# junofficial/mppi_RobotArm

Hardware: AMD Instinct MI355X
Metric: MPPI rollouts/sec (K×T state-steps/s) + control-step latency, K=65536 T=64 (higher is better)
Workload: dtype f32

## Files before the change

### include/mppi_rocm.h

```cpp
#ifndef MPPI_ROCM_H
#define MPPI_ROCM_H

#ifdef __cplusplus
extern "C" {
#endif

#define MPPI_MAX_T 128
#define MPPI_SEARCH_LEN 30

#define MPPI_OK 0
#define MPPI_E_ARG -1
#define MPPI_E_HIP -2
#define MPPI_E_SINGULAR -3
#define MPPI_E_EXCHANGE -5
#define MPPI_E_RETRY -6
#define MPPI_E_PATH_END -4

#define MPPI_FLAG_FUSED_UPDATE 1u
#define MPPI_FLAG_EXCHANGE 2u
#define MPPI_FLAG_HOST_OUT 4u
#define MPPI_IPC_HANDLE_BYTES 64
#define MPPI_MAX_WORLD 8

typedef struct {
    double m1, m2, l1, l2, lc1, lc2, g;
    double fk_l1, fk_l2;
} mppi_arm_params;

typedef struct {
    int K_local;
    int T;
    int K_total;
    int k_offset;
    double delta_t;
    double param_lambda;
    double param_alpha;
    double param_exploration;
    double sigma[4];
    double stage_cost_weight[4];
    double terminal_cost_weight[4];
    mppi_arm_params arm;
    int lanes_per_sample;
    double param_gamma;
    int clamp_mode;
    double u_min[2];
    double u_max[2];
} mppi_config;

typedef struct mppi_ctx mppi_ctx;

void mppi_config_init(mppi_config *cfg);

int mppi_ctx_create(const mppi_config *cfg, int device, void *stream, mppi_ctx **out);
void mppi_ctx_destroy(mppi_ctx *ctx);
const char *mppi_last_error(void);
int mppi_set_stream(mppi_ctx *ctx, void *stream);
int mppi_ctx_info(const mppi_ctx *ctx, int *lanes_per_sample, int *blocks, int *threads_per_block);

int mppi_ctx_handoff(const mppi_ctx *ctx, int *poll);

int mppi_set_step_inputs(mppi_ctx *ctx, const double *x0, const double *window, int W,
                         const double *u);

int mppi_rollout(mppi_ctx *ctx, const float *noise_dev, double *S_dev, double *partial_dev,
                 unsigned flags);

int mppi_merge_partials(mppi_ctx *ctx, const double *partials_dev, int n, unsigned flags);

int mppi_exchange_handle(mppi_ctx *ctx, int world, void *handle_out);
int mppi_exchange_attach(mppi_ctx *ctx, int rank, int world, const void *handles);

int mppi_get_weighted_noise(mppi_ctx *ctx, double *w_eps_host );
int mppi_get_nominal(mppi_ctx *ctx, double *u_host );

int mppi_rollout_traj(mppi_ctx *ctx, const double *base_u, const float *noise_dev, int K,
                      float *out_dev);

typedef struct mppi_readback mppi_readback;
int mppi_readback_create(int device, int workers, int slots, long long chunk_floats, int copy_streams,
                         mppi_readback **out);
void mppi_readback_destroy(mppi_readback *rb);
int mppi_readback_run(mppi_readback *rb, void *stream, const float *src_dev, double *dst_host, long long n);

int mppi_optimal_traj(mppi_ctx *ctx, float *out_dev);

int mppi_get_step_outputs(mppi_ctx *ctx, double *u_host, const float *traj_dev, float *traj_host);

int mppi_optimal_traj_host(const mppi_ctx *ctx, const double *x0, const double *u_new, double *traj_out);

int mppi_wait_outputs(mppi_ctx *ctx, const double *x0, double *u_out, double *traj_out);

int mppi_step_dropin(mppi_ctx *ctx, const double *x0, const double *window, int W, const double *u,
                     const float *noise_dev, double *S_dev, float *next_noise_dev, unsigned long long seed,
                     unsigned long long next_step, double *u_out, double *traj_out);

typedef struct {
    const double *path;
    int rows, stride;
    double fk_l1, fk_l2;
    const double *x0;
    long long *idx;
    double *u;
    double *traj;
    const float *noise_dev;
    float *next_noise_dev;
    double *S_dev;
    unsigned long long seed;
} mppi_dropin_binding;

int mppi_dropin_bind(mppi_ctx *ctx, const mppi_dropin_binding *b);

int mppi_dropin_tick(mppi_ctx *ctx, unsigned long long next_step);

int mppi_dropin_tick_launch(mppi_ctx *ctx, unsigned long long next_step);
int mppi_dropin_tick_wait(mppi_ctx *ctx);

int mppi_noise_philox(mppi_ctx *ctx, unsigned long long seed, unsigned long long step,
                      float *out_dev);

int mppi_sync(mppi_ctx *ctx);

#define MPPI_MAX_OBSTACLES 8
int mppi_set_obstacles(mppi_ctx *ctx, int n, const double *discs, double cost);

int mppi_debug_obstacle_hits(mppi_ctx *ctx, const float *noise_dev, int K, unsigned *mask_dev,
                             float *dir_dev);

int mppi_debug_set_buffer(mppi_ctx *ctx, void *dbg_dev);

int mppi_debug_dropin_times(const mppi_ctx *ctx, double *us_out);

int mppi_debug_nearest(mppi_ctx *ctx, const float *noise_dev, int K, int *slot_dev, float *pos_dev);

#define MPPI_CHAIN_MAX_DOF 8

typedef struct {
    int n;
    double m[MPPI_CHAIN_MAX_DOF];
    double l[MPPI_CHAIN_MAX_DOF];
    double lc[MPPI_CHAIN_MAX_DOF];
    double I[MPPI_CHAIN_MAX_DOF];
    double fk[MPPI_CHAIN_MAX_DOF];
    double J[MPPI_CHAIN_MAX_DOF];
    double b[MPPI_CHAIN_MAX_DOF];
    double g;
} mppi_chain_params;

typedef struct {
    int K_local, T, K_total, k_offset;
    double delta_t, param_lambda, param_alpha, param_exploration;
    double sigma[MPPI_CHAIN_MAX_DOF * MPPI_CHAIN_MAX_DOF];
    double stage_cost_weight[4];
    double terminal_cost_weight[4];
    mppi_chain_params chain;
    int precision;
    int lanes_per_sample;
    double param_gamma;
    int clamp_mode;
    double u_min[MPPI_CHAIN_MAX_DOF];
    double u_max[MPPI_CHAIN_MAX_DOF];
} mppi_chain_config;

typedef struct mppi_chain_ctx mppi_chain_ctx;

void mppi_chain_config_init(mppi_chain_config *cfg);

int mppi_chain_ctx_create(const mppi_chain_config *cfg, int device, void *stream, mppi_chain_ctx **out);
void mppi_chain_ctx_destroy(mppi_chain_ctx *ctx);
int mppi_chain_set_stream(mppi_chain_ctx *ctx, void *stream);
int mppi_chain_ctx_info(const mppi_chain_ctx *ctx, int *blocks, int *threads_per_block, int *poll,
                        int *lanes_per_sample);
int mppi_chain_set_step_inputs(mppi_chain_ctx *ctx, const double *x0, const double *window, int W,
                               const double *u);
int mppi_chain_rollout(mppi_chain_ctx *ctx, const float *noise_dev, double *S_dev, double *partial_dev,
                       unsigned flags);
int mppi_chain_merge_partials(mppi_chain_ctx *ctx, const double *partials_dev, int n, unsigned flags);
int mppi_chain_exchange_handle(mppi_chain_ctx *ctx, int world, void *handle_out);
int mppi_chain_exchange_attach(mppi_chain_ctx *ctx, int rank, int world, const void *handles);
int mppi_chain_get_weighted_noise(mppi_chain_ctx *ctx, double *w_eps_host);
int mppi_chain_get_nominal(mppi_chain_ctx *ctx, double *u_host);
int mppi_chain_wait_outputs(mppi_chain_ctx *ctx, const double *x0, double *u_out, double *traj_out);
int mppi_chain_last_eta(const mppi_chain_ctx *ctx, double *eta);
int mppi_chain_optimal_traj_host(mppi_chain_ctx *ctx, const double *x0, const double *u_new, double *traj_out);
int mppi_chain_rollout_traj(mppi_chain_ctx *ctx, const double *base_u, const float *noise_dev, int K,
                            float *out_dev);
int mppi_chain_noise_philox(mppi_chain_ctx *ctx, unsigned long long seed, unsigned long long step,
                            float *out_dev);
int mppi_chain_sync(mppi_chain_ctx *ctx);
int mppi_chain_debug_set_buffer(mppi_chain_ctx *ctx, void *dbg_dev);
int mppi_chain_debug_slots(mppi_chain_ctx *ctx, const float *noise_dev, double *S_dev, int *slots_dev);

#define MPPI_NP_POLY_WORDS 312
#define MPPI_NP_LOG_DATA 274
#define MPPI_NP_MAX_DU 8
#define MPPI_NP_MAX_STREAMS 1024
#define MPPI_NP_MAX_NORMALS 2147483647LL

typedef struct {
    unsigned key[624];
    int pos;
    int has_gauss;
    double gauss;
} mppi_np_state;

typedef struct {
    void *out_dev;
    long long K, T;
    int du;
    long long k_offset, K_local;
    long long stride_t, stride_k, stride_d;
    int src[MPPI_NP_MAX_DU];
    double scale[MPPI_NP_MAX_DU];
    double mean[MPPI_NP_MAX_DU];
    int dot2;
    double mat[4];
} mppi_np_target;

typedef struct mppi_np_ctx mppi_np_ctx;

int mppi_np_ctx_create(int device, const double *log_params, mppi_np_ctx **out);
void mppi_np_ctx_destroy(mppi_np_ctx *ctx);
int mppi_np_plan(const mppi_np_ctx *ctx, long long n, int pos, int has_gauss, int *block_stride, int *streams);
int mppi_np_set_jumps(mppi_np_ctx *ctx, int block_stride, int streams, const unsigned long long *polys, int words);
int mppi_np_draw(mppi_np_ctx *ctx, void *stream, const mppi_np_state *st, long long n, const mppi_np_target *tgt);
int mppi_np_draw_result(mppi_np_ctx *ctx, mppi_np_state *st_out);

#ifdef __cplusplus
}
#endif
#endif
```

### mppi_robotarm_amd/_native.py

```python
from __future__ import annotations

import ctypes as C
import os

HERE = os.path.dirname(os.path.abspath(__file__))
LIB_PATH = os.environ.get("MPPI_LIB_PATH") or os.path.join(HERE, "_lib", "libmppi_rocm.so")

MPPI_MAX_T = 128
MPPI_SEARCH_LEN = 30
MPPI_OK = 0
MPPI_E_ARG = -1
MPPI_E_HIP = -2
MPPI_E_SINGULAR = -3
MPPI_E_PATH_END = -4
MPPI_E_EXCHANGE = -5
MPPI_E_RETRY = -6
MPPI_FLAG_FUSED_UPDATE = 1
MPPI_FLAG_EXCHANGE = 2
MPPI_FLAG_HOST_OUT = 4
DP = C.POINTER(C.c_double)
MPPI_IPC_HANDLE_BYTES = 64
MPPI_MAX_WORLD = 8
MPPI_MAX_OBSTACLES = 8

EXPORTS = (
    "mppi_ctx_create", "mppi_ctx_destroy", "mppi_last_error", "mppi_set_stream", "mppi_ctx_info", "mppi_ctx_handoff",
    "mppi_set_step_inputs", "mppi_rollout", "mppi_merge_partials", "mppi_exchange_handle", "mppi_exchange_attach",
    "mppi_get_weighted_noise",
    "mppi_get_nominal", "mppi_rollout_traj", "mppi_optimal_traj", "mppi_get_step_outputs", "mppi_step_dropin",
    "mppi_optimal_traj_host", "mppi_wait_outputs", "mppi_dropin_bind", "mppi_dropin_tick",
    "mppi_dropin_tick_launch", "mppi_dropin_tick_wait",
    "mppi_noise_philox",
    "mppi_sync", "mppi_debug_set_buffer",
    "mppi_debug_nearest", "mppi_debug_dropin_times", "mppi_set_obstacles", "mppi_debug_obstacle_hits",
    "mppi_chain_ctx_create", "mppi_chain_ctx_destroy", "mppi_chain_set_stream", "mppi_chain_ctx_info",
    "mppi_chain_set_step_inputs", "mppi_chain_rollout", "mppi_chain_merge_partials", "mppi_chain_exchange_handle",
    "mppi_chain_exchange_attach",
    "mppi_chain_get_weighted_noise", "mppi_chain_get_nominal", "mppi_chain_rollout_traj",
    "mppi_chain_noise_philox", "mppi_chain_sync", "mppi_chain_debug_set_buffer", "mppi_chain_debug_slots",
    "mppi_chain_wait_outputs", "mppi_chain_optimal_traj_host", "mppi_chain_last_eta",
    "mppi_config_init", "mppi_chain_config_init",
    "mppi_np_ctx_create", "mppi_np_ctx_destroy", "mppi_np_plan", "mppi_np_set_jumps", "mppi_np_draw",
    "mppi_np_draw_result", "mppi_readback_create", "mppi_readback_destroy", "mppi_readback_run",
)


class DropinBindingC(C.Structure):
    _fields_ = [("path", C.c_void_p), ("rows", C.c_int), ("stride", C.c_int), ("fk_l1", C.c_double),
                ("fk_l2", C.c_double), ("x0", C.c_void_p), ("idx", C.c_void_p), ("u", C.c_void_p),
                ("traj", C.c_void_p), ("noise_dev", C.c_void_p), ("next_noise_dev", C.c_void_p),
                ("S_dev", C.c_void_p), ("seed", C.c_ulonglong)]


NP_MAX_DU = 8
NP_LOG_DATA = 274
NP_POLY_WORDS = 312


class NpStateC(C.Structure):
    _fields_ = [("key", C.c_uint * 624), ("pos", C.c_int), ("has_gauss", C.c_int), ("gauss", C.c_double)]


class NpTargetC(C.Structure):
    _fields_ = [("out_dev", C.c_void_p), ("K", C.c_longlong), ("T", C.c_longlong), ("du", C.c_int),
                ("k_offset", C.c_longlong), ("K_local", C.c_longlong), ("stride_t", C.c_longlong),
                ("stride_k", C.c_longlong), ("stride_d", C.c_longlong), ("src", C.c_int * NP_MAX_DU),
                ("scale", C.c_double * NP_MAX_DU), ("mean", C.c_double * NP_MAX_DU), ("dot2", C.c_int),
                ("mat", C.c_double * 4)]


class ArmParamsC(C.Structure):
    _fields_ = [(n, C.c_double) for n in ("m1", "m2", "l1", "l2", "lc1", "lc2", "g", "fk_l1", "fk_l2")]


class ConfigC(C.Structure):
    _fields_ = [
        ("K_local", C.c_int), ("T", C.c_int), ("K_total", C.c_int), ("k_offset", C.c_int),
        ("delta_t", C.c_double), ("param_lambda", C.c_double), ("param_alpha", C.c_double),
        ("param_exploration", C.c_double), ("sigma", C.c_double * 4),
        ("stage_cost_weight", C.c_double * 4), ("terminal_cost_weight", C.c_double * 4),
        ("arm", ArmParamsC), ("lanes_per_sample", C.c_int), ("param_gamma", C.c_double),
        ("clamp_mode", C.c_int), ("u_min", C.c_double * 2), ("u_max", C.c_double * 2),
    ]

    def __init__(self, *args, **kw):
        super().__init__(*args, **kw)
        if "param_gamma" not in kw and len(args) <= [f for f, _ in self._fields_].index("param_gamma"):
            self.param_gamma = float("nan")


CHAIN_MAX_DOF = 8


class ChainParamsC(C.Structure):
    _fields_ = [("n", C.c_int)] + [(f, C.c_double * CHAIN_MAX_DOF) for f in ("m", "l", "lc", "I", "fk", "J", "b")] + \
               [("g", C.c_double)]


class ChainConfigC(C.Structure):
    _fields_ = [
        ("K_local", C.c_int), ("T", C.c_int), ("K_total", C.c_int), ("k_offset", C.c_int),
        ("delta_t", C.c_double), ("param_lambda", C.c_double), ("param_alpha", C.c_double),
        ("param_exploration", C.c_double), ("sigma", C.c_double * (CHAIN_MAX_DOF * CHAIN_MAX_DOF)),
        ("stage_cost_weight", C.c_double * 4), ("terminal_cost_weight", C.c_double * 4),
        ("chain", ChainParamsC), ("precision", C.c_int), ("lanes_per_sample", C.c_int),
        ("param_gamma", C.c_double),
        ("clamp_mode", C.c_int), ("u_min", C.c_double * CHAIN_MAX_DOF), ("u_max", C.c_double * CHAIN_MAX_DOF),
    ]

    def __init__(self, *args, **kw):
        super().__init__(*args, **kw)
        if "param_gamma" not in kw and len(args) <= [f for f, _ in self._fields_].index("param_gamma"):
            self.param_gamma = float("nan")


class MPPIError(RuntimeError):
    """A failed C-ABI call (message from mppi_last_error)."""


class ExchangeError(MPPIError):
    """MPPI_E_EXCHANGE: the in-launch multi-GPU exchange of a step missed its poll bound on some rank.  Every
    rank of that step raises it and none applied the update (the controllers then run the step again over
    the collective fallback)."""


_lib = None


def open_library(path: str):
    if not os.path.exists(path):
        raise OSError(f"{path} is missing: build it with `python -c 'import __graft_entry__ as g; g.build()'`")
    L = C.CDLL(path)
    vp, dp, fp, ip = C.c_void_p, C.POINTER(C.c_double), C.c_void_p, C.POINTER(C.c_int)
    sig = {
        "mppi_ctx_create": ([C.POINTER(ConfigC), C.c_int, vp, C.POINTER(vp)], C.c_int),
        "mppi_ctx_destroy": ([vp], None),
        "mppi_last_error": ([], C.c_char_p),
        "mppi_set_stream": ([vp, vp], C.c_int),
        "mppi_ctx_info": ([vp, ip, ip, ip], C.c_int),
        "mppi_ctx_handoff": ([vp, ip], C.c_int),
        "mppi_set_step_inputs": ([vp, dp, dp, C.c_int, dp], C.c_int),
        "mppi_rollout": ([vp, fp, vp, vp, C.c_uint], C.c_int),
        "mppi_merge_partials": ([vp, vp, C.c_int, C.c_uint], C.c_int),
        "mppi_exchange_handle": ([vp, C.c_int, vp], C.c_int),
        "mppi_exchange_attach": ([vp, C.c_int, C.c_int, vp], C.c_int),
        "mppi_get_weighted_noise": ([vp, dp], C.c_int),
        "mppi_get_nominal": ([vp, dp], C.c_int),
        "mppi_rollout_traj": ([vp, dp, fp, C.c_int, fp], C.c_int),
        "mppi_optimal_traj": ([vp, fp], C.c_int),
        "mppi_get_step_outputs": ([vp, dp, fp, fp], C.c_int),
        "mppi_optimal_traj_host": ([vp, dp, dp, dp], C.c_int),
        "mppi_wait_outputs": ([vp, dp, dp, dp], C.c_int),
        "mppi_step_dropin": ([vp, vp, vp, C.c_int, vp, vp, vp, vp, C.c_ulonglong, C.c_ulonglong, vp, vp], C.c_int),
        "mppi_noise_philox": ([vp, C.c_ulonglong, C.c_ulonglong, fp], C.c_int),
        "mppi_dropin_bind": ([vp, C.POINTER(DropinBindingC)], C.c_int),
        "mppi_dropin_tick": ([vp, C.c_ulonglong], C.c_int),
        "mppi_dropin_tick_launch": ([vp, C.c_ulonglong], C.c_int),
        "mppi_dropin_tick_wait": ([vp], C.c_int),
        "mppi_sync": ([vp], C.c_int),
        "mppi_debug_set_buffer": ([vp, vp], C.c_int),
        "mppi_debug_dropin_times": ([vp, dp], C.c_int),
        "mppi_debug_nearest": ([vp, fp, C.c_int, vp, fp], C.c_int),
        "mppi_set_obstacles": ([vp, C.c_int, dp, C.c_double], C.c_int),
        "mppi_debug_obstacle_hits": ([vp, fp, C.c_int, vp, fp], C.c_int),
        "mppi_chain_ctx_create": ([C.POINTER(ChainConfigC), C.c_int, vp, C.POINTER(vp)], C.c_int),
        "mppi_chain_ctx_destroy": ([vp], None),
        "mppi_chain_set_stream": ([vp, vp], C.c_int),
        "mppi_chain_ctx_info": ([vp, ip, ip, ip, ip], C.c_int),
        "mppi_chain_set_step_inputs": ([vp, dp, dp, C.c_int, dp], C.c_int),
        "mppi_chain_rollout": ([vp, fp, vp, vp, C.c_uint], C.c_int),
        "mppi_chain_merge_partials": ([vp, vp, C.c_int, C.c_uint], C.c_int),
        "mppi_chain_exchange_handle": ([vp, C.c_int, vp], C.c_int),
        "mppi_chain_exchange_attach": ([vp, C.c_int, C.c_int, vp], C.c_int),
        "mppi_chain_get_weighted_noise": ([vp, dp], C.c_int),
        "mppi_chain_get_nominal": ([vp, dp], C.c_int),
        "mppi_chain_rollout_traj": ([vp, dp, fp, C.c_int, fp], C.c_int),
        "mppi_chain_noise_philox": ([vp, C.c_ulonglong, C.c_ulonglong, fp], C.c_int),
        "mppi_chain_sync": ([vp], C.c_int),
        "mppi_chain_debug_set_buffer": ([vp, vp], C.c_int),
        "mppi_chain_debug_slots": ([vp, fp, vp, vp], C.c_int),
        "mppi_chain_wait_outputs": ([vp, dp, dp, dp], C.c_int),
        "mppi_chain_optimal_traj_host": ([vp, dp, dp, dp], C.c_int),
        "mppi_chain_last_eta": ([vp, dp], C.c_int),
        "mppi_config_init": ([C.POINTER(ConfigC)], None),
        "mppi_np_ctx_create": ([C.c_int, vp, C.POINTER(vp)], C.c_int),
        "mppi_np_ctx_destroy": ([vp], None),
        "mppi_np_plan": ([vp, C.c_longlong, C.c_int, C.c_int, ip, ip], C.c_int),
        "mppi_np_set_jumps": ([vp, C.c_int, C.c_int, vp, C.c_int], C.c_int),
        "mppi_np_draw": ([vp, vp, C.POINTER(NpStateC), C.c_longlong, C.POINTER(NpTargetC)], C.c_int),
        "mppi_np_draw_result": ([vp, C.POINTER(NpStateC)], C.c_int),
        "mppi_chain_config_init": ([C.POINTER(ChainConfigC)], None),
        "mppi_readback_create": ([C.c_int, C.c_int, C.c_int, C.c_longlong, C.c_int, C.POINTER(vp)], C.c_int),
        "mppi_readback_destroy": ([vp], None),
        "mppi_readback_run": ([vp, vp, vp, vp, C.c_longlong], C.c_int),
    }
    for name, (args, res) in sig.items():
        if not hasattr(L, name):
            continue
        fn = getattr(L, name)
        fn.argtypes = args
        fn.restype = res
    return L


def load():
    global _lib
    if _lib is None:
        L = open_library(LIB_PATH)
        missing = [n for n in EXPORTS if not hasattr(L, n)]
        if missing:
            raise OSError(f"{LIB_PATH} is stale (missing {', '.join(missing)}): rebuild it")
        _lib = L
    return _lib


def check(rc: int, what: str) -> None:
    if rc != MPPI_OK:
        msg = load().mppi_last_error().decode(errors="replace")
        if rc == MPPI_E_SINGULAR:
            import numpy as np
            raise np.linalg.LinAlgError(msg)
        if rc == MPPI_E_ARG:
            raise ValueError(f"{what}: {msg}")
        if rc == MPPI_E_EXCHANGE:
            raise ExchangeError(f"{what}: {msg}")
        raise MPPIError(f"{what} failed ({rc}): {msg}")
```

### mppi_robotarm_amd/csrc/mppi_device.h

```cpp
#pragma once

#include <hip/hip_runtime.h>

#include <math.h>
#include <stdint.h>

#include <type_traits>
#include <utility>

#include "mppi_rocm.h"

namespace mppi {

#ifdef MPPI_STAMPS
#define STAMP(slot, val) do { if (dbg && threadIdx.x == 0) dbg[(size_t)blockIdx.x * 16 + (slot)] = (val); } while (0)
#define NOW() __builtin_amdgcn_s_memrealtime()
#else
#define STAMP(slot, val) do { (void)dbg; } while (0)
#define NOW() 0ull
#endif

constexpr int kMaxT = MPPI_MAX_T;

constexpr int kSlots = 32;
constexpr float kPadKey = 1.0e30f;
constexpr int kMaxWaves = 16;
constexpr int kGroup = 16;
constexpr double kMergeFloor = 5.421010862427522e-20;
constexpr int kDirectRows = 256;
constexpr int kDirectMax = 16;
constexpr int kSparseMax = 16;


__device__ __forceinline__ void sincos_f32(float x, float* s, float* c) { __sincosf(x, s, c); }

constexpr bool kDppBC = true;
template <int CTRL>
__device__ __forceinline__ float dpp_f32(float v) {
    return __int_as_float(__builtin_amdgcn_mov_dpp(__float_as_int(v), CTRL, 0xF, 0xF, kDppBC));
}

__device__ __forceinline__ int lanes_below(unsigned long long mask) {
    return __builtin_amdgcn_mbcnt_hi((unsigned)(mask >> 32), __builtin_amdgcn_mbcnt_lo((unsigned)mask, 0u));
}

template <int CTRL>
__device__ __forceinline__ double dpp_f64(double v) {
    const long long b = __double_as_longlong(v);
    const int lo = __builtin_amdgcn_mov_dpp((int)b, CTRL, 0xF, 0xF, kDppBC);
    const int hi = __builtin_amdgcn_mov_dpp((int)(b >> 32), CTRL, 0xF, 0xF, kDppBC);
    return __longlong_as_double(((long long)hi << 32) | (unsigned)lo);
}

__device__ __forceinline__ double readlane_f64(double v, int l) {
    const long long b = __double_as_longlong(v);
    const int lo = __builtin_amdgcn_readlane((int)b, l);
    const int hi = __builtin_amdgcn_readlane((int)(b >> 32), l);
    return __longlong_as_double(((long long)hi << 32) | (unsigned)lo);
}
__device__ __forceinline__ float readlane_f32(float v, int l) {
    return __int_as_float(__builtin_amdgcn_readlane(__float_as_int(v), l));
}

__device__ __forceinline__ double min_raw_f64(double a, double b) {
    double r;
    asm("v_min_f64 %0, %1, %2" : "=v"(r) : "v"(a), "v"(b));
    return r;
}
__device__ __forceinline__ double max_raw_f64(double a, double b) {
    double r;
    asm("v_max_f64 %0, %1, %2" : "=v"(r) : "v"(a), "v"(b));
    return r;
}

template <class T, class Op>
__device__ __forceinline__ T wave_reduce(T v, Op op) {
    if constexpr (sizeof(T) == 8) {
        v = op(v, dpp_f64<0xB1>(v));
        v = op(v, dpp_f64<0x4E>(v));
        v = op(v, dpp_f64<0x141>(v));
        v = op(v, dpp_f64<0x140>(v));
        return op(op(readlane_f64(v, 0), readlane_f64(v, 16)), op(readlane_f64(v, 32), readlane_f64(v, 48)));
    } else {
        v = op(v, dpp_f32<0xB1>(v));
        v = op(v, dpp_f32<0x4E>(v));
        v = op(v, dpp_f32<0x141>(v));
        v = op(v, dpp_f32<0x140>(v));
        return op(op(readlane_f32(v, 0), readlane_f32(v, 16)), op(readlane_f32(v, 32), readlane_f32(v, 48)));
    }
}
struct OpMin {
    __device__ double operator()(double a, double b) const { return min_raw_f64(a, b); }
};
struct OpAdd {
    template <class T>
    __device__ T operator()(T a, T b) const { return a + b; }
};
__device__ __forceinline__ double wave_min_f64(double v) { return wave_reduce(v, OpMin{}); }
__device__ __forceinline__ double wave_sum_f64(double v) { return wave_reduce(v, OpAdd{}); }
__device__ __forceinline__ float wave_sum_f32(float v) { return wave_reduce(v, OpAdd{}); }

__device__ __forceinline__ int select_bit(unsigned long long m, int k) {
    int pos = 0;
#pragma unroll
    for (int w = 32; w > 0; w >>= 1) {
        const int cnt = __popcll(m & ((1ull << w) - 1));
        if (k >= cnt) {
            k -= cnt;
            m >>= w;
            pos += w;
        }
    }
    return pos;
}

template <class F, int... I>
__device__ __forceinline__ void unroll_seq(F&& f, std::integer_sequence<int, I...>) {
    (f(std::integral_constant<int, I>{}), ...);
}

#define PIN_LOADS() asm volatile("" ::: "memory")

typedef __attribute__((address_space(4))) const float cfloat;
__device__ __forceinline__ float4 const_ld4(cfloat* p) { return make_float4(p[0], p[1], p[2], p[3]); }

typedef float f32x2 __attribute__((ext_vector_type(2)));
typedef float f32x4 __attribute__((ext_vector_type(4)));

__device__ __forceinline__ float min3_raw(float a, float b, float c) {
    float r;
    asm("v_min3_f32 %0, %1, %2, %3" : "=v"(r) : "v"(a), "v"(b), "v"(c));
    return r;
}
__device__ __forceinline__ float min_raw(float a, float b) {
    float r;
    asm("v_min_f32 %0, %1, %2" : "=v"(r) : "v"(a), "v"(b));
    return r;
}


template <int N>
__device__ __forceinline__ float min_tree(const float (&k)[N]) {
    if constexpr (N == 1) {
        return k[0];
    } else {
        constexpr int M = (N + 2) / 3;
        float r[M];
#pragma unroll
        for (int g = 0; g < M; ++g) {
            const int a = 3 * g;
            if (a + 2 < N) r[g] = min3_raw(k[a], k[a + 1], k[a + 2]);
            else if (a + 1 < N) r[g] = min_raw(k[a], k[a + 1]);
            else r[g] = k[a];
        }
        return min_tree<M>(r);
    }
}

template <int LPS, bool PRECISE = false>
struct Search {
    static constexpr int SL = ((MPPI_SEARCH_LEN + LPS - 1) / LPS + 1) & ~1;
    static constexpr int SP = SL / 2;
    f32x2 krx[SP], kry[SP], kc[SP];
    int sub;
    float cx, cy;

    __device__ __forceinline__ void load(const float4* key, float4 ctr, int lane_sub) {
        static_assert(SL * LPS <= kSlots, "window slots");
        if (LPS == 1) {
            int z;
            asm volatile("v_mov_b32 %0, 0" : "=v"(z));
            sub = z;
        } else {
            sub = lane_sub;
        }
#pragma unroll
        for (int i = 0; i < SP; ++i) {
            const float4 k0 = key[sub * SL + 2 * i];
            const float4 k1 = key[sub * SL + 2 * i + 1];
            krx[i] = f32x2{k0.x, k1.x};
            kry[i] = f32x2{k0.y, k1.y};
            kc[i] = f32x2{k0.z, k1.z};
        }
        cx = ctr.x;
        cy = ctr.y;
    }

    __device__ __forceinline__ unsigned nearest(float px, float py) const { return nearest_d(px - cx, py - cy); }

    __device__ __forceinline__ unsigned nearest_d(float dx, float dy) const {
        const f32x2 ax2 = {dx, dx}, ay2 = {dy, dy};
        const float pp = fmaf(dx, dx, dy * dy);
        const f32x2 pp2 = {pp, pp};
        float kk[2 * SP];
#pragma unroll
        for (int i = 0; i < SP; ++i) {
            f32x2 key = __builtin_elementwise_fma(ax2, krx[i], __builtin_elementwise_fma(ay2, kry[i], kc[i]));
            if constexpr (PRECISE) key = key + pp2;
            const unsigned j = (unsigned)(sub * SL + 2 * i);
            const float k0 = __uint_as_float((__float_as_uint(key.x) & ~31u) | j);
            const float k1 = __uint_as_float((__float_as_uint(key.y) & ~31u) | (j + 1));
            kk[2 * i] = k0;
            kk[2 * i + 1] = k1;
        }
        float best = min_tree<2 * SP>(kk);
        if (LPS >= 2) best = min_raw(best, dpp_f32<0xB1>(best));
        if (LPS >= 4) best = min_raw(best, dpp_f32<0x4E>(best));
        if (LPS >= 8) best = min_raw(best, dpp_f32<0x141>(best));
        if (LPS >= 16) best = min_raw(best, dpp_f32<0x128>(best));
        return __float_as_uint(best) & 31u;
    }
};

struct alignas(16) KeyPair {
    float4 xy;
    float4 c;
};
constexpr int kKeyPairs = kSlots / 2;

template <bool PRECISE = false>
struct SearchLDS {
    const KeyPair* kp;
    float cx, cy;

    __device__ __forceinline__ static void fill(KeyPair* dst, const float4* key, int tid) {
        if (tid < kKeyPairs) {
            const float4 k0 = key[2 * tid], k1 = key[2 * tid + 1];
            dst[tid].xy = make_float4(k0.x, k1.x, k0.y, k1.y);
            dst[tid].c = make_float4(k0.z, k1.z, 0.f, 0.f);
        }
    }

    __device__ __forceinline__ unsigned nearest(float px, float py) const {
        const float dx = px - cx, dy = py - cy;
        const f32x2 ax2 = {dx, dx}, ay2 = {dy, dy};
        const float pp = fmaf(dx, dx, dy * dy);
        const f32x2 pp2 = {pp, pp};
        float best = 3.0e38f;
        constexpr int SP = (MPPI_SEARCH_LEN + 1) / 2;
#pragma unroll
        for (int i = 0; i < SP; ++i) {
            const float4 xy = kp[i].xy, cc = kp[i].c;
            f32x2 key = __builtin_elementwise_fma(ax2, f32x2{xy.x, xy.y},
                                                  __builtin_elementwise_fma(ay2, f32x2{xy.z, xy.w}, f32x2{cc.x, cc.y}));
            if constexpr (PRECISE) key = key + pp2;
            const unsigned j = (unsigned)(2 * i);
            const float k0 = __uint_as_float((__float_as_uint(key.x) & ~31u) | j);
            const float k1 = __uint_as_float((__float_as_uint(key.y) & ~31u) | (j + 1));
            best = min3_raw(best, k0, k1);
        }
        return __float_as_uint(best) & 31u;
    }
};

template <int NL>
__device__ __forceinline__ double gather_col_n(const float* base, int kstride, const int* s_k, const double* s_e,
                                               int nl) {
    float e[NL];
#pragma unroll
    for (int l = 0; l < NL; ++l) e[l] = base[(size_t)(nl > 0 ? s_k[min(l, nl - 1)] : 0) * kstride];
    double acc = 0.0;
#pragma unroll
    for (int l = 0; l < NL; ++l)
        if (l < nl) acc = fma(s_e[l], (double)e[l], acc);
    return acc;
}
__device__ __forceinline__ double gather_col(const float* base, int kstride, const int* s_k, const double* s_e,
                                             int nl) {
    static_assert(kSparseMax == 16, "buckets");
    if (nl <= 1) return gather_col_n<1>(base, kstride, s_k, s_e, nl);
    if (nl <= 2) return gather_col_n<2>(base, kstride, s_k, s_e, nl);
    if (nl <= 4) return gather_col_n<4>(base, kstride, s_k, s_e, nl);
    if (nl <= 8) return gather_col_n<8>(base, kstride, s_k, s_e, nl);
    return gather_col_n<16>(base, kstride, s_k, s_e, nl);
}

__device__ __forceinline__ float weighted_sq(float ex, float ey, float e1, float e2, const float* w) {
    return fmaf(w[0], ex * ex, fmaf(w[1], ey * ey, fmaf(w[2], e1 * e1, w[3] * e2 * e2)));
}


typedef unsigned int u32x2 __attribute__((__vector_size__(2 * sizeof(unsigned int))));
typedef unsigned int u32x4 __attribute__((__vector_size__(4 * sizeof(unsigned int))));
constexpr int kSC1 = 16;

__device__ __forceinline__ __amdgpu_buffer_rsrc_t rows_rsrc(const void* p, int bytes) {
    return __builtin_amdgcn_make_buffer_rsrc(const_cast<void*>(p), 0, bytes, 0x00020000);
}
__device__ __forceinline__ double ld_wt(__amdgpu_buffer_rsrc_t r, int idx) {
    return __builtin_bit_cast(double, __builtin_amdgcn_raw_buffer_load_b64(r, idx * 8, 0, kSC1));
}
__device__ __forceinline__ void st_wt(__amdgpu_buffer_rsrc_t r, int idx, double v) {
    __builtin_amdgcn_raw_buffer_store_b64(__builtin_bit_cast(u32x2, v), r, idx * 8, 0, kSC1);
}
constexpr int kOffRange = 1 << 26;

__device__ __forceinline__ void st_gran(__amdgpu_buffer_rsrc_t r, int idx, double v, unsigned tag) {
    const unsigned long long b = (unsigned long long)__double_as_longlong(v);
    const u32x4 x = {(unsigned)b, tag, (unsigned)(b >> 32), tag};
    __builtin_amdgcn_raw_buffer_store_b128(x, r, idx * 16, 0, kSC1);
}
__device__ __forceinline__ u32x4 ld_gran(__amdgpu_buffer_rsrc_t r, int idx) {
    return __builtin_amdgcn_raw_buffer_load_b128(r, idx * 16, 0, kSC1);
}
__device__ __forceinline__ bool gran_ok(u32x4 x, unsigned tag) { return x[1] == tag && x[3] == tag; }
__device__ __forceinline__ double gran_val(u32x4 x) {
    return __longlong_as_double((long long)(((unsigned long long)x[2] << 32) | x[0]));
}
constexpr unsigned kSpinMax = 1u << 20;
__device__ __forceinline__ void report_timeout(unsigned* tmo) {
    if (tmo) __hip_atomic_store(tmo, 1u, __ATOMIC_RELAXED, __HIP_MEMORY_SCOPE_SYSTEM);
}
#define MPPI_SPIN_OR_GIVE_UP(spins, tmo, lane) MPPI_SPIN_OR_GIVE_UP_L(spins, 0ull, tmo, lane, (void)0)
#define MPPI_SPIN_OR_GIVE_UP_L(spins, deadline, tmo, lane, on_give_up)                                   \
    if (spins >= kSpinMax || ((deadline) && __builtin_amdgcn_s_memrealtime() > (deadline))) {            \
        if ((lane) == 0) report_timeout(tmo);                                                            \
        on_give_up;                                                                                      \
        break;                                                                                           \
    }                                                                                                    \
    __builtin_amdgcn_s_sleep(1)

__device__ __forceinline__ unsigned long long ord_key(double x) {
    const unsigned long long b = (unsigned long long)__double_as_longlong(x);
    return (b >> 63) ? ~b : (b | (1ull << 63));
}
__device__ __forceinline__ double ord_val(unsigned long long k) {
    return __longlong_as_double((long long)((k >> 63) ? (k & ~(1ull << 63)) : ~k));
}


template <int MAXV>
struct MergeScratch {
    double red[kMaxWaves];
    double weps[MAXV];
    double unew[MAXV];
    double rho[kDirectRows];
    double part[2 * kDirectRows];
    double eta;
    double rho_fin;
    int nrel;
};

template <int NT, class SM>
__device__ __forceinline__ double block_min_f64(double v, SM& sm) {
    const int lane = threadIdx.x & 63, wave = threadIdx.x >> 6;
    v = wave_min_f64(v);
    if (lane == 0) sm.red[wave] = v;
    __syncthreads();
    double r = sm.red[0];
#pragma unroll
    for (int w = 1; w < NT / 64; ++w) r = min_raw_f64(r, sm.red[w]);
    return r;
}

struct RowGeo {
    int stride, ncol;
    __device__ explicit RowGeo(int nval) : stride(2 + nval), ncol(1 + nval) {}
};

template <int NT, int MAXCH, class SM>
__device__ __forceinline__ void put_final(double rho, const double (&acc)[MAXCH], double eta, int nrel,
                                          const RowGeo& geo, SM& sm, double* out_row, double* w_eps_out) {
    const int tid = threadIdx.x;
#pragma unroll
    for (int ch = 0; ch < MAXCH; ++ch) {
        const int col = tid + ch * NT;
        if (col >= geo.ncol) continue;
        if (col == 0) {
            sm.nrel = nrel;
            sm.eta = eta;
            sm.rho_fin = rho;
            if (out_row) {
                out_row[0] = rho;
                out_row[1] = acc[ch];
            }
        } else {
            if (out_row) out_row[1 + col] = acc[ch];
            const double w = acc[ch] / eta;
            sm.weps[col - 1] = w;
            if (w_eps_out) w_eps_out[col - 1] = w;
        }
    }
    __syncthreads();
}

template <int NT, int MAXCH, bool final, bool GRAN, class SM>
__device__ __forceinline__ void merge_rows_block(__amdgpu_buffer_rsrc_t rows, int row0, int n, const RowGeo& geo,
                                                 double inv_lambda, SM& sm, const __amdgpu_buffer_rsrc_t* out_wt,
                                                 int out_idx, double* out_row, double* w_eps_out, unsigned tag,
                                                 unsigned* tmo, unsigned long long deadline = 0ull,
                                                 bool* failed = nullptr) {
    constexpr bool EAGER = !GRAN && MAXCH == 1;
    constexpr int LB = EAGER ? 32 : 16;
    constexpr int RB = LB / MAXCH;
    constexpr int R1 = EAGER ? 32 : 16;
    static_assert(RB >= 1 && R1 <= 64, "one row per lane");
    const int tid = threadIdx.x, lane = tid & 63;
    const int stride = geo.stride, ncol = geo.ncol;
    double acc[MAXCH], eta = 0.0, rho = INFINITY;
#pragma unroll
    for (int ch = 0; ch < MAXCH; ++ch) acc[ch] = 0.0;
    int nrel = 0;
    bool gave_up = false;
    for (int r0 = 0; r0 < n; r0 += R1) {
        const int nr = min(R1, n - r0);
        const int rb = row0 + r0;
        const int lrow = lane < nr ? (rb + lane) * stride : kOffRange;
        double rho_r, eta_l = 0.0, v[EAGER ? LB : 1];
        if constexpr (GRAN) {
            u32x4 gr;
            for (unsigned spins = 0;; ++spins) {
                asm volatile("" ::: "memory");
                gr = ld_gran(rows, lrow);
                if (__all(lane >= nr || gran_ok(gr, tag))) break;
                MPPI_SPIN_OR_GIVE_UP_L(spins, deadline, tmo, lane, gave_up = true);
            }
            rho_r = gran_val(gr);
        } else if constexpr (!EAGER) {
            rho_r = ld_wt(rows, lrow);
        } else {
            rho_r = ld_wt(rows, lrow);
            eta_l = ld_wt(rows, lrow + 1);
#pragma unroll
            for (int j = 0; j < LB; ++j) {
                const int i = j / MAXCH, col = tid + (j % MAXCH) * NT;
                v[j] = ld_wt(rows, (i < nr && col < ncol) ? (rb + i) * stride + 1 + col : kOffRange);
            }
        }
        const double rho_l = lane < nr ? rho_r : INFINITY;
        const double rnew = min_raw_f64(rho, wave_min_f64(rho_l));
        double s_l = 0.0;
        if (lane < nr) {
            const double s = exp((rnew - rho_l) * inv_lambda);
            s_l = s >= kMergeFloor ? s : 0.0;
        }
        const unsigned long long rel = __ballot(s_l != 0.0);
        const int nrr = __popcll(rel);
        nrel += nrr;
        if (rnew < rho && rho != INFINITY) {
            const double f = exp((rnew - rho) * inv_lambda);
#pragma unroll
            for (int ch = 0; ch < MAXCH; ++ch) acc[ch] *= f;
            eta *= f;
        }
        rho = rnew;
        if constexpr (EAGER) {
#pragma unroll
            for (int j = 0; j < LB; ++j) {
                const int i = j / MAXCH, ch = j % MAXCH;
                if (i < nr) {
                    const double s = readlane_f64(s_l, i);
                    if (s != 0.0) {
                        acc[ch] = fma(s, v[j], acc[ch]);
                        if (ch == 0) eta = fma(s, readlane_f64(eta_l, i), eta);
                    }
                }
            }
        } else {
            const int krow = lane < nrr ? select_bit(rel, lane) : 0;
            for (int b0 = 0; b0 < nrr; b0 += RB) {
                const bool eta_on = b0 == 0 && lane < nrr;
                const int eidx = eta_on ? (rb + krow) * stride + 1 : kOffRange;
                double x[LB];
                if constexpr (GRAN) {
                    u32x4 ge, gv[LB];
                    for (unsigned spins = 0;; ++spins) {
                        asm volatile("" ::: "memory");
                        ge = ld_gran(rows, eidx);
                        bool ok = !eta_on || gran_ok(ge, tag);
#pragma unroll
                        for (int j = 0; j < LB; ++j) {
                            const int i = b0 + j / MAXCH, col = tid + (j % MAXCH) * NT;
                            const bool on = i < nrr && col < ncol;
                            gv[j] = ld_gran(rows, on ? (rb + __builtin_amdgcn_readlane(krow, i)) * stride + 1 + col
                                                     : kOffRange);
                            ok = ok && (!on || gran_ok(gv[j], tag));
                        }
                        if (__all(ok)) break;
                        MPPI_SPIN_OR_GIVE_UP_L(spins, deadline, tmo, lane, gave_up = true);
                    }
                    if (eta_on) eta_l = gran_val(ge);
#pragma unroll
                    for (int j = 0; j < LB; ++j) x[j] = gran_val(gv[j]);
                } else {
                    if (b0 == 0) eta_l = ld_wt(rows, eidx);
#pragma unroll
                    for (int j = 0; j < LB; ++j) {
                        const int i = b0 + j / MAXCH, col = tid + (j % MAXCH) * NT;
                        x[j] = ld_wt(rows, (i < nrr && col < ncol)
                                               ? (rb + __builtin_amdgcn_readlane(krow, i)) * stride + 1 + col
                                               : kOffRange);
                    }
                }
#pragma unroll
                for (int j = 0; j < LB; ++j) {
                    const int i = b0 + j / MAXCH, ch = j % MAXCH;
                    if (i < nrr) {
                        const double s = readlane_f64(s_l, __builtin_amdgcn_readlane(krow, i));
                        acc[ch] = fma(s, x[j], acc[ch]);
                        if (ch == 0) eta = fma(s, readlane_f64(eta_l, i), eta);
                    }
                }
            }
        }
    }
    if (failed) *failed = __syncthreads_or(gave_up);
    if constexpr (final) {
        put_final<NT, MAXCH>(rho, acc, eta, nrel, geo, sm, out_row, w_eps_out);
    } else {
        auto put = [&](int col, double x) {
            if constexpr (GRAN) st_gran(*out_wt, out_idx * stride + col, x, tag);
            else st_wt(*out_wt, out_idx * stride + col, x);
        };
#pragma unroll
        for (int ch = 0; ch < MAXCH; ++ch) {
            const int col = tid + ch * NT;
            if (col >= ncol) continue;
            if (col == 0) put(0, rho);
            put(1 + col, acc[ch]);
        }
    }
}

template <int NT, int MAXCH, bool GRAN, class SM>
__device__ __forceinline__ bool direct_merge(__amdgpu_buffer_rsrc_t rows, int n, const RowGeo& geo,
                                             double inv_lambda, SM& sm, double* out_row, double* w_eps_out,
                                             unsigned tag, unsigned* tmo, unsigned long long* dbg = nullptr) {
    constexpr int P = kDirectRows / 64;
    constexpr int LB = 16;
    constexpr int RB = LB / MAXCH;
    const int tid = threadIdx.x, lane = tid & 63;
    const int stride = geo.stride, ncol = geo.ncol;
    double rho_l[P];
    if constexpr (GRAN) {
        if (tid < 64) {
            u32x4 gr[P];
            for (unsigned spins = 0;; ++spins) {
                asm volatile("" ::: "memory");
                bool ok = true;
#pragma unroll
                for (int j = 0; j < P; ++j) {
                    const int r = lane + 64 * j;
                    gr[j] = ld_gran(rows, r < n ? r * stride : kOffRange);
                    ok = ok && (r >= n || gran_ok(gr[j], tag));
                }
                if (__all(ok)) break;
                MPPI_SPIN_OR_GIVE_UP(spins, tmo, lane);
            }
#pragma unroll
            for (int j = 0; j < P; ++j) sm.rho[lane + 64 * j] = lane + 64 * j < n ? gran_val(gr[j]) : INFINITY;
        }
        __syncthreads();
#pragma unroll
        for (int j = 0; j < P; ++j) rho_l[j] = sm.rho[lane + 64 * j];
    } else {
#pragma unroll
        for (int j = 0; j < P; ++j) {
            const int r = lane + 64 * j;
            const double x = ld_wt(rows, r < n ? r * stride : kOffRange);
            rho_l[j] = r < n ? x : INFINITY;
        }
    }
    double m = rho_l[0];
#pragma unroll
    for (int j = 1; j < P; ++j) m = min_raw_f64(m, rho_l[j]);
    const double rho = wave_min_f64(m);
    double s_l[P];
    unsigned long long rel[P];
    int nrel = 0;
#pragma unroll
    for (int j = 0; j < P; ++j) {
        const double s = exp((rho - rho_l[j]) * inv_lambda);
        s_l[j] = (lane + 64 * j < n && s >= kMergeFloor) ? s : 0.0;
        rel[j] = __ballot(s_l[j] != 0.0);
        nrel += __popcll(rel[j]);
    }
    const int G = MAXCH == 1 ? max(1, NT / ncol) : 1;
    if (nrel > (G > 1 ? min(64, 2 * kDirectMax * G) : kDirectMax)) return false;
    int k = lane, row = 0;
    bool found = false;
#pragma unroll
    for (int j = 0; j < P; ++j) {
        const int cnt = __popcll(rel[j]);
        if (!found && k < cnt) {
            row = 64 * j + select_bit(rel[j], k);
            found = true;
        } else if (!found) {
            k -= cnt;
        }
    }
    double sk = 0.0;
#pragma unroll
    for (int j = 0; j < P; ++j) {
        const double sj = __shfl(s_l[j], row & 63);
        if ((row >> 6) == j) sk = sj;
    }
    const bool mine = lane < nrel;
    STAMP(13, NOW());
    double acc[MAXCH], eta = 0.0, eta_k = 0.0;
#pragma unroll
    for (int ch = 0; ch < MAXCH; ++ch) acc[ch] = 0.0;
    if (G == 1) {
        for (int b0 = 0; b0 < nrel; b0 += RB) {
            double v[LB];
            if constexpr (GRAN) {
                const bool eta_on = b0 == 0 && mine;
                u32x4 ge, gv[LB];
                for (unsigned spins = 0;; ++spins) {
                    asm volatile("" ::: "memory");
                    ge = ld_gran(rows, eta_on ? row * stride + 1 : kOffRange);
                    bool ok = !eta_on || gran_ok(ge, tag);
#pragma unroll
                    for (int j = 0; j < LB; ++j) {
                        const int i = b0 + j / MAXCH, col = tid + (j % MAXCH) * NT;
                        const bool on = i < nrel && col < ncol;
                        gv[j] = ld_gran(rows, on ? __builtin_amdgcn_readlane(row, i) * stride + 1 + col : kOffRange);
                        ok = ok && (!on || gran_ok(gv[j], tag));
                    }
                    if (__all(ok)) break;
                    MPPI_SPIN_OR_GIVE_UP(spins, tmo, lane);
                }
                if (eta_on) eta_k = gran_val(ge);
#pragma unroll
                for (int j = 0; j < LB; ++j) v[j] = gran_val(gv[j]);
            } else {
                if (b0 == 0) eta_k = ld_wt(rows, mine ? row * stride + 1 : kOffRange);
#pragma unroll
                for (int j = 0; j < LB; ++j) {
                    const int i = b0 + j / MAXCH, col = tid + (j % MAXCH) * NT;
                    v[j] = ld_wt(rows, (i < nrel && col < ncol) ? __builtin_amdgcn_readlane(row, i) * stride + 1 + col
                                                                 : kOffRange);
                }
            }
#pragma unroll
            for (int j = 0; j < LB; ++j) {
                const int i = b0 + j / MAXCH, ch = j % MAXCH;
                if (i < nrel) {
                    const double s = readlane_f64(sk, i);
                    acc[ch] = fma(s, v[j], acc[ch]);
                    if (ch == 0) eta = fma(s, readlane_f64(eta_k, i), eta);
                }
            }
        }
    } else {
        const int grp = tid / ncol, gcol = tid - grp * ncol;
        const bool active = grp < G;
        for (int b0 = 0; b0 < nrel; b0 += RB * G) {
            double v[LB], sf[LB];
            int roff[LB];
            bool on[LB];
#pragma unroll
            for (int j = 0; j < LB; ++j) {
                const int i = b0 + grp + G * j;
                on[j] = active && i < nrel;
                const int r = __builtin_amdgcn_ds_bpermute(min(i, 63) << 2, row);
                sf[j] = __shfl(sk, min(i, 63));
                roff[j] = on[j] ? r * stride + 1 + gcol : kOffRange;
            }
            if constexpr (GRAN) {
                u32x4 gv[LB];
                for (unsigned spins = 0;; ++spins) {
                    asm volatile("" ::: "memory");
                    bool ok = true;
#pragma unroll
                    for (int j = 0; j < LB; ++j) {
                        gv[j] = ld_gran(rows, roff[j]);
                        ok = ok && (!on[j] || gran_ok(gv[j], tag));
                    }
                    if (__all(ok)) break;
                    MPPI_SPIN_OR_GIVE_UP(spins, tmo, lane);
                }
#pragma unroll
                for (int j = 0; j < LB; ++j) v[j] = gran_val(gv[j]);
            } else {
#pragma unroll
                for (int j = 0; j < LB; ++j) v[j] = ld_wt(rows, roff[j]);
            }
#pragma unroll
            for (int j = 0; j < LB; ++j)
                if (on[j]) acc[0] = fma(sf[j], v[j], acc[0]);
        }
        if (active) sm.part[tid] = acc[0];
        __syncthreads();
        if (grp == 0) {
            double a = sm.part[gcol];
            for (int g = 1; g < G; ++g) a += sm.part[g * ncol + gcol];
            acc[0] = a;
            if (tid == 0) sm.red[0] = a;
        }
        __syncthreads();
        eta = sm.red[0];
    }
    STAMP(14, NOW());
    put_final<NT, MAXCH>(rho, acc, eta, nrel, geo, sm, out_row, w_eps_out);
    return true;
}

__device__ __forceinline__ bool arrive_last(unsigned* counter, unsigned expected, unsigned* s_flag, bool acquire) {
    asm volatile("s_waitcnt vmcnt(0)" ::: "memory");
    __syncthreads();
    if (threadIdx.x == 0) {
        const unsigned prev = __hip_atomic_fetch_add(counter, 1u, __ATOMIC_RELAXED, __HIP_MEMORY_SCOPE_AGENT);
        const bool last = prev == expected - 1;
        if (last) __hip_atomic_store(counter, 0u, __ATOMIC_RELAXED, __HIP_MEMORY_SCOPE_AGENT);
        if (last && acquire) {
            __builtin_amdgcn_fence(__ATOMIC_ACQUIRE, "agent");
            asm volatile("s_waitcnt vmcnt(0)" ::: "memory");
        }
        *s_flag = last ? 1u : 0u;
    }
    __syncthreads();
    return *s_flag != 0;
}


struct LaneWeight {
    double wgt;
    bool nz;
    unsigned long long bal;
};

__device__ __forceinline__ LaneWeight block_weigh(bool owner, double S, double rho_b, double inv_lambda, int lane,
                                                  int wave, int* s_cnt, double* s_redd) {
    const double warg = (rho_b - S) * inv_lambda;
    double wgt = 0.0;
    if (__any(owner && warg >= -45.0)) wgt = owner ? exp(warg) : 0.0;
    const bool nz = wgt >= kMergeFloor;
    const unsigned long long bal = __ballot(nz);
    const double esum = wave_sum_f64(nz ? wgt : 0.0);
    if (lane == 0) {
        s_cnt[wave] = __popcll(bal);
        s_redd[wave] = esum;
    }
    return LaneWeight{wgt, nz, bal};
}

template <int NT>
__device__ __forceinline__ int block_compact(const LaneWeight& lw, int k, int wave, const int* s_cnt,
                                             const double* s_redd, int* s_k, double* s_e, double* eta_b) {
    int off = 0, nl = 0;
    double eta = 0.0;
#pragma unroll
    for (int w = 0; w < NT / 64; ++w) {
        off += (w < wave) ? s_cnt[w] : 0;
        nl += s_cnt[w];
        eta += s_redd[w];
    }
    if (lw.nz) {
        const int pos = off + lanes_below(lw.bal);
        s_k[pos] = k;
        s_e[pos] = lw.wgt;
    }
    *eta_b = eta;
    return nl;
}

template <int NT, int NS>
__device__ __forceinline__ void dense_weights(const LaneWeight& lw, int k, int K, double* s_e,
                                              double (&w)[(NS + 63) / 64]) {
    const int tid = threadIdx.x, lane = tid & 63;
    const int k0 = blockIdx.x * NS;
    if (tid < NS) s_e[tid] = 0.0;
    __syncthreads();
    if (lw.nz) s_e[k - k0] = lw.wgt;
    __syncthreads();
#pragma unroll
    for (int i = 0; i < (NS + 63) / 64; ++i) {
        const int ks = lane + 64 * i;
        w[i] = (ks < NS && k0 + ks < K) ? s_e[ks] : 0.0;
    }
}

template <int NT, int MAXCH, bool POLL, class SM>
__device__ __forceinline__ bool handoff_merge(__amdgpu_buffer_rsrc_t slab_r, __amdgpu_buffer_rsrc_t gslab_r, int nrows,
                                              const RowGeo& geo, double inv_lambda, SM& sm, unsigned* counters,
                                              bool acquire, unsigned* s_flag, double* partial_out, double* w_eps_out,
                                              unsigned tag, unsigned* epoch, unsigned* tmo, unsigned long long* dbg,
                                              unsigned long long* direct_dbg) {
    const int ngroups = (nrows + kGroup - 1) / kGroup;
    const int g = blockIdx.x / kGroup;
    const int gsz = min(kGroup, nrows - g * kGroup);
    if constexpr (POLL) {
        if ((int)blockIdx.x != g * kGroup) return false;
        STAMP(3, NOW());
        if (ngroups == 1) {
            merge_rows_block<NT, MAXCH, true, true>(slab_r, 0, gsz, geo, inv_lambda, sm, nullptr, 0, partial_out,
                                                    w_eps_out, tag, tmo);
        } else if (blockIdx.x == 0 && nrows <= kDirectRows &&
                   direct_merge<NT, MAXCH, true>(slab_r, nrows, geo, inv_lambda, sm, partial_out, w_eps_out, tag, tmo,
                                                 direct_dbg)) {
        } else {
            merge_rows_block<NT, MAXCH, false, true>(slab_r, g * kGroup, gsz, geo, inv_lambda, sm, &gslab_r, g, nullptr,
                                                     nullptr, tag, tmo);
            STAMP(10, NOW());
            if (blockIdx.x != 0) return false;
            STAMP(4, NOW());
            merge_rows_block<NT, MAXCH, true, true>(gslab_r, 0, ngroups, geo, inv_lambda, sm, nullptr, 0, partial_out,
                                                    w_eps_out, tag, tmo);
        }
        if (threadIdx.x == 0) __hip_atomic_store(epoch, tag, __ATOMIC_RELAXED, __HIP_MEMORY_SCOPE_AGENT);
    } else {
        if (!arrive_last(counters + g, (unsigned)gsz, s_flag, acquire)) return false;
        STAMP(3, NOW());
        merge_rows_block<NT, MAXCH, false, false>(slab_r, g * kGroup, gsz, geo, inv_lambda, sm, &gslab_r, g, nullptr,
                                                  nullptr, 0u, nullptr);
        STAMP(10, NOW());
        if (!arrive_last(counters + ngroups, (unsigned)ngroups, s_flag, acquire)) return false;
        STAMP(4, NOW());
        if (!(ngroups > 1 && nrows <= kDirectRows &&
              direct_merge<NT, MAXCH, false>(slab_r, nrows, geo, inv_lambda, sm, partial_out, w_eps_out, 0u, nullptr)))
            merge_rows_block<NT, MAXCH, true, false>(gslab_r, 0, ngroups, geo, inv_lambda, sm, nullptr, 0, partial_out,
                                                     w_eps_out, 0u, nullptr);
    }
    return true;
}

__device__ __forceinline__ double median10(double* v) {
#define CX(i, j) { const double lo = min_raw_f64(v[i], v[j]), hi = max_raw_f64(v[i], v[j]); v[i] = lo; v[j] = hi; }
    CX(4, 9) CX(3, 8) CX(2, 7) CX(1, 6) CX(0, 5) CX(1, 4) CX(6, 9) CX(0, 3) CX(5, 8) CX(0, 2)
    CX(3, 6) CX(7, 9) CX(0, 1) CX(2, 4) CX(5, 7) CX(8, 9) CX(1, 2) CX(4, 6) CX(7, 8) CX(3, 5)
    CX(2, 5) CX(6, 8) CX(1, 3) CX(4, 7) CX(2, 3) CX(6, 7) CX(3, 4) CX(5, 6) CX(4, 5)
#undef CX
    return v[5];
}

template <class SM>
__device__ __forceinline__ double median_at(const SM& sm, int t, int d, int T, int du) {
    double v[10];
#pragma unroll
    for (int i = 0; i < 10; ++i) {
        int m = t - 5 + i;
        m = m < 0 ? -m - 1 : m;
        m = m >= T ? 2 * T - 1 - m : m;
        v[i] = sm.weps[m * du + d];
    }
    return median10(v);
}


__device__ __forceinline__ unsigned long long mul_wide(unsigned a, unsigned m) {
    return (unsigned long long)a * m;
}
__device__ __forceinline__ unsigned xor3(unsigned a, unsigned b, unsigned k) {
    unsigned r;
    asm("v_bitop3_b32 %0, %1, %2, %3 bitop3:0x96" : "=v"(r) : "v"(a), "v"(b), "s"(k));
    return r;
}
__device__ __forceinline__ uint4 philox4x32_10(uint4 ctr, uint2 key) {
#pragma unroll
    for (int r = 0; r < 10; ++r) {
        const unsigned long long p0 = mul_wide(ctr.x, 0xD2511F53u);
        const unsigned long long p1 = mul_wide(ctr.z, 0xCD9E8D57u);
        ctr = make_uint4(xor3((unsigned)(p1 >> 32), ctr.y, key.x), (unsigned)p1,
                         xor3((unsigned)(p0 >> 32), ctr.w, key.y), (unsigned)p0);
        key.x += 0x9E3779B9u;
        key.y += 0xBB67AE85u;
    }
    return ctr;
}

constexpr double kBoxMullerScale = 1.1774100225154747;
__device__ __forceinline__ float2 box_muller(unsigned a, unsigned b) {
    const float inv = 2.3283064365386963e-10f;
    const float u0 = fmaf((float)a, inv, inv), u1 = (float)b * inv;
    const float r = __builtin_amdgcn_sqrtf(-__builtin_amdgcn_logf(u0));
    return make_float2(r * __builtin_amdgcn_cosf(u1), r * __builtin_amdgcn_sinf(u1));
}

}

namespace mppi {

constexpr int kMaxWorld = MPPI_MAX_WORLD;
struct XDesc {
    const void* peer[kMaxWorld];
    double* row;
    unsigned* epoch;
    int rank, world, bytes;
    unsigned timeout_ticks;
};
constexpr unsigned kTmoLocal = 1u, kTmoExchange = 2u, kTmoSplit = 4u;
__device__ __forceinline__ void st_gran_sys(__amdgpu_buffer_rsrc_t r, int idx, double v, unsigned tag) {
    const unsigned long long b = (unsigned long long)__double_as_longlong(v);
    const u32x4 x = {(unsigned)b, tag, (unsigned)(b >> 32), tag};
    __builtin_amdgcn_raw_buffer_store_b128(x, r, idx * 16, 0, kSC1 | 1);
}

template <int NT, int MAXCH, class SM>
__device__ __forceinline__ unsigned exchange_send_merge(const XDesc& x, const RowGeo& geo, double inv_lambda, SM& sm,
                                                        double* w_eps_out, unsigned* tmo) {
    const unsigned tag = (unsigned)__builtin_amdgcn_readfirstlane((int)*x.epoch) + 1u;
    const int par = (int)(tag & 1u), stride = geo.stride;
    for (int idx = threadIdx.x; idx < stride; idx += NT) {
        const double v = x.row[idx];
        for (int p = 0; p < x.world; ++p)
            st_gran_sys(rows_rsrc(x.peer[p], x.bytes), (par * x.world + x.rank) * stride + idx, v, tag);
    }
    bool late = false;
    const unsigned long long dl = x.timeout_ticks ? __builtin_amdgcn_s_memrealtime() + x.timeout_ticks : 0ull;
    merge_rows_block<NT, MAXCH, true, true>(rows_rsrc(x.peer[x.rank], x.bytes), par * x.world, x.world, geo,
                                            inv_lambda, sm, nullptr, 0, nullptr, w_eps_out, tag, nullptr, dl, &late);
    late = __syncthreads_or(late || (threadIdx.x == 0 && tmo &&
                                     __hip_atomic_load(tmo, __ATOMIC_RELAXED, __HIP_MEMORY_SCOPE_SYSTEM) != 0u));
    const int sbase = 2 * x.world * stride + par * x.world;
    if ((int)threadIdx.x < x.world)
        st_gran_sys(rows_rsrc(x.peer[threadIdx.x], x.bytes), sbase + x.rank, late ? -1.0 : 1.0, tag);
    return tag;
}

template <int NT>
__device__ __forceinline__ bool exchange_verdict(const XDesc& x, const RowGeo& geo, unsigned tag, unsigned* tmo) {
    const int par = (int)(tag & 1u);
    const int sbase = 2 * x.world * geo.stride + par * x.world;
    const int tid = threadIdx.x, lane = tid & 63;
    bool bad = false, split = false;
    if (tid < 64) {
        const __amdgpu_buffer_rsrc_t own = rows_rsrc(x.peer[x.rank], x.bytes);
        u32x4 g;
        bool missing = false;
        const unsigned long long dl = x.timeout_ticks ? __builtin_amdgcn_s_memrealtime() + x.timeout_ticks : 0ull;
        for (unsigned spins = 0;; ++spins) {
            asm volatile("" ::: "memory");
            g = ld_gran(own, lane < x.world ? sbase + lane : kOffRange);
            if (__all(lane >= x.world || gran_ok(g, tag))) break;
            MPPI_SPIN_OR_GIVE_UP_L(spins, dl, nullptr, lane, missing = true);
        }
        bad = __any(lane < x.world && !(gran_ok(g, tag) && gran_val(g) > 0.0)) || missing;
        split = missing && !__any(lane == x.rank && gran_ok(g, tag) && gran_val(g) < 0.0);
    }
    bad = __syncthreads_or(bad);
    split = __syncthreads_or(split);
    if (tid == 0) {
        if (bad)
            __hip_atomic_store(tmo + 1, split ? kTmoExchange | kTmoSplit : kTmoExchange, __ATOMIC_RELAXED,
                               __HIP_MEMORY_SCOPE_SYSTEM);
        *x.epoch = tag;
    }
    return !bad;
}

}

constexpr int kCuSlots = 2048;
constexpr int kPrioShift = 12;
__device__ __forceinline__ unsigned cu_key() {
    const unsigned hw = __builtin_amdgcn_s_getreg(0xF804);
    const unsigned xcc = __builtin_amdgcn_s_getreg(0xF814);
    return ((xcc & 7u) << 8) | (((hw >> 13) & 7u) << 5) | (((hw >> 12) & 1u) << 4) | ((hw >> 8) & 0xFu);
}
__device__ __forceinline__ void draw_cu_ticket(unsigned* cu_ctr, unsigned* s_parity) {
    if (threadIdx.x == 0)
        *s_parity = __hip_atomic_fetch_add(cu_ctr + cu_key(), 1u, __ATOMIC_RELAXED, __HIP_MEMORY_SCOPE_AGENT) & 1u;
}
__device__ __forceinline__ void fair_priority(unsigned parity) {
    if ((((unsigned)__builtin_amdgcn_s_memrealtime() >> kPrioShift) & 1u) ^ parity)
        __builtin_amdgcn_s_setprio(1);
    else
        __builtin_amdgcn_s_setprio(0);
}
```

### mppi_robotarm_amd/csrc/mppi_rocm.hip

```cpp
#include <hip/hip_runtime.h>

#include <math.h>
#include <stdint.h>
#include <stdio.h>
#include <stdlib.h>
#include <string.h>

#include <algorithm>
#include <chrono>
#include <string>
#include <type_traits>

#include "mppi_device.h"
#include "mppi_host.h"
#include "mppi_rocm.h"

namespace {

using namespace mppi;

constexpr int kThreads = 256;

struct alignas(16) StepStatic {
    float4 win[kSlots];
    float4 key[kSlots];
    float4 x0;
    float4 ctr;
};

struct alignas(16) DevStep {
    float4 ua[kMaxT];
    double u[kMaxT][2];
};

struct KConst {
    int K_local, T, k_offset, k_exploit, nblocks, acquire;
    float dt, fk1, fk2;
    float A, B, D, E, P, Q;
    float sw[4], tw[4];
    double lambda, inv_lambda, gamma;
    double sig_inv[4];
};

struct ClampK {
    double u_lo[2], u_hi[2];
    float v_lo[2], v_hi[2];
    int mode;
};

struct ObstK {
    float cx[MPPI_MAX_OBSTACLES], cy[MPPI_MAX_OBSTACLES];
    float r2[MPPI_MAX_OBSTACLES];
    double w;
    int n;
};

struct Arm {
    f32x2 Q;
    f32x2 dq;
    f32x2 cs1;
    f32x2 cs12;
};

struct DynK {
    f32x2 zB, DA;
    f32x2 ED;
    f32x2 nP0, nQ;
    f32x2 dt2;
    f32x2 fk;
    f32x2 ctr;
    f32x2 w01, w23;
    f32x2 vlo, vhi;
};

template <class V>
__device__ __forceinline__ V vgpr_opaque(V v) {
    asm volatile("" : "+v"(v));
    return v;
}

__device__ __forceinline__ float arg_f(const float& f) {
    float x = f;
    asm volatile("" : "+s"(x));
    return x;
}

__device__ __forceinline__ DynK make_dynk(const KConst& c, float cx, float cy) {
    const float A = arg_f(c.A), B = arg_f(c.B), D = arg_f(c.D), E = arg_f(c.E), P = arg_f(c.P), Q = arg_f(c.Q);
    const float dt = arg_f(c.dt), fk1 = arg_f(c.fk1), fk2 = arg_f(c.fk2);
    DynK k;
    k.zB = vgpr_opaque(f32x2{0.f, B});
    k.DA = vgpr_opaque(f32x2{D, A});
    k.ED = vgpr_opaque(f32x2{E, D});
    k.nP0 = vgpr_opaque(f32x2{-P, 0.f});
    k.nQ = vgpr_opaque(f32x2{-Q, -Q});
    k.dt2 = vgpr_opaque(f32x2{dt, dt * 0.15915494309189535f});
    k.fk = vgpr_opaque(f32x2{fk1, fk2});
    k.ctr = vgpr_opaque(f32x2{cx, cy});
    k.w01 = vgpr_opaque(f32x2{arg_f(c.sw[0]), arg_f(c.sw[1])});
    k.w23 = vgpr_opaque(f32x2{arg_f(c.sw[2]), arg_f(c.sw[3])});
    return k;
}

__device__ __forceinline__ void dynk_limits(DynK& k, const ClampK& cl) {
    k.vlo = vgpr_opaque(f32x2{arg_f(cl.v_lo[0]), arg_f(cl.v_lo[1])});
    k.vhi = vgpr_opaque(f32x2{arg_f(cl.v_hi[0]), arg_f(cl.v_hi[1])});
}

__device__ __forceinline__ f32x2 clamp_v(f32x2 v, const DynK& k) {
    return f32x2{__builtin_amdgcn_fmed3f(v.x, k.vlo.x, k.vhi.x), __builtin_amdgcn_fmed3f(v.y, k.vlo.y, k.vhi.y)};
}

__device__ __forceinline__ f32x2 splat(float x) { return f32x2{x, x}; }

constexpr int kObstPairs = MPPI_MAX_OBSTACLES / 2;
struct ObstR {
    const float4* rec;
    int n;
};
struct DiscPair {
    f32x2 cX, cY, r2;
};
__device__ __forceinline__ void stage_obst(float4* rec, const ObstK& ob) {
#pragma unroll
    for (int p = 0; p < kObstPairs; ++p) {
        rec[2 * p] = make_float4(ob.cx[2 * p], ob.cx[2 * p + 1], ob.cy[2 * p], ob.cy[2 * p + 1]);
        rec[2 * p + 1] = make_float4(ob.r2[2 * p], ob.r2[2 * p + 1], 0.f, 0.f);
    }
}
__device__ __forceinline__ DiscPair load_pair(const ObstR& o, int p) {
    const float4 a = o.rec[2 * p], b = o.rec[2 * p + 1];
    return DiscPair{f32x2{a.x, a.y}, f32x2{a.z, a.w}, f32x2{b.x, b.y}};
}

__device__ __forceinline__ void seg_hits(f32x2 pX, f32x2 pY, f32x2 cs, float L, f32x2 r2, bool& ha, bool& hb) {
    const f32x2 s = __builtin_elementwise_fma(pY, splat(cs.y), pX * splat(cs.x));
    const f32x2 t = {__builtin_amdgcn_fmed3f(s.x, 0.f, L), __builtin_amdgcn_fmed3f(s.y, 0.f, L)};
    const f32x2 oX = __builtin_elementwise_fma(-t, splat(cs.x), pX);
    const f32x2 oY = __builtin_elementwise_fma(-t, splat(cs.y), pY);
    const f32x2 d = __builtin_elementwise_fma(oY, oY, oX * oX);
    ha = d.x < r2.x;
    hb = d.y < r2.y;
}

__device__ __forceinline__ void disc_pair_hits(const ObstR& o, int p, f32x2 cs1, f32x2 cs12, f32x2 fk, bool (&h)[4]) {
    const DiscPair d = load_pair(o, p);
    seg_hits(d.cX, d.cY, cs1, fk.x, d.r2, h[0], h[2]);
    const f32x2 qX = __builtin_elementwise_fma(splat(-fk.x), splat(cs1.x), d.cX);
    const f32x2 qY = __builtin_elementwise_fma(splat(-fk.x), splat(cs1.y), d.cY);
    seg_hits(qX, qY, cs12, fk.y, d.r2, h[1], h[3]);
}

template <int NP>
__device__ __forceinline__ bool obst_any(const ObstR& o, f32x2 cs1, f32x2 cs12, f32x2 fk) {
    bool any = false;
#pragma unroll
    for (int p = 0; p < (NP ? NP : kObstPairs); ++p) {
        if (NP == 0 && 2 * p >= o.n) break;
        bool h[4];
        disc_pair_hits(o, p, cs1, cs12, fk, h);
        any |= (h[0] | h[1]) | (h[2] | h[3]);
    }
    return any;
}

__device__ __forceinline__ unsigned obst_mask(const ObstR& o, f32x2 cs1, f32x2 cs12, f32x2 fk) {
    unsigned m = 0;
#pragma unroll
    for (int p = 0; p < kObstPairs; ++p) {
        if (2 * p >= o.n) break;
        bool h[4];
        disc_pair_hits(o, p, cs1, cs12, fk, h);
#pragma unroll
        for (int b = 0; b < 4; ++b) m |= (h[b] ? 1u : 0u) << (4 * p + b);
    }
    return m;
}

__device__ __forceinline__ f32x2 cossin_rev(float a) { return f32x2{__builtin_amdgcn_cosf(a), __builtin_amdgcn_sinf(a)}; }

__device__ __forceinline__ void arm_init(Arm& x, float4 x0) {
    x.Q = f32x2{x0.x, x0.y} * 0.15915494309189535f;
    x.dq = f32x2{x0.z, x0.w};
    x.cs1 = cossin_rev(x.Q.x);
    x.cs12 = cossin_rev(x.Q.x + x.Q.y);
}

__device__ __forceinline__ f32x2 cos_sin_diff(f32x2 cs1, f32x2 cs12) {
    const f32x2 m = cs12 * splat(cs1.x);
    f32x2 r;
    asm("v_pk_fma_f32 %0, %1, %2, %3 op_sel:[1,1,0] op_sel_hi:[0,1,1] neg_hi:[1,0,0]"
        : "=v"(r) : "v"(cs12), "v"(cs1), "v"(m));
    return r;
}

__device__ __forceinline__ void arm_step(Arm& x, f32x2 v, const DynK& k) {
    const float c1 = x.cs1.x, c12 = x.cs12.x;
    const f32x2 cs2 = cos_sin_diff(x.cs1, x.cs12);
    const float c2 = cs2.x, s2 = cs2.y;
    const f32x2 DM11 = __builtin_elementwise_fma(k.zB, splat(c2), k.DA);
    const float M12 = fmaf(k.ED.x, c2, k.ED.y);
    const float h = k.ED.x * s2;
    const f32x2 w = __builtin_elementwise_fma(k.nQ, splat(c12), __builtin_elementwise_fma(k.nP0, splat(c1), v));
    const float dq1 = x.dq.x, dq2 = x.dq.y;
    const float hd1 = h * dq1;
    const f32x2 r = {fmaf(h * dq2, fmaf(2.f, dq1, dq2), w.x), fmaf(-hd1, dq1, w.y)};
    const float det = fmaf(DM11.y, k.ED.y, -(M12 * M12));
    const float rdet = __builtin_amdgcn_rcpf(det);
    const f32x2 ddq = __builtin_elementwise_fma(splat(-M12), f32x2{r.y, r.x}, DM11 * r) * splat(rdet);
    x.dq = __builtin_elementwise_fma(ddq, splat(k.dt2.x), x.dq);
    x.Q = __builtin_elementwise_fma(x.dq, splat(k.dt2.y), x.Q);
    x.cs1 = cossin_rev(x.Q.x);
    x.cs12 = cossin_rev(x.Q.x + x.Q.y);
}

__device__ __forceinline__ f32x2 arm_fk(const Arm& x, const DynK& k) {
    return __builtin_elementwise_fma(splat(k.fk.x), x.cs1, splat(k.fk.y) * x.cs12);
}

__device__ __forceinline__ float cost_pk(f32x2 e, f32x2 f, f32x2 w01, f32x2 w23) {
    const f32x2 s = __builtin_elementwise_fma(f * w23, f, (e * w01) * e);
    return s.x + s.y;
}

using Scratch = MergeScratch<2 * kMaxT>;

__device__ __forceinline__ double nominal_src(const DevStep* st, int tid, int T) {
    const int t = tid >> 1, src = t + 1 < T ? t + 1 : T - 1;
    return tid < 2 * T ? st->u[src][tid & 1] : 0.0;
}
__device__ __forceinline__ double nominal_first(const DevStep* st, int tid) {
    return tid < 2 ? st->u[0][tid] : 0.0;
}

struct HostOut {
    double* p;
    unsigned seq;
};

__host__ __device__ __forceinline__ double clamp_u(double u, double lo, double hi) { return u < lo ? lo : (u > hi ? hi : u); }

template <int NT, bool CLAMP>
__device__ void nominal_update_block(DevStep* nxt, const KConst& c, Scratch& sm, double u_src, double u_first,
                                     float* upd, HostOut ho, const ClampK& cl, bool publish = true) {
    const int tid = threadIdx.x;
    const int T = c.T;
    if (tid < ((2 * T + 63) & ~63)) {
        const int t = tid >> 1, d = tid & 1;
        const int src = t + 1 < T ? t + 1 : T - 1;
        double un = tid < 2 * T ? u_src + median_at(sm, src, d, T, 2) : 0.0;
        bool clampu = false;
        if constexpr (CLAMP) clampu = cl.mode == 2;
        if (clampu) un = clamp_u(un, cl.u_lo[d], cl.u_hi[d]);
        const double other = dpp_f64<0xB1>(un);
        if ((upd || ho.p) && tid < 2) {
            double u0 = u_first + median_at(sm, 0, d, T, 2);
            if (clampu) u0 = clamp_u(u0, cl.u_lo[d], cl.u_hi[d]);
            if (upd) upd[d] = (float)u0;
            if (ho.p) ho.p[2 + d] = u0;
        }
        if (tid < 2 * T) {
            if (upd && t + 1 < T) upd[2 * (t + 1) + d] = (float)un;
            if (ho.p) ho.p[4 + tid] = un;
            nxt->u[t][d] = un;
            if (d == 0) {
                const double u0 = un, u1 = other;
                const double g0 = c.gamma * u0, g1 = c.gamma * u1;
                const double a0 = g0 * c.sig_inv[0] + g1 * c.sig_inv[2];
                const double a1 = g0 * c.sig_inv[1] + g1 * c.sig_inv[3];
                nxt->ua[t] = make_float4((float)u0, (float)u1, (float)a0, (float)a1);
            }
        }
    }
    if (ho.p) {
        __threadfence_system();
        if (!publish) return;
        __syncthreads();
        if (tid == 0) __hip_atomic_store(reinterpret_cast<unsigned*>(ho.p), ho.seq, __ATOMIC_RELEASE, __HIP_MEMORY_SCOPE_SYSTEM);
    }
}


constexpr int kPF = 4;

template <int LPS, int NT, bool POLL, bool CLAMP, bool OBST>
__global__ __launch_bounds__(NT) void rollout_kernel(
    const KConst c, const StepStatic ss, const DevStep* __restrict__ st, const float2* __restrict__ noise,
    double* __restrict__ S_out, double* __restrict__ slab, double* __restrict__ gslab,
    unsigned* __restrict__ counters, double* __restrict__ partial_out, double* __restrict__ w_eps_out,
    DevStep* __restrict__ nxt, unsigned flags, const XDesc xd, unsigned* __restrict__ epoch, unsigned* __restrict__ tmo,
    float* __restrict__ upd, const HostOut ho, unsigned long long* __restrict__ dbg, const ClampK cl,
    const ObstK ob) {
    static_assert(CLAMP || !OBST, "the OBST kernels are built with CLAMP only");
    __shared__ float4 s_win[kSlots];
    __shared__ float4 s_ua[kMaxT + kPF];
    __shared__ double s_redd[NT / 64];
    __shared__ int s_cnt[NT / 64];
    __shared__ int s_k[NT];
    __shared__ double s_e[NT];
    __shared__ unsigned s_flag;
    __shared__ Scratch sm;

    const int tid = threadIdx.x, lane = tid & 63, wave = tid >> 6;
    const int k_raw = (blockIdx.x * NT + tid) / LPS;
    const bool valid = k_raw < c.K_local;
    const int k = valid ? k_raw : c.K_local - 1;
    const float exf = (c.k_offset + k) < c.k_exploit ? 1.f : 0.f;
    const int K = c.K_local, T = c.T;

    STAMP(0, NOW());
#ifdef MPPI_STAMPS
    STAMP(8, (unsigned long long)__builtin_amdgcn_s_getreg(0xF804));
    STAMP(9, (unsigned long long)__builtin_amdgcn_s_getreg(0xF814));
#endif
    const float2* np = noise + k;
    float2 ring[kPF];
#pragma unroll
    for (int j = 0; j < kPF; ++j) ring[j] = np[(size_t)(j < T ? j : T - 1) * K];
    const unsigned tag_v = POLL ? __hip_atomic_load(epoch, __ATOMIC_RELAXED, __HIP_MEMORY_SCOPE_AGENT) + 1u : 0u;
    const double u_cur = (flags & MPPI_FLAG_FUSED_UPDATE) ? nominal_src(st, tid, T) : 0.0;
    const double u_first = (flags & MPPI_FLAG_FUSED_UPDATE) ? nominal_first(st, tid) : 0.0;
    const float4 wrow = ss.win[tid & (kSlots - 1)];
    Search<LPS> sr;
    sr.load(ss.key, ss.ctr, tid & (LPS - 1));
    Arm x;
    arm_init(x, ss.x0);
    DynK dk = make_dynk(c, sr.cx, sr.cy);
    if constexpr (CLAMP) dynk_limits(dk, cl);
    ObstR od{};
    if constexpr (OBST) {
        __shared__ float4 s_obst[2 * kObstPairs];
        if (tid == 0) stage_obst(s_obst, ob);
        od = ObstR{s_obst, __builtin_amdgcn_readfirstlane(ob.n)};
    }
    int hits = 0;
    bool hit_last = false;
    for (int i = tid; i < T + kPF; i += NT) s_ua[i] = st->ua[i < T ? i : T - 1];
    if (tid < kSlots) s_win[tid] = wrow;
    __syncthreads();
    float4 uring[kPF];
#pragma unroll
    for (int j = 0; j < kPF; ++j) uring[j] = s_ua[j < T ? j : T - 1];

    double S = 0.0;
    f32x2 S4 = {0.f, 0.f};
    f32x2 ee = {0.f, 0.f}, ef = {0.f, 0.f};
    float4 pr = make_float4(0.f, 0.f, 0.f, 0.f);
    f32x2 pp = {0.f, 0.f}, pd = {0.f, 0.f};
    auto add_pending = [&]() {
        f32x4 r = {pr.x, pr.y, pr.z, pr.w};
        asm volatile("" : "+v"(r) : "v"(x.cs12));
        ee = pp - f32x2{r.x, r.y};
        ef = pd - f32x2{r.z, r.w};
        S4 = __builtin_elementwise_fma(ef * dk.w23, ef, __builtin_elementwise_fma(ee * dk.w01, ee, S4));
    };
    int ua_off = vgpr_opaque(0);
    auto dstep = [&](int t, auto slot_c, auto h_c, auto np_c) {
        constexpr int slot = decltype(slot_c)::value;
        constexpr int H = decltype(h_c)::value;
        constexpr int NP = decltype(np_c)::value;
        const bool h = H == 2 ? t > 0 : H == 1;
        f32x2 e = {ring[slot].x, ring[slot].y};
        f32x4 ua = {uring[slot].x, uring[slot].y, uring[slot].z, uring[slot].w};
        asm volatile("" : "+v"(e), "+v"(ua));
        f32x2 v = __builtin_elementwise_fma(splat(exf), f32x2{ua.x, ua.y}, e);
        if constexpr (CLAMP) v = clamp_v(v, dk);
        S4 = __builtin_elementwise_fma(f32x2{ua.z, ua.w}, v, S4);
        const int tl = t + kPF < T ? t + kPF : T - 1;
        ring[slot] = np[(size_t)tl * K];
        uring[slot] = *reinterpret_cast<const float4*>(reinterpret_cast<const char*>(s_ua) + ua_off +
                                                       (kPF + slot) * (int)sizeof(float4));
        if (slot == kPF - 1) ua_off += kPF * (int)sizeof(float4);
        PIN_LOADS();
        arm_step(x, v, dk);
        if (h) {
            add_pending();
            if (slot == 0) {
                S += (double)(S4.x + S4.y);
                S4 = f32x2{0.f, 0.f};
            }
        }
        if constexpr (OBST) {
            hit_last = obst_any<NP>(od, x.cs1, x.cs12, dk.fk);
            hits += hit_last ? 1 : 0;
        }
        pp = arm_fk(x, dk);
        pd = x.dq;
        const f32x2 d = pp - dk.ctr;
        pr = s_win[sr.nearest_d(d.x, d.y)];
    };
    using I0 = std::integral_constant<int, 0>;
    using I1 = std::integral_constant<int, 1>;
    using I2 = std::integral_constant<int, 2>;
    using I3 = std::integral_constant<int, 3>;
    using H0 = std::integral_constant<int, 0>;
    using H1 = std::integral_constant<int, 1>;
    using H2 = std::integral_constant<int, 2>;
    static_assert(kPF == 4, "unrolled for a 4-deep ring");
    using NP = std::integral_constant<int, (OBST && LPS == 1) ? kObstPairs : 0>;
    int t = 0;
    STAMP(12, NOW());
    if constexpr (LPS == 1) {
        dstep(0, I0{}, H0{}, NP{});
        for (t = 1; t + kPF <= T; t += kPF) {
            dstep(t, I1{}, H1{}, NP{});
            dstep(t + 1, I2{}, H1{}, NP{});
            dstep(t + 2, I3{}, H1{}, NP{});
            dstep(t + 3, I0{}, H1{}, NP{});
#ifdef MPPI_STAMPS
            if (t == 1) STAMP(13, NOW());
            if (t + kPF == T / 2 + 1) STAMP(14, NOW());
#endif
        }
        if (t < T) dstep(t, I1{}, H1{}, NP{});
        if (t + 1 < T) dstep(t + 1, I2{}, H1{}, NP{});
        if (t + 2 < T) dstep(t + 2, I3{}, H1{}, NP{});
    } else {
        for (; t + kPF <= T; t += kPF) {
            dstep(t, I0{}, H2{}, NP{});
            dstep(t + 1, I1{}, H2{}, NP{});
            dstep(t + 2, I2{}, H2{}, NP{});
            dstep(t + 3, I3{}, H2{}, NP{});
#ifdef MPPI_STAMPS
            if (t == 0) STAMP(13, NOW());
            if (t + kPF == T / 2) STAMP(14, NOW());
#endif
        }
        if (t < T) dstep(t, I0{}, H2{}, NP{});
        if (t + 1 < T) dstep(t + 1, I1{}, H2{}, NP{});
        if (t + 2 < T) dstep(t + 2, I2{}, H2{}, NP{});
    }
    add_pending();
    S += (double)(S4.x + S4.y);
    S += (double)cost_pk(ee, ef, f32x2{arg_f(c.tw[0]), arg_f(c.tw[1])}, f32x2{arg_f(c.tw[2]), arg_f(c.tw[3])});
    if constexpr (OBST) {
        hits += hit_last ? 1 : 0;
        S += ob.w * (double)hits;
    }

    STAMP(1, NOW());
    const bool owner = valid && sr.sub == 0;
    if (S_out && owner) S_out[k] = S;

    const int stride = 2 + 2 * T;
    const RowGeo geo(2 * T);
    const int nrows = c.nblocks;
    const int ngroups = (nrows + kGroup - 1) / kGroup;
    constexpr int kValBytes = POLL ? 16 : 8;
    const __amdgpu_buffer_rsrc_t slab_r = rows_rsrc(slab, nrows * stride * kValBytes);
    const __amdgpu_buffer_rsrc_t gslab_r = rows_rsrc(gslab, ngroups * stride * kValBytes);
    const unsigned tag = __builtin_amdgcn_readfirstlane(tag_v);
    auto publish = [&](int idx, double v) {
        if constexpr (POLL) st_gran(slab_r, idx, v, tag);
        else st_wt(slab_r, idx, v);
    };
    const double rho_b = block_min_f64<NT>(owner ? S : INFINITY, sm);
    if (tid == 0) publish(blockIdx.x * stride, rho_b);
    const LaneWeight lw = block_weigh(owner, S, rho_b, c.inv_lambda, lane, wave, s_cnt, s_redd);
    __syncthreads();
    double eta_b;
    int nl = block_compact<NT>(lw, k, wave, s_cnt, s_redd, s_k, s_e, &eta_b);
    __syncthreads();
    if (tid == 0) publish(blockIdx.x * stride + 1, eta_b);
    STAMP(15, NOW());
    nl = __builtin_amdgcn_readfirstlane(nl);
    if (nl <= kSparseMax) {
        const float* nf = reinterpret_cast<const float*>(noise);
        for (int col = tid; col < 2 * T; col += NT) {
            const float* base = nf + (size_t)(col >> 1) * K * 2 + (col & 1);
            publish(blockIdx.x * stride + 2 + col, gather_col(base, 2, s_k, s_e, nl));
        }
    } else {
        constexpr int NS = NT / LPS;
        constexpr int PER = (NS + 63) / 64;
        constexpr int kRowBatch = 4;
        const int k0 = blockIdx.x * NS;
        double w[PER];
        dense_weights<NT, NS>(lw, k, K, s_e, w);
        for (int tb = wave * kRowBatch; tb < T; tb += (NT / 64) * kRowBatch) {
            float2 e[kRowBatch][PER];
#pragma unroll
            for (int r = 0; r < kRowBatch; ++r) {
                const int tr = min(tb + r, T - 1);
#pragma unroll
                for (int i = 0; i < PER; ++i)
                    e[r][i] = noise[(size_t)tr * K + min(k0 + lane + 64 * i, K - 1)];
            }
#pragma unroll
            for (int r = 0; r < kRowBatch; ++r) {
                double ax = 0.0, ay = 0.0;
#pragma unroll
                for (int i = 0; i < PER; ++i) {
                    ax = fma(w[i], (double)e[r][i].x, ax);
                    ay = fma(w[i], (double)e[r][i].y, ay);
                }
                ax = wave_sum_f64(ax);
                ay = wave_sum_f64(ay);
                if (lane == 0 && tb + r < T) {
                    publish(blockIdx.x * stride + 2 + 2 * (tb + r), ax);
                    publish(blockIdx.x * stride + 3 + 2 * (tb + r), ay);
                }
            }
        }
    }
    STAMP(2, NOW());
    STAMP(5, (unsigned long long)nl);
    if (!handoff_merge<NT, 1, POLL>(slab_r, gslab_r, nrows, geo, c.inv_lambda, sm, counters, c.acquire != 0, &s_flag,
                                    partial_out, w_eps_out, tag, epoch, tmo, dbg, dbg))
        return;
    STAMP(11, NOW());
    STAMP(6, (unsigned long long)sm.nrel);
    if (flags & MPPI_FLAG_EXCHANGE) {
        const unsigned xtag = exchange_send_merge<NT, 1>(xd, geo, c.inv_lambda, sm, w_eps_out, tmo);
        if (flags & MPPI_FLAG_FUSED_UPDATE) nominal_update_block<NT, CLAMP>(nxt, c, sm, u_cur, u_first, upd, ho, cl, false);
        exchange_verdict<NT>(xd, geo, xtag, tmo);
        if ((flags & MPPI_FLAG_FUSED_UPDATE) && ho.p && threadIdx.x == 0)
            __hip_atomic_store(reinterpret_cast<unsigned*>(ho.p), ho.seq, __ATOMIC_RELEASE, __HIP_MEMORY_SCOPE_SYSTEM);
    } else if (flags & MPPI_FLAG_FUSED_UPDATE) {
        nominal_update_block<NT, CLAMP>(nxt, c, sm, u_cur, u_first, upd, ho, cl);
    }
    STAMP(7, NOW());
}

template <int NT, bool CLAMP>
__global__ __launch_bounds__(NT) void merge_kernel(const KConst c, const double* parts, int n, double* w_eps_out,
                                                   const DevStep* cur, DevStep* nxt, unsigned flags, float* upd,
                                                   const HostOut ho, const ClampK cl) {
    __shared__ Scratch sm;
    const int tid = threadIdx.x;
    const double u_cur = (flags & MPPI_FLAG_FUSED_UPDATE) ? nominal_src(cur, tid, c.T) : 0.0;
    const double u_first = (flags & MPPI_FLAG_FUSED_UPDATE) ? nominal_first(cur, tid) : 0.0;
    const __amdgpu_buffer_rsrc_t r = rows_rsrc(parts, n * (2 + 2 * c.T) * 8);
    merge_rows_block<NT, 1, true, false>(r, 0, n, RowGeo(2 * c.T), c.inv_lambda, sm, nullptr, 0, nullptr, w_eps_out,
                                         0u, nullptr);
    if (flags & MPPI_FLAG_FUSED_UPDATE) nominal_update_block<NT, CLAMP>(nxt, c, sm, u_cur, u_first, upd, ho, cl);
}

constexpr int kTrajTB = 8;
template <bool NOISE, bool CLAMP>
__global__ __launch_bounds__(kThreads) void traj_kernel(const KConst c, const StepStatic ss,
                                                        const float2* __restrict__ base, int bstride,
                                                        const float2* __restrict__ noise, int Kn,
                                                        float4* __restrict__ out, const ClampK cl) {
    __shared__ float4 tile[kTrajTB][kThreads];
    const int tid = threadIdx.x;
    const int k0 = blockIdx.x * kThreads;
    const int k = min(k0 + tid, Kn - 1);
    const int nk = min(kThreads, Kn - k0);
    const int T = c.T;
    const float exf = NOISE ? ((c.k_offset + k) < c.k_exploit ? 1.f : 0.f) : 1.f;
    Arm x;
    arm_init(x, ss.x0);
    DynK dk = make_dynk(c, 0.f, 0.f);
    if constexpr (CLAMP) dynk_limits(dk, cl);
    auto load_tile = [&](int t0, float2 (&d)[kTrajTB]) {
#pragma unroll
        for (int j = 0; j < kTrajTB; ++j) {
            const int t = min(t0 + j, T - 1);
            const int ti = t == 0 ? T - 1 : t - 1;
            d[j] = NOISE ? noise[(size_t)ti * c.K_local + k] : make_float2(0.f, 0.f);
        }
    };
    auto tile_steps = [&](const float2 (&cur)[kTrajTB], int t0) {
        const int nt = min(kTrajTB, T - t0);
#pragma unroll
        for (int j = 0; j < kTrajTB; ++j) {
            if (j >= nt) break;
            const int t = t0 + j;
            const int ti = t == 0 ? T - 1 : t - 1;
            const float2 b = base[ti * bstride];
            f32x2 v = {b.x, b.y};
            if (NOISE) v = __builtin_elementwise_fma(splat(exf), v, f32x2{cur[j].x, cur[j].y});
            if constexpr (CLAMP) v = clamp_v(v, dk);
            arm_step(x, v, dk);
            const f32x2 q = x.Q * 6.283185307179586f;
            tile[j][tid] = make_float4(q.x, q.y, x.dq.x, x.dq.y);
        }
        __syncthreads();
        for (int i = tid; i < nk * nt; i += kThreads) {
            const int s = i / nt, j = i - s * nt;
            out[(size_t)(k0 + s) * T + t0 + j] = tile[j][s];
        }
        __syncthreads();
    };
    float2 ta[kTrajTB], tb[kTrajTB], tc[kTrajTB];
    load_tile(0, ta);
    load_tile(kTrajTB, tb);
    for (int t0 = 0; t0 < T; t0 += 3 * kTrajTB) {
        load_tile(t0 + 2 * kTrajTB, tc);
        tile_steps(ta, t0);
        if (t0 + kTrajTB >= T) break;
        load_tile(t0 + 3 * kTrajTB, ta);
        tile_steps(tb, t0 + kTrajTB);
        if (t0 + 2 * kTrajTB >= T) break;
        load_tile(t0 + 4 * kTrajTB, tb);
        tile_steps(tc, t0 + 2 * kTrajTB);
    }
}

__global__ __launch_bounds__(kThreads) void nearest_debug_kernel(const KConst c, const StepStatic ss,
                                                                 const DevStep* __restrict__ st,
                                                                 const float2* __restrict__ noise, int Kn,
                                                                 int* __restrict__ slot, float2* __restrict__ pos,
                                                                 const ClampK cl) {
    const int k = blockIdx.x * kThreads + threadIdx.x;
    if (k >= Kn) return;
    const int T = c.T;
    const float exf = (c.k_offset + k) < c.k_exploit ? 1.f : 0.f;
    Search<1> sr;
    sr.load(ss.key, ss.ctr, 0);
    Arm x;
    arm_init(x, ss.x0);
    DynK dk = make_dynk(c, sr.cx, sr.cy);
    dynk_limits(dk, cl);
    const bool clampv = cl.mode != 0;
    for (int t = 0; t < T; ++t) {
        const float4 ua = st->ua[t];
        const float2 e = noise[(size_t)t * c.K_local + k];
        f32x2 v = __builtin_elementwise_fma(splat(exf), f32x2{ua.x, ua.y}, f32x2{e.x, e.y});
        if (clampv) v = clamp_v(v, dk);
        arm_step(x, v, dk);
        const f32x2 p = arm_fk(x, dk);
        const f32x2 d = p - dk.ctr;
        slot[(size_t)k * T + t] = (int)sr.nearest_d(d.x, d.y);
        pos[(size_t)k * T + t] = make_float2(p.x, p.y);
    }
}

__global__ __launch_bounds__(kThreads) void obstacle_debug_kernel(const KConst c, const StepStatic ss,
                                                                  const DevStep* __restrict__ st,
                                                                  const float2* __restrict__ noise, int Kn,
                                                                  unsigned* __restrict__ mask, float4* __restrict__ dir,
                                                                  const ClampK cl, const ObstK ob) {
    const int k = blockIdx.x * kThreads + threadIdx.x;
    const int T = c.T;
    const float exf = (c.k_offset + k) < c.k_exploit ? 1.f : 0.f;
    Arm x;
    arm_init(x, ss.x0);
    DynK dk = make_dynk(c, 0.f, 0.f);
    dynk_limits(dk, cl);
    __shared__ float4 s_obst[2 * kObstPairs];
    if (threadIdx.x == 0) stage_obst(s_obst, ob);
    __syncthreads();
    const ObstR od{s_obst, __builtin_amdgcn_readfirstlane(ob.n)};
    if (k >= Kn) return;
    for (int t = 0; t < T; ++t) {
        const float4 ua = st->ua[t];
        const float2 e = noise[(size_t)t * c.K_local + k];
        f32x2 v = __builtin_elementwise_fma(splat(exf), f32x2{ua.x, ua.y}, f32x2{e.x, e.y});
        v = clamp_v(v, dk);
        arm_step(x, v, dk);
        mask[(size_t)k * T + t] = obst_mask(od, x.cs1, x.cs12, dk.fk);
        dir[(size_t)k * T + t] = make_float4(x.cs1.x, x.cs1.y, x.cs12.x, x.cs12.y);
    }
}

__global__ __launch_bounds__(kThreads) void philox_noise_kernel(int K_local, int T, long long k_offset,
                                                                unsigned long long seed,
                                                                unsigned long long step, float L00,
                                                                float L10, float L11, float2* out) {
    const int k = (int)blockIdx.x * kThreads + (int)threadIdx.x;
    if (k >= K_local) return;
    const int t0 = 2 * (int)blockIdx.y;
    const unsigned long long kg = (unsigned long long)(k_offset + k);
    const uint4 ctr = make_uint4((unsigned)kg, (unsigned)(kg >> 32), (unsigned)t0, (unsigned)step);
    const uint2 key = make_uint2((unsigned)seed, (unsigned)(seed >> 32) ^ (unsigned)(step >> 32));
    const uint4 r = philox4x32_10(ctr, key);
    const float2 za = box_muller(r.x, r.y), zb = box_muller(r.z, r.w);
    const float z0 = za.x, z1 = za.y, z2 = zb.x, z3 = zb.y;
    out[(size_t)t0 * K_local + k] = make_float2(L00 * z0, fmaf(L10, z0, L11 * z1));
    if (t0 + 1 < T) out[(size_t)(t0 + 1) * K_local + k] = make_float2(L00 * z2, fmaf(L10, z2, L11 * z3));
}

}


struct mppi_ctx {
    mppi_config cfg;
    int device = 0;
    hipStream_t stream = nullptr;
    int lps = 1, nt = 256, nblocks = 0;
    KConst kc;
    ClampK ck{};
    ObstK ok{};
    StepStatic stat{};
    mppi_host::DevBuf<DevStep> d_step;
    int cur = 0;
    mppi_host::PinnedBuf<DevStep> h_step;
    mppi_host::Event staged;
    bool stage_pending = false;
    bool nominal_published = false;
    bool x_flipped = false;
    mppi_host::MappedBuf<double> h_dout;
    unsigned dseq = 0;
    double dropin_us[6] = {};
    mppi_host::Handoff hand;
    mppi_host::DevBuf<double> d_weps;
    mppi_host::PinnedBuf<double> h_buf;
    mppi_host::DevBuf<float2> d_base;
    mppi_host::PinnedBuf<float2> h_base;
    mppi_host::DevBuf<float2> d_upd;
    bool upd_valid = false;
    mppi_host::PinnedBuf<double> h_out;
    mppi_dropin_binding bind{};
    bool bound = false;
    std::chrono::steady_clock::time_point tick_t0{};
    bool in_tick = false;
    bool tick_launched = false;
    std::chrono::steady_clock::time_point step_t0{};
    double sig_inv[4];
    unsigned long long* d_dbg = nullptr;
    mppi_host::Exchange ex;
};

namespace {
using mppi_host::fail;
using mppi_host::launch_check;

using mppi_host::with_bool;
using mppi_host::with_value;

template <class F>
void with_rollout(const mppi_ctx* c, bool poll, F&& f) {
    with_value<1, 2, 4, 8, 16>(c->lps, [&](auto lps) {
        with_value<256, 512>(c->nt, [&](auto nt) {
            with_bool(poll, [&](auto p) {
                if (c->ok.n > 0)
                    f(lps, nt, p, std::true_type{}, std::true_type{});
                else
                    with_bool(c->ck.mode != 0, [&](auto cl) { f(lps, nt, p, cl, std::false_type{}); });
            });
        });
    });
}

bool took_update(mppi_ctx* c, int rc, unsigned flags) {
    if (rc != MPPI_OK || !(flags & MPPI_FLAG_FUSED_UPDATE)) return false;
    c->cur ^= 1;
    c->upd_valid = true;
    c->nominal_published = false;
    return true;
}

int check_timeout(mppi_ctx* c) {
    unsigned v;
    const int rc = c->hand.take_timeout(&v);
    if (v == kTmoExchange) {
        if (c->x_flipped) c->cur ^= 1;
        c->x_flipped = false;
        c->upd_valid = false;
        c->nominal_published = false;
    }
    return rc;
}

int auto_lps(int K_local) {
    const long long waves1 = ((long long)K_local + 63) / 64;
    if (waves1 >= 1024) return 1;
    if (waves1 >= 512) return 2;
    if (waves1 >= 128) return 4;
    if (waves1 >= 64) return 8;
    return 16;
}

int alloc(mppi_ctx* c) {
    HIP_TRY(hipSetDevice(c->device));
    int ncu = 0, per_cu = 0;
    HIP_TRY(hipDeviceGetAttribute(&ncu, hipDeviceAttributeMultiprocessorCount, c->device));
    with_rollout(c, true, [&](auto lps, auto nt, auto p, auto cl, auto ob) {
        const void* f = (const void*)rollout_kernel<lps, nt, p, cl, ob>;
        if (hipOccupancyMaxActiveBlocksPerMultiprocessor(&per_cu, f, nt, 0) != hipSuccess) per_cu = 0;
    });
    if (int rc = c->hand.setup(c->nblocks, ncu, per_cu, 2 + 2 * c->cfg.T, 0)) return rc;
    c->kc.acquire = c->hand.acquire;
    if (int rc = c->d_step.alloc_zeroed(2)) return rc;
    if (int rc = c->d_weps.alloc_zeroed(2 * kMaxT)) return rc;
    if (int rc = c->d_base.alloc(kMaxT)) return rc;
    if (int rc = c->d_upd.alloc(kMaxT)) return rc;
    if (int rc = c->h_out.alloc(4 * kMaxT)) return rc;
    if (int rc = c->h_step.alloc(1)) return rc;
    if (int rc = c->h_buf.alloc(2 * kMaxT)) return rc;
    if (int rc = c->h_base.alloc(kMaxT)) return rc;
    if (int rc = c->h_dout.alloc(4 + 2 * kMaxT, mppi_host::kCoherent)) return rc;
    if (int rc = c->staged.create()) return rc;
    HIP_TRY(hipDeviceSynchronize());
    memset(c->h_step, 0, sizeof(DevStep));
    memset(c->h_dout, 0, (4 + 2 * kMaxT) * sizeof(double));
    return MPPI_OK;
}
}

extern "C" {

void mppi_config_init(mppi_config* cfg) {
    if (!cfg) return;
    memset(cfg, 0, sizeof(*cfg));
    cfg->param_gamma = NAN;
    cfg->arm = mppi_arm_params{1.0, 1.0, 1.0, 1.0, 0.5, 0.5, 9.81, 1.0, 1.0};
}

const char* mppi_last_error(void) { return mppi_host::last_error(); }

int mppi_ctx_create(const mppi_config* cfg, int device, void* stream, mppi_ctx** out) {
    if (!cfg || !out) return fail(MPPI_E_ARG, "null argument");
    *out = nullptr;
    if (cfg->T < 1 || cfg->T > MPPI_MAX_T) return fail(MPPI_E_ARG, "T must be in [1, 128]");
    if (int rc = mppi_host::check_sample_geometry(cfg->K_local, cfg->K_total, cfg->k_offset)) return rc;
    if (cfg->clamp_mode < 0 || cfg->clamp_mode > 2) return fail(MPPI_E_ARG, "clamp_mode must be 0, 1 or 2");
    if (cfg->clamp_mode > 0)
        for (int d = 0; d < 2; ++d) {
            if (isnan(cfg->u_min[d])) return fail(MPPI_E_ARG, "u_min: a limit is NaN (use -inf for no limit)");
            if (isnan(cfg->u_max[d])) return fail(MPPI_E_ARG, "u_max: a limit is NaN (use +inf for no limit)");
            if (cfg->u_min[d] > cfg->u_max[d]) return fail(MPPI_E_ARG, "u_min[d] > u_max[d]: the limits are crossed");
        }
    const double* S = cfg->sigma;
    const double det = S[0] * S[3] - S[1] * S[2];
    if (det == 0.0 || !isfinite(det)) return fail(MPPI_E_SINGULAR, "Singular matrix");
    auto c = std::make_unique<mppi_ctx>();
    c->cfg = *cfg;
    c->device = device;
    c->stream = (hipStream_t)stream;
    c->sig_inv[0] = S[3] / det;
    c->sig_inv[1] = -S[1] / det;
    c->sig_inv[2] = -S[2] / det;
    c->sig_inv[3] = S[0] / det;
    int lps = cfg->lanes_per_sample > 0 ? cfg->lanes_per_sample : auto_lps(cfg->K_local);
    if (lps != 1 && lps != 2 && lps != 4 && lps != 8 && lps != 16)
        return fail(MPPI_E_ARG, "lanes_per_sample must be 0, 1, 2, 4, 8 or 16");
    c->lps = lps;
    const long long lanes = (long long)cfg->K_local * lps;
    c->nt = lanes >= 512LL * 256 ? 512 : 256;
    if (const char* ev = getenv("MPPI_BLOCK")) c->nt = atoi(ev) == 512 ? 512 : 256;
    if (2 * cfg->T + 1 > c->nt) c->nt = 512;
    c->nblocks = (int)((lanes + c->nt - 1) / c->nt);
    if (c->nblocks > 1024 * 1024) return fail(MPPI_E_ARG, "too many samples");
    const mppi_arm_params& a = cfg->arm;
    KConst& k = c->kc;
    memset(&k, 0, sizeof(k));
    mppi_host::set_common_consts(k, *cfg, c->nblocks);
    k.dt = (float)cfg->delta_t;
    k.fk1 = (float)a.fk_l1;
    k.fk2 = (float)a.fk_l2;
    k.A = (float)(a.m1 * a.lc1 * a.lc1 + a.l1 + a.m2 * (a.l1 * a.l1 + a.lc2 * a.lc2) + a.l2);
    k.B = (float)(2.0 * a.m2 * a.l1 * a.lc2);
    k.D = (float)(a.m2 * a.lc2 * a.lc2 + a.l2);
    k.E = (float)(a.m2 * a.l1 * a.lc2);
    k.P = (float)((a.m1 * a.lc1 + a.m2 * a.l1) * a.g);
    k.Q = (float)(a.m2 * a.lc2 * a.g);
    for (int i = 0; i < 4; ++i) {
        k.sw[i] = (float)(cfg->stage_cost_weight[i] * 10000.0);
        k.tw[i] = (float)(cfg->terminal_cost_weight[i] * 10000.0);
    }
    for (int i = 0; i < 4; ++i) k.sig_inv[i] = c->sig_inv[i];
    ClampK& ck = c->ck;
    ck.mode = cfg->clamp_mode;
    for (int d = 0; d < 2; ++d) {
        ck.u_lo[d] = cfg->clamp_mode ? cfg->u_min[d] : -INFINITY;
        ck.u_hi[d] = cfg->clamp_mode ? cfg->u_max[d] : INFINITY;
        ck.v_lo[d] = (float)ck.u_lo[d];
        ck.v_hi[d] = (float)ck.u_hi[d];
    }

    for (int j = 0; j < MPPI_MAX_OBSTACLES; ++j) c->ok.r2[j] = -1.f;

    if (int rc = alloc(c.get())) return rc;
    *out = c.release();
    return MPPI_OK;
}

void mppi_ctx_destroy(mppi_ctx* c) {
    if (!c) return;
    if (c->stream) (void)hipStreamSynchronize(c->stream);
    (void)hipDeviceSynchronize();
    delete c;
}

int mppi_set_stream(mppi_ctx* c, void* stream) {
    if (!c) return fail(MPPI_E_ARG, "null context");
    c->stream = (hipStream_t)stream;
    return MPPI_OK;
}

int mppi_ctx_info(const mppi_ctx* c, int* lps, int* blocks, int* threads) {
    if (!c) return fail(MPPI_E_ARG, "null context");
    if (lps) *lps = c->lps;
    if (blocks) *blocks = c->nblocks;
    if (threads) *threads = c->nt;
    return MPPI_OK;
}

}

namespace {

int stage_inputs(mppi_ctx* c, const double* x0, const double* window, int W, const double* u, bool skip_same) {
    if (!x0 || !window) return fail(MPPI_E_ARG, "null argument");
    if (W < 1 || W > MPPI_SEARCH_LEN) return fail(MPPI_E_ARG, "window rows must be in [1, 30]");
    StepStatic& h = c->stat;
    mppi_host::stage_window(window, W, h.win, h.key, &h.ctr);
    h.x0 = make_float4((float)x0[0], (float)x0[1], (float)x0[2], (float)x0[3]);
    if (!u) return MPPI_OK;
    const int T = c->cfg.T;
    if (skip_same && c->nominal_published && !memcmp(u, c->h_dout + 4, 2 * (size_t)T * sizeof(double)))
        return MPPI_OK;
    if (c->stage_pending) HIP_TRY(hipEventSynchronize(c->staged));
    DevStep* d = c->h_step;
    const KConst& k = c->kc;
    for (int t = 0; t < T; ++t) {
        const double u0 = u[2 * t], u1 = u[2 * t + 1];
        const double g0 = k.gamma * u0, g1 = k.gamma * u1;
        const double a0 = g0 * k.sig_inv[0] + g1 * k.sig_inv[2];
        const double a1 = g0 * k.sig_inv[1] + g1 * k.sig_inv[3];
        d->ua[t] = make_float4((float)u0, (float)u1, (float)a0, (float)a1);
        d->u[t][0] = u0;
        d->u[t][1] = u1;
    }
    HIP_TRY(hipMemcpyAsync(c->d_step + c->cur, d, sizeof(DevStep), hipMemcpyHostToDevice, c->stream));
    HIP_TRY(hipEventRecord(c->staged, c->stream));
    c->stage_pending = true;
    c->nominal_published = false;
    c->upd_valid = false;
    return MPPI_OK;
}

int launch_rollout(mppi_ctx* c, const float* noise_dev, double* S_dev, double* partial_dev, unsigned flags,
                   HostOut ho);

HostOut next_host_out(mppi_ctx* c, unsigned flags) {
    if (!(flags & MPPI_FLAG_HOST_OUT)) return HostOut{nullptr, 0u};
    if (++c->dseq == 0) ++c->dseq;
    return HostOut{c->h_dout.dev, c->dseq};
}

int wait_host_out(mppi_ctx* c) {
    if (c->dseq == 0) return fail(MPPI_E_ARG, "no MPPI_FLAG_HOST_OUT launch to wait for");
    const unsigned seq = c->dseq;
    volatile unsigned* flag = reinterpret_cast<volatile unsigned*>(c->h_dout.h);
    const auto t0 = std::chrono::steady_clock::now();
    for (unsigned long long n = 0; __atomic_load_n(flag, __ATOMIC_ACQUIRE) != seq; ++n) {
        if ((n & 1023) == 1023) {
            const hipError_t e = hipStreamQuery(c->stream);
            if (e != hipSuccess && e != hipErrorNotReady)
                return fail(MPPI_E_HIP, std::string("fused step: ") + hipGetErrorString(e));
            if (e == hipSuccess && __atomic_load_n(flag, __ATOMIC_ACQUIRE) != seq)
                return fail(MPPI_E_HIP, "fused step finished without publishing its outputs");
            if (std::chrono::steady_clock::now() - t0 > std::chrono::seconds(30))
                return fail(MPPI_E_HIP, "fused step: no result after 30 s");
        }
        __builtin_ia32_pause();
    }
    c->stage_pending = false;
    if (int rc = check_timeout(c)) return rc;
    c->nominal_published = true;
    c->x_flipped = false;
    return MPPI_OK;
}

void host_F(const mppi_arm_params& a, double dt, double* x, double u1, double u2) {
    const double q1 = x[0], q2 = x[1], dq1 = x[2], dq2 = x[3];
    double s2, c2;
    sincos(q2, &s2, &c2);
    const double M11 = a.m1 * a.lc1 * a.lc1 + a.l1 + a.m2 * (a.l1 * a.l1 + a.lc2 * a.lc2 + 2 * a.l1 * a.lc2 * c2) + a.l2;
    const double M22 = a.m2 * a.lc2 * a.lc2 + a.l2;
    const double M12 = a.m2 * a.l1 * a.lc2 * c2 + a.m2 * a.lc2 * a.lc2 + a.l2;
    const double h = a.m2 * a.l1 * a.lc2 * s2;
    const double c1 = cos(q1), c12 = cos(q1 + q2);
    const double g1 = a.m1 * a.lc1 * a.g * c1 + a.m2 * a.g * (a.lc2 * c12 + a.l1 * c1);
    const double g2 = a.m2 * a.lc2 * a.g * c12;
    const double r1 = u1 - ((-h * dq2) * dq1 + (-h * dq1 - h * dq2) * dq2) - g1;
    const double r2 = u2 - ((h * dq1) * dq1 + 0.0 * dq2) - g2;
    const double det = M11 * M22 - M12 * M12;
    const double ddq1 = (M22 * r1 - M12 * r2) / det;
    const double ddq2 = (-M12 * r1 + M11 * r2) / det;
    x[2] = dq1 + ddq1 * dt;
    x[3] = dq2 + ddq2 * dt;
    x[0] = q1 + x[2] * dt;
    x[1] = q2 + x[3] * dt;
}

void launch_traj(mppi_ctx* c, int blocks, const float2* base, int bstride, const float2* noise, int K, float4* out) {
    const bool cl = c->ck.mode != 0;
    auto* f = noise ? (cl ? traj_kernel<true, true> : traj_kernel<true, false>)
                    : (cl ? traj_kernel<false, true> : traj_kernel<false, false>);
    hipLaunchKernelGGL(f, dim3(blocks), dim3(kThreads), 0, c->stream, c->kc, c->stat, base, bstride, noise, K, out,
                       c->ck);
}

}

extern "C" {

int mppi_set_step_inputs(mppi_ctx* c, const double* x0, const double* window, int W, const double* u) {
    if (!c) return fail(MPPI_E_ARG, "null argument");
    return stage_inputs(c, x0, window, W, u, false);
}

int mppi_rollout(mppi_ctx* c, const float* noise_dev, double* S_dev, double* partial_dev, unsigned flags) {
    if (!c || !noise_dev) return fail(MPPI_E_ARG, "null argument");
    if ((flags & MPPI_FLAG_HOST_OUT) && !(flags & MPPI_FLAG_FUSED_UPDATE))
        return fail(MPPI_E_ARG, "MPPI_FLAG_HOST_OUT needs MPPI_FLAG_FUSED_UPDATE");
    return launch_rollout(c, noise_dev, S_dev, partial_dev, flags, next_host_out(c, flags));
}

}

namespace {
int launch_rollout(mppi_ctx* c, const float* noise_dev, double* S_dev, double* partial_dev, unsigned flags,
                   HostOut ho) {
    if ((flags & MPPI_FLAG_FUSED_UPDATE) && c->cfg.T < 5)
        return fail(MPPI_E_ARG, "device median filter needs T >= 5 (use the host update)");
    if (flags & MPPI_FLAG_EXCHANGE) {
        if (c->ex.xd.world < 1) return fail(MPPI_E_ARG, "MPPI_FLAG_EXCHANGE before mppi_exchange_attach");
        if (partial_dev) return fail(MPPI_E_ARG, "MPPI_FLAG_EXCHANGE merges on device: no partial_out");
        partial_dev = c->ex.d_xrow;
    }
    const DevStep* cur = c->d_step + c->cur;
    DevStep* nxt = c->d_step + (c->cur ^ 1);
    const float2* nz = reinterpret_cast<const float2*>(noise_dev);
    with_rollout(c, c->hand.poll, [&](auto lps, auto nt, auto p, auto cl, auto ob) {
        hipLaunchKernelGGL((rollout_kernel<lps, nt, p, cl, ob>), dim3(c->nblocks), dim3(nt), 0, c->stream, c->kc, c->stat, cur,
                           nz, S_dev, c->hand.d_slab, c->hand.d_gslab, c->hand.d_counter, partial_dev, c->d_weps, nxt,
                           flags, c->ex.xd, c->hand.d_epoch, c->hand.h_tmo.dev, reinterpret_cast<float*>(c->d_upd.h),
                           ho, c->d_dbg, c->ck, c->ok);
    });
    const int rc = launch_check("rollout_kernel");
    if (took_update(c, rc, flags)) c->x_flipped = (flags & MPPI_FLAG_EXCHANGE) != 0;
    return rc;
}
}

extern "C" {

int mppi_exchange_handle(mppi_ctx* c, int world, void* handle_out) {
    if (!c || !handle_out || world < 1 || world > kMaxWorld) return fail(MPPI_E_ARG, "bad argument");
    return c->ex.handle(c->device, 2 + 2 * c->cfg.T, world, handle_out);
}

int mppi_exchange_attach(mppi_ctx* c, int rank, int world, const void* handles) {
    if (!c || !handles || world < 1 || rank < 0 || rank >= world) return fail(MPPI_E_ARG, "bad argument");
    if (!c->ex.d_inbox || c->ex.world_alloc != world) return fail(MPPI_E_ARG, "call mppi_exchange_handle(world) first");
    return c->ex.attach(c->device, rank, world, handles);
}

int mppi_merge_partials(mppi_ctx* c, const double* partials_dev, int n, unsigned flags) {
    if (!c || !partials_dev || n < 1) return fail(MPPI_E_ARG, "bad argument");
    if ((flags & MPPI_FLAG_FUSED_UPDATE) && c->cfg.T < 5)
        return fail(MPPI_E_ARG, "device median filter needs T >= 5 (use the host update)");
    if ((flags & MPPI_FLAG_HOST_OUT) && !(flags & MPPI_FLAG_FUSED_UPDATE))
        return fail(MPPI_E_ARG, "MPPI_FLAG_HOST_OUT needs MPPI_FLAG_FUSED_UPDATE");
    const DevStep* cur = c->d_step + c->cur;
    DevStep* nxt = c->d_step + (c->cur ^ 1);
    const HostOut ho = next_host_out(c, flags);
    const bool big = 2 * c->cfg.T + 1 > 256, cl = c->ck.mode != 0;
    auto* f = big ? (cl ? merge_kernel<512, true> : merge_kernel<512, false>)
                  : (cl ? merge_kernel<256, true> : merge_kernel<256, false>);
    hipLaunchKernelGGL(f, dim3(1), dim3(big ? 512 : 256), 0, c->stream, c->kc, partials_dev, n, c->d_weps, cur, nxt,
                       flags, reinterpret_cast<float*>(c->d_upd.h), ho, c->ck);
    const int rc = launch_check("merge_kernel");
    took_update(c, rc, flags);
    return rc;
}

int mppi_get_weighted_noise(mppi_ctx* c, double* w_eps_host) {
    if (!c || !w_eps_host) return fail(MPPI_E_ARG, "null argument");
    const size_t bytes = 2 * (size_t)c->cfg.T * sizeof(double);
    HIP_TRY(hipMemcpyAsync(c->h_buf, c->d_weps, bytes, hipMemcpyDeviceToHost, c->stream));
    HIP_TRY(hipStreamSynchronize(c->stream));
    memcpy(w_eps_host, c->h_buf, bytes);
    return check_timeout(c);
}

int mppi_get_nominal(mppi_ctx* c, double* u_host) {
    if (!c || !u_host) return fail(MPPI_E_ARG, "null argument");
    const size_t bytes = 2 * (size_t)c->cfg.T * sizeof(double);
    HIP_TRY(hipMemcpyAsync(c->h_buf, (const char*)(c->d_step + c->cur) + offsetof(DevStep, u), bytes,
                           hipMemcpyDeviceToHost, c->stream));
    HIP_TRY(hipStreamSynchronize(c->stream));
    memcpy(u_host, c->h_buf, bytes);
    return MPPI_OK;
}

int mppi_rollout_traj(mppi_ctx* c, const double* base_u, const float* noise_dev, int K, float* out_dev) {
    if (!c || !out_dev || K < 1 || K > c->cfg.K_local) return fail(MPPI_E_ARG, "bad argument");
    const DevStep* cur = c->d_step + c->cur;
    const float2* base;
    int bstride = 1;
    if (base_u) {
        HIP_TRY(hipEventSynchronize(c->staged));
        for (int t = 0; t < c->cfg.T; ++t) c->h_base[t] = make_float2((float)base_u[2 * t], (float)base_u[2 * t + 1]);
        HIP_TRY(hipMemcpyAsync(c->d_base, c->h_base, c->cfg.T * sizeof(float2), hipMemcpyHostToDevice, c->stream));
        HIP_TRY(hipEventRecord(c->staged, c->stream));
        base = c->d_base;
    } else {
        base = reinterpret_cast<const float2*>(reinterpret_cast<const char*>(cur) + offsetof(DevStep, ua));
        bstride = 2;
    }
    const int blocks = (K + kThreads - 1) / kThreads;
    launch_traj(c, blocks, base, bstride, reinterpret_cast<const float2*>(noise_dev), K, reinterpret_cast<float4*>(out_dev));
    return launch_check("traj_kernel");
}

int mppi_optimal_traj(mppi_ctx* c, float* out_dev) {
    if (!c || !out_dev) return fail(MPPI_E_ARG, "null argument");
    if (!c->upd_valid) return fail(MPPI_E_ARG, "mppi_optimal_traj needs a preceding MPPI_FLAG_FUSED_UPDATE launch");
    launch_traj(c, 1, c->d_upd, 1, nullptr, 1, reinterpret_cast<float4*>(out_dev));
    return launch_check("traj_kernel");
}

int mppi_get_step_outputs(mppi_ctx* c, double* u_host, const float* traj_dev, float* traj_host) {
    if (!c || !u_host || (traj_dev && !traj_host)) return fail(MPPI_E_ARG, "bad argument");
    const int T = c->cfg.T;
    const size_t ub = 2 * (size_t)T * sizeof(double), tb = 4 * (size_t)T * sizeof(float);
    float* h_traj = reinterpret_cast<float*>(c->h_out + 2 * kMaxT);
    HIP_TRY(hipMemcpyAsync(c->h_out, (const char*)(c->d_step + c->cur) + offsetof(DevStep, u), ub,
                           hipMemcpyDeviceToHost, c->stream));
    if (traj_dev) HIP_TRY(hipMemcpyAsync(h_traj, traj_dev, tb, hipMemcpyDeviceToHost, c->stream));
    HIP_TRY(hipStreamSynchronize(c->stream));
    memcpy(u_host, c->h_out, ub);
    if (traj_dev) memcpy(traj_host, h_traj, tb);
    return check_timeout(c);
}

int mppi_optimal_traj_host(const mppi_ctx* c, const double* x0, const double* u_new, double* traj_out) {
    if (!c || !x0 || !u_new || !traj_out) return fail(MPPI_E_ARG, "null argument");
    const int T = c->cfg.T;
    double x[4] = {x0[0], x0[1], x0[2], x0[3]};
    const ClampK& k = c->ck;
    for (int t = 0; t < T; ++t) {
        const double* ut = u_new + 2 * (t == 0 ? T - 1 : t - 1);
        double u0 = ut[0], u1 = ut[1];
        if (k.mode >= 1) {
            u0 = clamp_u(u0, k.u_lo[0], k.u_hi[0]);
            u1 = clamp_u(u1, k.u_lo[1], k.u_hi[1]);
        }
        host_F(c->cfg.arm, c->cfg.delta_t, x, u0, u1);
        memcpy(traj_out + 4 * t, x, sizeof(x));
    }
    return MPPI_OK;
}

int mppi_wait_outputs(mppi_ctx* c, const double* x0, double* u_out, double* traj_out) {
    if (!c || !u_out || (traj_out && !x0)) return fail(MPPI_E_ARG, "bad argument");
    if (int rc = wait_host_out(c)) return rc;
    const int T = c->cfg.T;
    memcpy(u_out, c->h_dout + 4, 2 * (size_t)T * sizeof(double));
    if (traj_out) {
        double un[2 * kMaxT];
        un[0] = c->h_dout[2];
        un[1] = c->h_dout[3];
        memcpy(un + 2, c->h_dout + 4, 2 * (size_t)(T - 1) * sizeof(double));
        return mppi_optimal_traj_host(c, x0, un, traj_out);
    }
    return MPPI_OK;
}

}

namespace {
int dropin_launch(mppi_ctx* c, const double* x0, const double* window, int W, const double* u, const float* noise_dev,
                  double* S_dev, float* next_noise_dev, unsigned long long seed, unsigned long long next_step) {
    if (!c || !x0 || !window || !noise_dev) return fail(MPPI_E_ARG, "null argument");
    if (c->cfg.T < 5) return fail(MPPI_E_ARG, "device median filter needs T >= 5 (use the host update)");
    using clk = std::chrono::steady_clock;
    const auto t0 = c->in_tick ? c->tick_t0 : clk::now();
    c->in_tick = false;
    c->step_t0 = t0;
    auto mark = [&](int i) { c->dropin_us[i] = std::chrono::duration<double, std::micro>(clk::now() - t0).count(); };
    if (int rc = stage_inputs(c, x0, window, W, u, true)) return rc;
    mark(0);
    const unsigned fl = MPPI_FLAG_FUSED_UPDATE | MPPI_FLAG_HOST_OUT | (c->ex.xd.world >= 1 ? MPPI_FLAG_EXCHANGE : 0u);
    if (int rc = launch_rollout(c, noise_dev, S_dev, nullptr, fl, next_host_out(c, fl))) return rc;
    mark(1);
    if (next_noise_dev)
        if (int rc = mppi_noise_philox(c, seed, next_step, next_noise_dev)) return rc;
    mark(2);
    return MPPI_OK;
}

int dropin_finish(mppi_ctx* c, const double* x0, double* u_out, double* traj_out) {
    if (!u_out) return fail(MPPI_E_ARG, "null argument");
    using clk = std::chrono::steady_clock;
    auto mark = [&](int i) {
        c->dropin_us[i] = std::chrono::duration<double, std::micro>(clk::now() - c->step_t0).count();
    };
    if (int rc = wait_host_out(c)) return rc;
    mark(3);
    if (int rc = mppi_wait_outputs(c, x0, u_out, traj_out)) return rc;
    mark(4);
    return MPPI_OK;
}
}

extern "C" {

int mppi_step_dropin(mppi_ctx* c, const double* x0, const double* window, int W, const double* u,
                     const float* noise_dev, double* S_dev, float* next_noise_dev, unsigned long long seed,
                     unsigned long long next_step, double* u_out, double* traj_out) {
    if (!u_out) return fail(MPPI_E_ARG, "null argument");
    if (int rc = dropin_launch(c, x0, window, W, u, noise_dev, S_dev, next_noise_dev, seed, next_step)) return rc;
    return dropin_finish(c, x0, u_out, traj_out);
}

int mppi_dropin_bind(mppi_ctx* c, const mppi_dropin_binding* b) {
    if (!c || !b) return fail(MPPI_E_ARG, "null argument");
    if (!b->path || b->rows < 1 || b->stride < 4 || !b->x0 || !b->idx || !b->u || !b->noise_dev)
        return fail(MPPI_E_ARG, "binding: path (rows >= 1, stride >= 4), x0, idx, u and noise_dev are required");
    c->bind = *b;
    c->bound = true;
    return MPPI_OK;
}

int mppi_dropin_tick(mppi_ctx* c, unsigned long long next_step) {
    if (int rc = mppi_dropin_tick_launch(c, next_step)) return rc;
    return mppi_dropin_tick_wait(c);
}

int mppi_dropin_tick_wait(mppi_ctx* c) {
    if (!c) return fail(MPPI_E_ARG, "null context");
    if (!c->tick_launched) return fail(MPPI_E_ARG, "mppi_dropin_tick_wait without a launched tick");
    c->tick_launched = false;
    return dropin_finish(c, c->bind.x0, c->bind.u, c->bind.traj);
}

int mppi_dropin_tick_launch(mppi_ctx* c, unsigned long long next_step) {
    if (!c) return fail(MPPI_E_ARG, "null context");
    if (!c->bound) return fail(MPPI_E_ARG, "mppi_dropin_tick before mppi_dropin_bind");
    if (c->tick_launched) return fail(MPPI_E_ARG, "a launched tick was not waited for (mppi_dropin_tick_wait)");
    const mppi_dropin_binding& b = c->bind;
    c->tick_t0 = std::chrono::steady_clock::now();
    c->in_tick = true;
    const double q1 = b.x0[0], q2 = b.x0[1];
    const double x = b.fk_l1 * cos(q1) + b.fk_l2 * cos(q1 + q2);
    const double y = b.fk_l1 * sin(q1) + b.fk_l2 * sin(q1 + q2);
    const long long prev = b.idx[0];
    if (prev < 0 || prev >= b.rows) {
        c->in_tick = false;
        return fail(MPPI_E_ARG, "prev_waypoints_idx outside ref_path");
    }
    const int n = (int)std::min<long long>(MPPI_SEARCH_LEN, b.rows - prev);
    int best = 0;
    double dmin = 0.0;
    for (int j = 0; j < n; ++j) {
        const double* r = b.path + (prev + j) * (long long)b.stride;
        const double dx = x - r[0], dy = y - r[1];
        const double d = (dx * dx + dy * dy) * 100;
        if (j == 0 || d < dmin) {
            dmin = d;
            best = j;
        }
    }
    const long long idx = prev + best;
    b.idx[1] = prev;
    b.idx[0] = idx;
    if (idx >= b.rows - 1) {
        c->in_tick = false;
        return fail(MPPI_E_PATH_END, "Reached the end of the reference path.");
    }
    const int W = (int)std::min<long long>(MPPI_SEARCH_LEN, b.rows - idx);
    double win[4 * MPPI_SEARCH_LEN];
    for (int j = 0; j < W; ++j) memcpy(win + 4 * j, b.path + (idx + j) * (long long)b.stride, 4 * sizeof(double));
    const int rc = dropin_launch(c, b.x0, win, W, b.u, b.noise_dev, b.S_dev, b.next_noise_dev, b.seed, next_step);
    c->tick_launched = rc == MPPI_OK;
    return rc;
}

int mppi_noise_philox(mppi_ctx* c, unsigned long long seed, unsigned long long step, float* out_dev) {
    if (!c || !out_dev) return fail(MPPI_E_ARG, "null argument");
    const double* S = c->cfg.sigma;
    const double s01 = 0.5 * (S[1] + S[2]);
    if (!(S[0] > 0.0)) return fail(MPPI_E_ARG, "Sigma not positive definite");
    const double L00 = sqrt(S[0]), L10 = s01 / L00, d = S[3] - L10 * L10;
    if (!(d >= 0.0)) return fail(MPPI_E_ARG, "Sigma not positive semi-definite");
    const double L11 = sqrt(d);
    constexpr double bm = kBoxMullerScale;
    const dim3 grid((unsigned)((c->cfg.K_local + kThreads - 1) / kThreads), (unsigned)((c->cfg.T + 1) / 2));
    hipLaunchKernelGGL(philox_noise_kernel, grid, dim3(kThreads), 0, c->stream, c->cfg.K_local,
                       c->cfg.T, (long long)c->cfg.k_offset, seed, step, (float)(L00 * bm), (float)(L10 * bm), (float)(L11 * bm),
                       reinterpret_cast<float2*>(out_dev));
    return launch_check("philox_noise_kernel");
}

int mppi_debug_set_buffer(mppi_ctx* c, void* dbg_dev) {
    if (!c) return fail(MPPI_E_ARG, "null context");
    c->d_dbg = (unsigned long long*)dbg_dev;
    return MPPI_OK;
}

int mppi_debug_nearest(mppi_ctx* c, const float* noise_dev, int K, int* slot_dev, float* pos_dev) {
    if (!c || !noise_dev || !slot_dev || !pos_dev || K < 1 || K > c->cfg.K_local) return fail(MPPI_E_ARG, "bad argument");
    hipLaunchKernelGGL(nearest_debug_kernel, dim3((K + kThreads - 1) / kThreads), dim3(kThreads), 0, c->stream, c->kc,
                       c->stat, c->d_step + c->cur, reinterpret_cast<const float2*>(noise_dev), K, slot_dev,
                       reinterpret_cast<float2*>(pos_dev), c->ck);
    return launch_check("nearest_debug_kernel");
}

int mppi_set_obstacles(mppi_ctx* c, int n, const double* discs, double cost) {
    if (!c) return fail(MPPI_E_ARG, "null context");
    if (n < 0 || n > MPPI_MAX_OBSTACLES) return fail(MPPI_E_ARG, "obstacles: n must be in [0, 8]");
    if (n > 0 && !discs) return fail(MPPI_E_ARG, "obstacles: null discs");
    if (!(cost >= 0.0) || isinf(cost)) return fail(MPPI_E_ARG, "obstacles: the cost must be finite and >= 0");
    ObstK k{};
    for (int j = 0; j < MPPI_MAX_OBSTACLES; ++j) k.r2[j] = -1.f;
    for (int j = 0; j < n; ++j) {
        const double cx = discs[3 * j], cy = discs[3 * j + 1], r = discs[3 * j + 2];
        if (!isfinite((float)cx) || !isfinite((float)cy)) return fail(MPPI_E_ARG, "obstacles: a centre is not finite");
        if (!(r >= 0.0)) return fail(MPPI_E_ARG, "obstacles: a radius is NaN or negative");
        k.cx[j] = (float)cx;
        k.cy[j] = (float)cy;
        k.r2[j] = (float)(r * r);
    }
    k.w = cost;
    k.n = n;
    c->ok = k;
    return MPPI_OK;
}

int mppi_debug_obstacle_hits(mppi_ctx* c, const float* noise_dev, int K, unsigned* mask_dev, float* dir_dev) {
    if (!c || !noise_dev || !mask_dev || !dir_dev || K < 1 || K > c->cfg.K_local) return fail(MPPI_E_ARG, "bad argument");
    hipLaunchKernelGGL(obstacle_debug_kernel, dim3((K + kThreads - 1) / kThreads), dim3(kThreads), 0, c->stream, c->kc,
                       c->stat, c->d_step + c->cur, reinterpret_cast<const float2*>(noise_dev), K, mask_dev,
                       reinterpret_cast<float4*>(dir_dev), c->ck, c->ok);
    return launch_check("obstacle_debug_kernel");
}

int mppi_debug_dropin_times(const mppi_ctx* c, double* us_out) {
    if (!c || !us_out) return fail(MPPI_E_ARG, "null argument");
    memcpy(us_out, c->dropin_us, 5 * sizeof(double));
    return MPPI_OK;
}

int mppi_sync(mppi_ctx* c) {
    if (!c) return fail(MPPI_E_ARG, "null context");
    HIP_TRY(hipStreamSynchronize(c->stream));
    return check_timeout(c);
}

int mppi_ctx_handoff(const mppi_ctx* c, int* poll) {
    if (!c || !poll) return fail(MPPI_E_ARG, "null argument");
    *poll = c->hand.poll ? 1 : 0;
    return MPPI_OK;
}

}
```

### mppi_robotarm_amd/engine.py

```python
from __future__ import annotations

import ctypes as C
import math

import numpy as np
import torch

from . import _native as N
from .params import ArmParams


def _raw_stream(index: int) -> int:
    get = getattr(torch._C, "_cuda_getCurrentRawStream", None)
    return get(index) if get is not None else torch.cuda.current_stream(index).cuda_stream


def _dptr(a: np.ndarray):
    return a.ctypes.data_as(C.POINTER(C.c_double))


class _Engine:

    CALLS = ("ctx_create", "ctx_destroy", "set_stream", "set_step_inputs", "rollout", "merge_partials",
             "exchange_handle", "exchange_attach", "get_weighted_noise", "get_nominal", "rollout_traj",
             "wait_outputs", "optimal_traj_host", "noise_philox", "sync")
    WAIT_FOLLOWS_STREAM = False

    def __init__(self, prefix: str, dim_u: int, dim_x: int, cfg, K_local: int, T: int, K_total: int | None,
                 k_offset: int, device: int | torch.device | None):
        self._lib = N.load()
        self._prefix, self.dim_u, self.dim_x = prefix, int(dim_u), int(dim_x)
        for name in self.CALLS:
            setattr(self, "_c_" + name, getattr(self._lib, prefix + name))
        if device is None:
            device = torch.cuda.current_device()
        self.device = torch.device("cuda", device if isinstance(device, int) else device.index)
        self.K_local, self.T = int(K_local), int(T)
        self.K_total = int(K_total if K_total is not None else K_local)
        self.k_offset = int(k_offset)
        cfg.K_local, cfg.T, cfg.K_total, cfg.k_offset = self.K_local, self.T, self.K_total, self.k_offset
        with torch.cuda.device(self.device):
            self.stream = torch.cuda.current_stream(self.device)
            ctx = C.c_void_p()
            N.check(self._c_ctx_create(C.byref(cfg), self.device.index, C.c_void_p(self.stream.cuda_stream),
                                       C.byref(ctx)), prefix + "ctx_create")
        self._ctx = ctx
        self.partial_len = 2 + self.dim_u * self.T

    @staticmethod
    def clamp_mode(u_min, u_max, clamp_nominal: bool) -> int:
        if u_min is None and u_max is None:
            return 0
        return 2 if clamp_nominal else 1

    def _set_limits(self, cfg, dim_u: int, u_min, u_max, clamp_nominal: bool) -> None:
        cfg.clamp_mode = self.clamp_mode(u_min, u_max, clamp_nominal)
        if cfg.clamp_mode:
            lo = np.broadcast_to(np.asarray(-np.inf if u_min is None else u_min, dtype=np.float64), (dim_u,))
            hi = np.broadcast_to(np.asarray(np.inf if u_max is None else u_max, dtype=np.float64), (dim_u,))
            for d in range(dim_u):
                cfg.u_min[d], cfg.u_max[d] = float(lo[d]), float(hi[d])
        self.u_min = None if not cfg.clamp_mode else np.array(cfg.u_min[:dim_u])
        self.u_max = None if not cfg.clamp_mode else np.array(cfg.u_max[:dim_u])

    def close(self) -> None:
        if getattr(self, "_ctx", None):
            self._c_ctx_destroy(self._ctx)
            self._ctx = None
        self._noise_stage = None

    def __del__(self):
        try:
            self.close()
        except Exception:
            pass

    def _sync_stream(self):
        if _raw_stream(self.device.index) == self.stream.cuda_stream:
            return
        s = torch.cuda.current_stream(self.device)
        if s.cuda_stream != self.stream.cuda_stream:
            s.wait_stream(self.stream)
            self.stream = s
            N.check(self._c_set_stream(self._ctx, C.c_void_p(s.cuda_stream)), self._prefix + "set_stream")

    def new_noise(self) -> torch.Tensor:
        return torch.empty((self.T, self.K_local, self.dim_u), dtype=torch.float32, device=self.device)

    def new_partial(self) -> torch.Tensor:
        return torch.empty(self.partial_len, dtype=torch.float64, device=self.device)

    def upload_noise(self, eps_kt: np.ndarray, out: torch.Tensor | None = None) -> torch.Tensor:
        out = self.new_noise() if out is None else out
        eps = np.ascontiguousarray(eps_kt, dtype=np.float64)
        stage = getattr(self, "_noise_stage", None)
        if stage is None or tuple(stage.shape) != eps.shape:
            stage = self._noise_stage = torch.empty(eps.shape, dtype=torch.float64, device=self.device)
        stage.copy_(torch.from_numpy(eps))
        out.copy_(stage.permute(1, 0, 2))
        return out

    def upload_std_noise(self, noise, z: torch.Tensor, out: torch.Tensor) -> torch.Event:
        self._sync_stream()
        K, T, du = noise.z.shape
        lo, kl = self.k_offset, self.K_local
        zz = z[:K * T * du].view(K, T, du)[lo:lo + kl]
        stage = getattr(self, "_noise_stage", None)
        if stage is None or tuple(stage.shape) != (kl, T, du):
            stage = self._noise_stage = torch.empty((kl, T, du), dtype=torch.float64, device=self.device)
        stage.copy_(zz, non_blocking=True)
        ev = torch.cuda.Event()
        ev.record(self.stream)
        key = (noise.src.tobytes(), noise.scale.tobytes(), noise.mean.tobytes())
        if getattr(self, "_std_key", None) != key:
            self._std_key = key
            self._std_t = (torch.from_numpy(noise.src).to(self.device), torch.from_numpy(noise.scale).to(self.device),
                           torch.from_numpy(noise.mean).to(self.device),
                           bool(np.array_equal(noise.src, np.arange(du))))
        src, scale, mean, ident = self._std_t
        x = stage if ident else stage.index_select(2, src)
        x = torch.mul(x, scale)
        x.add_(mean)
        out.copy_(x.permute(1, 0, 2))
        return ev

    def set_step_inputs(self, x0, window, u=None) -> None:
        self._sync_stream()
        x0 = np.ascontiguousarray(np.asarray(x0, dtype=np.float64).ravel()[:self.dim_x])
        win = np.ascontiguousarray(np.asarray(window, dtype=np.float64)[:, :4])
        if win.ndim != 2 or win.shape[0] < 1 or win.shape[0] > N.MPPI_SEARCH_LEN:
            raise ValueError("window must have 1..30 rows of [x, y, dq1, dq2]")
        uu = None
        if u is not None:
            uu = np.ascontiguousarray(np.asarray(u, dtype=np.float64).reshape(self.T, self.dim_u))
        N.check(self._c_set_step_inputs(self._ctx, _dptr(x0), _dptr(win), win.shape[0],
                                        _dptr(uu) if uu is not None else None),
                self._prefix + "set_step_inputs")
        self._keep = (x0, win, uu)

    def exchange_handle(self, world: int) -> bytes:
        buf = C.create_string_buffer(N.MPPI_IPC_HANDLE_BYTES)
        N.check(self._c_exchange_handle(self._ctx, int(world), buf), self._prefix + "exchange_handle")
        return buf.raw

    def exchange_attach(self, rank: int, world: int, handles) -> None:
        blob = b"".join(bytes(h) for h in handles)
        if len(blob) != world * N.MPPI_IPC_HANDLE_BYTES:
            raise ValueError("one 64-byte handle per rank")
        N.check(self._c_exchange_attach(self._ctx, int(rank), int(world), C.create_string_buffer(blob, len(blob))),
                self._prefix + "exchange_attach")
        self.exchange_world = int(world)

    def rollout(self, noise: torch.Tensor, S_out: torch.Tensor | None = None,
                partial_out: torch.Tensor | None = None, fused_update: bool = False, exchange: bool = False,
                host_out: bool = False) -> None:
        self._sync_stream()
        self._check_noise(noise)
        if S_out is not None:
            assert S_out.dtype == torch.float64 and S_out.numel() >= self.K_local and S_out.device == self.device
        if partial_out is not None:
            assert partial_out.dtype == torch.float64 and partial_out.numel() >= self.partial_len
        N.check(self._c_rollout(self._ctx, C.c_void_p(noise.data_ptr()),
                                C.c_void_p(S_out.data_ptr()) if S_out is not None else None,
                                C.c_void_p(partial_out.data_ptr()) if partial_out is not None else None,
                                (N.MPPI_FLAG_FUSED_UPDATE if fused_update else 0)
                                | (N.MPPI_FLAG_EXCHANGE if exchange else 0)
                                | (N.MPPI_FLAG_HOST_OUT if host_out else 0)),
                self._prefix + "rollout")

    def merge(self, partials: torch.Tensor, n: int, fused_update: bool = False, flags: int = 0) -> None:
        self._sync_stream()
        assert partials.dtype == torch.float64 and partials.is_contiguous()
        assert partials.numel() >= n * self.partial_len
        N.check(self._c_merge_partials(self._ctx, C.c_void_p(partials.data_ptr()), int(n),
                                       (N.MPPI_FLAG_FUSED_UPDATE if fused_update else 0) | flags),
                self._prefix + "merge_partials")

    def wait_outputs(self, x0=None):
        if self.WAIT_FOLLOWS_STREAM:
            self._sync_stream()
        u_out = np.empty((self.T, self.dim_u))
        traj = None
        xp = None
        if x0 is not None:
            x = np.ascontiguousarray(np.asarray(x0, dtype=np.float64).ravel()[:self.dim_x])
            traj = np.empty((self.T, self.dim_x))
            xp = _dptr(x)
        N.check(self._c_wait_outputs(self._ctx, xp, _dptr(u_out), _dptr(traj) if traj is not None else None),
                self._prefix + "wait_outputs")
        return u_out, traj

    def weighted_noise(self) -> np.ndarray:
        self._sync_stream()
        out = np.zeros((self.T, self.dim_u))
        N.check(self._c_get_weighted_noise(self._ctx, _dptr(out)), self._prefix + "get_weighted_noise")
        return out

    def nominal(self) -> np.ndarray:
        self._sync_stream()
        out = np.zeros((self.T, self.dim_u))
        N.check(self._c_get_nominal(self._ctx, _dptr(out)), self._prefix + "get_nominal")
        return out

    def trajectories(self, base_u=None, noise: torch.Tensor | None = None, K: int | None = None) -> torch.Tensor:
        self._sync_stream()
        K = self.K_local if K is None else int(K)
        out = torch.empty((K, self.T, self.dim_x), dtype=torch.float32, device=self.device)
        bu = None
        if base_u is not None:
            bu = np.ascontiguousarray(np.asarray(base_u, dtype=np.float64).reshape(self.T, self.dim_u))
        if noise is not None:
            self._check_noise(noise)
        N.check(self._c_rollout_traj(self._ctx, _dptr(bu) if bu is not None else None,
                                     C.c_void_p(noise.data_ptr()) if noise is not None else None,
                                     K, C.c_void_p(out.data_ptr())),
                self._prefix + "rollout_traj")
        self._keep_traj = bu
        return out

    def optimal_traj_host(self, x0, u_new) -> np.ndarray:
        x = np.ascontiguousarray(np.asarray(x0, dtype=np.float64).ravel()[:self.dim_x])
        un = np.ascontiguousarray(np.asarray(u_new, dtype=np.float64).reshape(self.T, self.dim_u))
        out = np.empty((self.T, self.dim_x))
        N.check(self._c_optimal_traj_host(self._ctx, _dptr(x), _dptr(un), _dptr(out)),
                self._prefix + "optimal_traj_host")
        return out

    def philox_noise(self, seed: int, step: int = 0, out: torch.Tensor | None = None) -> torch.Tensor:
        self._sync_stream()
        out = self.new_noise() if out is None else out
        self._check_noise(out)
        N.check(self._c_noise_philox(self._ctx, int(seed) & (2 ** 64 - 1), int(step) & (2 ** 64 - 1),
                                     C.c_void_p(out.data_ptr())), self._prefix + "noise_philox")
        return out

    def synchronize(self) -> None:
        N.check(self._c_sync(self._ctx), self._prefix + "sync")

    def _check_noise(self, noise: torch.Tensor) -> None:
        shape = (self.T, self.K_local, self.dim_u)
        if (noise.dtype != torch.float32 or not noise.is_contiguous() or noise.device != self.device
                or tuple(noise.shape) != shape):
            raise ValueError(f"noise must be a contiguous fp32 {shape} tensor on {self.device}")


class RolloutEngine(_Engine):

    def __init__(self, K_local: int, T: int, delta_t: float, param_lambda: float, param_alpha: float,
                 sigma, stage_cost_weight, terminal_cost_weight, param_exploration: float = 0.0,
                 arm: ArmParams = ArmParams(), K_total: int | None = None, k_offset: int = 0,
                 device: int | torch.device | None = None, lanes_per_sample: int = 0,
                 param_gamma: float | None = None, u_min=None, u_max=None, clamp_nominal: bool = True):
        cfg = N.ConfigC()
        self._set_limits(cfg, 2, u_min, u_max, clamp_nominal)
        cfg.delta_t = float(delta_t)
        cfg.param_lambda = float(param_lambda)
        cfg.param_alpha = float(param_alpha)
        cfg.param_exploration = float(param_exploration)
        sig = np.asarray(sigma, dtype=np.float64).reshape(2, 2)
        for i, v in enumerate(sig.ravel()):
            cfg.sigma[i] = float(v)
        for i in range(4):
            cfg.stage_cost_weight[i] = float(stage_cost_weight[i])
            cfg.terminal_cost_weight[i] = float(terminal_cost_weight[i])
        for f in ("m1", "m2", "l1", "l2", "lc1", "lc2", "g", "fk_l1", "fk_l2"):
            setattr(cfg.arm, f, float(getattr(arm, f)))
        cfg.lanes_per_sample = int(lanes_per_sample)
        cfg.param_gamma = float("nan") if param_gamma is None else float(param_gamma)
        self.sigma = sig
        self.param_lambda = float(param_lambda)
        super().__init__("mppi_", 2, 4, cfg, K_local, T, K_total, k_offset, device)
        lps, blocks, threads = C.c_int(), C.c_int(), C.c_int()
        N.check(self._lib.mppi_ctx_info(self._ctx, C.byref(lps), C.byref(blocks), C.byref(threads)), "mppi_ctx_info")
        self.lanes_per_sample, self.blocks, self.threads = lps.value, blocks.value, threads.value
        poll = C.c_int()
        N.check(self._lib.mppi_ctx_handoff(self._ctx, C.byref(poll)), "mppi_ctx_handoff")
        self.handoff = "poll" if poll.value else "counter"
        self.obstacles, self.obstacle_cost = np.zeros((0, 3)), 0.0

    def merge(self, partials: torch.Tensor, n: int, fused_update: bool = False, host_out: bool = False) -> None:
        super().merge(partials, n, fused_update, N.MPPI_FLAG_HOST_OUT if host_out else 0)

    @staticmethod
    def check_obstacles(discs, cost) -> tuple[np.ndarray, float]:
        try:
            a = np.zeros((0, 3)) if discs is None else np.array(discs, dtype=np.float64, ndmin=1)
            w = float(cost)
        except (TypeError, ValueError) as e:
            raise ValueError(f"obstacles: {e}") from None
        if a.size == 0:
            a = np.zeros((0, 3))
        if a.ndim != 2 or a.shape[1] != 3:
            raise ValueError(f"obstacles must be (n, 3) rows of (cx, cy, r), got shape {a.shape}")
        if a.shape[0] > N.MPPI_MAX_OBSTACLES:
            raise ValueError(f"at most {N.MPPI_MAX_OBSTACLES} obstacles, got {a.shape[0]}")
        if not np.all(np.isfinite(a[:, :2].astype(np.float32))):
            raise ValueError("obstacles: a centre is not finite")
        if not np.all(a[:, 2] >= 0.0):
            raise ValueError("obstacles: a radius is NaN or negative")
        if not (w >= 0.0 and math.isfinite(w)):
            raise ValueError("obstacle_cost must be finite and >= 0")
        return np.ascontiguousarray(a), w

    def set_obstacles(self, discs, cost: float = 1.0e10) -> None:
        a, w = self.check_obstacles(discs, cost)
        N.check(self._lib.mppi_set_obstacles(self._ctx, a.shape[0], _dptr(a) if a.shape[0] else None, w),
                "mppi_set_obstacles")
        self.obstacles, self.obstacle_cost = a, w

    def obstacle_hits(self, noise: torch.Tensor, K: int | None = None) -> tuple[np.ndarray, np.ndarray]:
        self._sync_stream()
        self._check_noise(noise)
        K = self.K_local if K is None else int(K)
        mask = torch.zeros((K, self.T), dtype=torch.int32, device=self.device)
        d = torch.empty((K, self.T, 4), dtype=torch.float32, device=self.device)
        N.check(self._lib.mppi_debug_obstacle_hits(self._ctx, C.c_void_p(noise.data_ptr()), K,
                                                   C.c_void_p(mask.data_ptr()), C.c_void_p(d.data_ptr())),
                "mppi_debug_obstacle_hits")
        self.synchronize()
        return mask.cpu().numpy().view(np.uint32), d.cpu().numpy()

    def optimal_traj(self, out: torch.Tensor | None = None) -> torch.Tensor:
        self._sync_stream()
        out = torch.empty((self.T, 4), dtype=torch.float32, device=self.device) if out is None else out
        N.check(self._lib.mppi_optimal_traj(self._ctx, C.c_void_p(out.data_ptr())), "mppi_optimal_traj")
        return out

    def step_outputs(self, traj: torch.Tensor | None = None):
        self._sync_stream()
        u = np.zeros((self.T, 2))
        tr = np.zeros((self.T, 4), dtype=np.float32) if traj is not None else None
        N.check(self._lib.mppi_get_step_outputs(self._ctx, _dptr(u),
                                                C.c_void_p(traj.data_ptr()) if traj is not None else None,
                                                tr.ctypes.data_as(C.c_void_p) if tr is not None else None),
                "mppi_get_step_outputs")
        return u, tr

    def step_dropin(self, x0, window, u, noise: torch.Tensor, S_out: torch.Tensor | None = None,
                    next_noise: torch.Tensor | None = None, seed: int = 0, next_step: int = 0,
                    want_traj: bool = True):
        self._sync_stream()
        x = np.ascontiguousarray(x0, dtype=np.float64)
        if x.shape != (4,):
            x = np.ascontiguousarray(x.ravel()[:4])
        win = window
        if not (isinstance(win, np.ndarray) and win.dtype == np.float64 and win.ndim == 2 and win.shape[1] == 4
                and win.flags.c_contiguous):
            win = np.ascontiguousarray(np.asarray(window, dtype=np.float64)[:, :4])
        if not 1 <= win.shape[0] <= N.MPPI_SEARCH_LEN:
            raise ValueError("window must have 1..30 rows of [x, y, dq1, dq2]")
        uu = None if u is None else np.ascontiguousarray(u, dtype=np.float64)
        if uu is not None and uu.shape != (self.T, 2):
            raise ValueError(f"u must be ({self.T}, 2)")
        if noise.data_ptr() != getattr(self, "_checked_noise", 0):
            self._check_noise(noise)
            self._checked_noise = noise.data_ptr()
        if getattr(self, "_u_out", None) is None:
            self._u_out = np.empty((self.T, 2))
        traj = np.empty((self.T, 4)) if want_traj else None
        N.check(self._lib.mppi_step_dropin(
            self._ctx, x.ctypes.data, win.ctypes.data, win.shape[0], uu.ctypes.data if uu is not None else None,
            noise.data_ptr(), S_out.data_ptr() if S_out is not None else None,
            next_noise.data_ptr() if next_noise is not None else None, seed & 0xFFFFFFFFFFFFFFFF,
            next_step & 0xFFFFFFFFFFFFFFFF,
            self._u_out.ctypes.data, traj.ctypes.data if traj is not None else None), "mppi_step_dropin")
        return self._u_out, traj

    def dropin_bind(self, path: np.ndarray, fk_l1: float, fk_l2: float, x_buf: np.ndarray, idx_buf: np.ndarray,
                    u: np.ndarray, traj_buf: np.ndarray | None, noise: torch.Tensor,
                    next_noise: torch.Tensor | None, S_out: torch.Tensor | None, seed: int) -> None:
        self._check_noise(noise)
        if next_noise is not None:
            self._check_noise(next_noise)
        b = N.DropinBindingC()
        b.path, b.rows, b.stride = path.ctypes.data, path.shape[0], path.strides[0] // 8
        b.fk_l1, b.fk_l2 = float(fk_l1), float(fk_l2)
        b.x0, b.idx, b.u = x_buf.ctypes.data, idx_buf.ctypes.data, u.ctypes.data
        b.traj = traj_buf.ctypes.data if traj_buf is not None else None
        b.noise_dev = noise.data_ptr()
        b.next_noise_dev = next_noise.data_ptr() if next_noise is not None else None
        b.S_dev = S_out.data_ptr() if S_out is not None else None
        b.seed = int(seed) & 0xFFFFFFFFFFFFFFFF
        N.check(self._lib.mppi_dropin_bind(self._ctx, C.byref(b)), "mppi_dropin_bind")

    def dropin_tick(self, next_step: int) -> int:
        self._sync_stream()
        rc = self._lib.mppi_dropin_tick(self._ctx, next_step)
        if rc != N.MPPI_OK and rc != N.MPPI_E_PATH_END:
            N.check(rc, "mppi_dropin_tick")
        return rc

    def dropin_tick_launch(self, next_step: int) -> int:
        self._sync_stream()
        rc = self._lib.mppi_dropin_tick_launch(self._ctx, next_step)
        if rc != N.MPPI_OK and rc != N.MPPI_E_PATH_END:
            N.check(rc, "mppi_dropin_tick_launch")
        return rc

    def dropin_tick_wait(self) -> None:
        N.check(self._lib.mppi_dropin_tick_wait(self._ctx), "mppi_dropin_tick_wait")

    def dropin_times(self) -> np.ndarray:
        out = np.zeros(5)
        N.check(self._lib.mppi_debug_dropin_times(self._ctx, _dptr(out)), "mppi_debug_dropin_times")
        return out

    def nearest_slots(self, noise: torch.Tensor, K: int | None = None) -> tuple[np.ndarray, np.ndarray]:
        self._sync_stream()
        self._check_noise(noise)
        K = self.K_local if K is None else int(K)
        slot = torch.empty((K, self.T), dtype=torch.int32, device=self.device)
        pos = torch.empty((K, self.T, 2), dtype=torch.float32, device=self.device)
        N.check(self._lib.mppi_debug_nearest(self._ctx, C.c_void_p(noise.data_ptr()), K,
                                             C.c_void_p(slot.data_ptr()), C.c_void_p(pos.data_ptr())),
                "mppi_debug_nearest")
        self.synchronize()
        return slot.cpu().numpy(), pos.cpu().numpy()


def readback_workers() -> int:
    import os
    env = os.environ.get("MPPI_READBACK_WORKERS")
    if env:
        return max(1, min(64, int(env)))
    n = len(os.sched_getaffinity(0)) if hasattr(os, "sched_getaffinity") else (os.cpu_count() or 1)
    omp = os.environ.get("OMP_NUM_THREADS", "")
    if omp.isdigit() and int(omp) > 0:
        n = min(n, int(omp))
    return max(1, min(16, n))


class HostReadback:

    CHUNK = 1 << 20
    SLOTS = 8
    STREAMS = 2

    def __init__(self, device: torch.device, workers: int | None = None, chunk: int | None = None,
                 slots: int | None = None, streams: int | None = None):
        self._lib = N.load()
        self.device = device
        self.workers = readback_workers() if workers is None else int(workers)
        self.chunk = self.CHUNK if chunk is None else int(chunk)
        self.slots = self.SLOTS if slots is None else int(slots)
        self.streams = self.STREAMS if streams is None else int(streams)
        rb = C.c_void_p()
        with torch.cuda.device(device):
            N.check(self._lib.mppi_readback_create(device.index, self.workers, self.slots, self.chunk, self.streams,
                                                   C.byref(rb)), "mppi_readback_create")
        self._rb = rb

    def run(self, src: torch.Tensor, dst: np.ndarray) -> np.ndarray:
        if not (src.dtype == torch.float32 and src.is_contiguous() and src.device == self.device
                and dst.dtype == np.float64 and dst.flags.c_contiguous and dst.flags.writeable
                and dst.size == src.numel()):
            raise ValueError("HostReadback.run: a contiguous fp32 device tensor into a writable C-contiguous "
                             "fp64 array of the same size")
        N.check(self._lib.mppi_readback_run(self._rb, C.c_void_p(_raw_stream(self.device.index)),
                                            C.c_void_p(src.data_ptr()), C.c_void_p(dst.ctypes.data), src.numel()),
                "mppi_readback_run")
        return dst

    def close(self) -> None:
        if getattr(self, "_rb", None):
            self._lib.mppi_readback_destroy(self._rb)
            self._rb = None

    def __del__(self):
        try:
            self.close()
        except Exception:
            pass


class NpDeviceStream:

    def __init__(self, device: torch.device):
        from . import hostrng
        self._lib = N.load()
        self.device = device
        params = hostrng.log_params()
        if params is None:
            raise RuntimeError("the device NumPy draw needs libm's log constants (hostrng.log_params)")
        self._params = params
        ctx = C.c_void_p()
        with torch.cuda.device(device):
            N.check(self._lib.mppi_np_ctx_create(device.index, params.ctypes.data, C.byref(ctx)), "mppi_np_ctx_create")
        self._ctx = ctx
        self._jumps = (0, 0)
        self._st = N.NpStateC()
        self._st_ref = C.byref(self._st)
        self._key_addr = C.addressof(self._st.key)
        self._P, self._ns = C.c_int(), C.c_int()
        self._P_ref, self._ns_ref = C.byref(self._P), C.byref(self._ns)
        self._targets = {}
        self.draws = 0
        self.retries = 0

    def close(self) -> None:
        if getattr(self, "_ctx", None):
            self._lib.mppi_np_ctx_destroy(self._ctx)
            self._ctx = None

    def __del__(self):
        try:
            self.close()
        except Exception:
            pass

    def draw(self, state, shape, plan, out: torch.Tensor, stream, k_offset: int, K_local: int, strides) -> None:
        K, T, du = shape
        n = K * T * du
        pos, has_gauss = int(state[2]), int(state[3])
        N.check(self._lib.mppi_np_plan(self._ctx, n, pos, has_gauss, self._P_ref, self._ns_ref), "mppi_np_plan")
        P, ns = self._P.value, self._ns.value
        if self._jumps[0] != P or self._jumps[1] < ns:
            from . import hostrng
            polys = hostrng.jump_polys(P, ns)
            if polys is None:
                raise RuntimeError("MT19937 jump polynomials unavailable")
            polys = np.ascontiguousarray(polys)
            N.check(self._lib.mppi_np_set_jumps(self._ctx, P, ns, polys.ctypes.data if polys.size else None,
                                                N.NP_POLY_WORDS), "mppi_np_set_jumps")
            self._jumps = (P, ns)
        st = self._st
        key = state[1]
        if not (isinstance(key, np.ndarray) and key.dtype == np.uint32 and key.flags.c_contiguous and key.size == 624):
            key = np.ascontiguousarray(key, dtype=np.uint32)
        C.memmove(self._key_addr, key.ctypes.data, 624 * 4)
        st.pos, st.has_gauss, st.gauss = pos, has_gauss, float(state[4])
        ck = (K, T, du, out.data_ptr(), int(k_offset), int(K_local), tuple(int(x) for x in strides))
        hit = self._targets.get(ck)
        if hit is None or hit[0] is not plan:
            t = N.NpTargetC()
            t.out_dev = out.data_ptr()
            t.K, t.T, t.du, t.k_offset, t.K_local = K, T, du, int(k_offset), int(K_local)
            t.stride_t, t.stride_k, t.stride_d = ck[6]
            src, scale, mean = plan[:3]
            for d in range(du):
                t.src[d], t.scale[d], t.mean[d] = int(src[d]), float(scale[d]), float(mean[d])
            mat = plan[4] if len(plan) > 4 else None
            t.dot2 = 0 if mat is None else 1
            if mat is not None:
                for i, v in enumerate(np.asarray(mat, dtype=np.float64).ravel()):
                    t.mat[i] = float(v)
            if len(self._targets) >= 8:
                self._targets.clear()
            hit = (plan, t, C.byref(t))
            self._targets[ck] = hit
        N.check(self._lib.mppi_np_draw(self._ctx, C.c_void_p(stream), self._st_ref, n, hit[2]), "mppi_np_draw")
        self.draws += 1

    def result(self):
        st = self._st
        rc = self._lib.mppi_np_draw_result(self._ctx, C.byref(st))
        if rc == N.MPPI_E_RETRY:
            self.retries += 1
            return None
        N.check(rc, "mppi_np_draw_result")
        key = np.frombuffer(st.key, dtype=np.uint32).copy()
        return ("MT19937", key, st.pos, st.has_gauss, st.gauss)


def exploit_count(param_exploration: float, K: int) -> int:
    thr = (1.0 - param_exploration) * K
    return 0 if thr <= 0 else min(K, int(math.ceil(thr)))
```

Before: 157.1 billion.

## Defer cross-block merge and nominal update into the next rollout launch

When a rollout runs with only the fused-update flag, each block writes its row and per-block minimum into a double-buffered slab and returns without the last-block hand-off merge. The merge and nominal update for that step run at the start of the next rollout launch, which reads the previous slab and rebuilds the control table in shared memory, so the serial tail of each step is removed. A finalize kernel and finalize_pending calls on every accessor keep outputs correct when results are read. In exchange, every block redundantly repeats the merge work at launch start, only block 0 stores the result, and the extra per-block minima plus the ping-pong slab add state and complexity.

```diff
diff --git a/include/mppi_rocm.h b/include/mppi_rocm.h
--- a/include/mppi_rocm.h
+++ b/include/mppi_rocm.h
@@ -19,6 +19,7 @@
 #define MPPI_FLAG_FUSED_UPDATE 1u
 #define MPPI_FLAG_EXCHANGE 2u
 #define MPPI_FLAG_HOST_OUT 4u
+#define MPPI_FLAG_INLINE_MERGE 8u
 #define MPPI_IPC_HANDLE_BYTES 64
 #define MPPI_MAX_WORLD 8
 
@@ -58,6 +59,8 @@
 int mppi_ctx_info(const mppi_ctx *ctx, int *lanes_per_sample, int *blocks, int *threads_per_block);
 
 int mppi_ctx_handoff(const mppi_ctx *ctx, int *poll);
+
+int mppi_debug_pending(const mppi_ctx *ctx, int *pending);
 
 int mppi_set_step_inputs(mppi_ctx *ctx, const double *x0, const double *window, int W,
                          const double *u);
diff --git a/mppi_robotarm_amd/_native.py b/mppi_robotarm_amd/_native.py
--- a/mppi_robotarm_amd/_native.py
+++ b/mppi_robotarm_amd/_native.py
@@ -18,6 +18,7 @@
 MPPI_FLAG_FUSED_UPDATE = 1
 MPPI_FLAG_EXCHANGE = 2
 MPPI_FLAG_HOST_OUT = 4
+MPPI_FLAG_INLINE_MERGE = 8
 DP = C.POINTER(C.c_double)
 MPPI_IPC_HANDLE_BYTES = 64
 MPPI_MAX_WORLD = 8
@@ -31,7 +32,7 @@
     "mppi_optimal_traj_host", "mppi_wait_outputs", "mppi_dropin_bind", "mppi_dropin_tick",
     "mppi_dropin_tick_launch", "mppi_dropin_tick_wait",
     "mppi_noise_philox",
-    "mppi_sync", "mppi_debug_set_buffer",
+    "mppi_sync", "mppi_debug_set_buffer", "mppi_debug_pending",
     "mppi_debug_nearest", "mppi_debug_dropin_times", "mppi_set_obstacles", "mppi_debug_obstacle_hits",
     "mppi_chain_ctx_create", "mppi_chain_ctx_destroy", "mppi_chain_set_stream", "mppi_chain_ctx_info",
     "mppi_chain_set_step_inputs", "mppi_chain_rollout", "mppi_chain_merge_partials", "mppi_chain_exchange_handle",
@@ -139,6 +140,7 @@
         "mppi_set_stream": ([vp, vp], C.c_int),
         "mppi_ctx_info": ([vp, ip, ip, ip], C.c_int),
         "mppi_ctx_handoff": ([vp, ip], C.c_int),
+        "mppi_debug_pending": ([vp, ip], C.c_int),
         "mppi_set_step_inputs": ([vp, dp, dp, C.c_int, dp], C.c_int),
         "mppi_rollout": ([vp, fp, vp, vp, C.c_uint], C.c_int),
         "mppi_merge_partials": ([vp, vp, C.c_int, C.c_uint], C.c_int),
diff --git a/mppi_robotarm_amd/csrc/mppi_device.h b/mppi_robotarm_amd/csrc/mppi_device.h
--- a/mppi_robotarm_amd/csrc/mppi_device.h
+++ b/mppi_robotarm_amd/csrc/mppi_device.h
@@ -289,6 +289,9 @@
 }
 __device__ __forceinline__ double ld_wt(__amdgpu_buffer_rsrc_t r, int idx) {
     return __builtin_bit_cast(double, __builtin_amdgcn_raw_buffer_load_b64(r, idx * 8, 0, kSC1));
+}
+__device__ __forceinline__ double ld_prev(__amdgpu_buffer_rsrc_t r, int idx) {
+    return __builtin_bit_cast(double, __builtin_amdgcn_raw_buffer_load_b64(r, idx * 8, 0, 0));
 }
 __device__ __forceinline__ void st_wt(__amdgpu_buffer_rsrc_t r, int idx, double v) {
     __builtin_amdgcn_raw_buffer_store_b64(__builtin_bit_cast(u32x2, v), r, idx * 8, 0, kSC1);
@@ -522,11 +525,14 @@
     }
 }
 
-template <int NT, int MAXCH, bool GRAN, class SM>
+template <int NT, int MAXCH, bool GRAN, bool PRE = false, class SM>
 __device__ __forceinline__ bool direct_merge(__amdgpu_buffer_rsrc_t rows, int n, const RowGeo& geo,
                                              double inv_lambda, SM& sm, double* out_row, double* w_eps_out,
-                                             unsigned tag, unsigned* tmo, unsigned long long* dbg = nullptr) {
+                                             unsigned tag, unsigned* tmo, unsigned long long* dbg = nullptr,
+                                             const double* rho_pre = nullptr) {
     constexpr int P = kDirectRows / 64;
+    static_assert(!(PRE && GRAN), "granules are polled here");
+    auto ld = [](__amdgpu_buffer_rsrc_t r, int idx) { return PRE ? ld_prev(r, idx) : ld_wt(r, idx); };
     constexpr int LB = 16;
     constexpr int RB = LB / MAXCH;
     const int tid = threadIdx.x, lane = tid & 63;
@@ -553,6 +559,9 @@
         __syncthreads();
 #pragma unroll
         for (int j = 0; j < P; ++j) rho_l[j] = sm.rho[lane + 64 * j];
+    } else if constexpr (PRE) {
+#pragma unroll
+        for (int j = 0; j < P; ++j) rho_l[j] = rho_pre[j];
     } else {
 #pragma unroll
         for (int j = 0; j < P; ++j) {
@@ -624,12 +633,12 @@
 #pragma unroll
                 for (int j = 0; j < LB; ++j) v[j] = gran_val(gv[j]);
             } else {
-                if (b0 == 0) eta_k = ld_wt(rows, mine ? row * stride + 1 : kOffRange);
+                if (b0 == 0) eta_k = ld(rows, mine ? row * stride + 1 : kOffRange);
 #pragma unroll
                 for (int j = 0; j < LB; ++j) {
                     const int i = b0 + j / MAXCH, col = tid + (j % MAXCH) * NT;
-                    v[j] = ld_wt(rows, (i < nrel && col < ncol) ? __builtin_amdgcn_readlane(row, i) * stride + 1 + col
-                                                                 : kOffRange);
+                    v[j] = ld(rows, (i < nrel && col < ncol) ? __builtin_amdgcn_readlane(row, i) * stride + 1 + col
+                                                              : kOffRange);
                 }
             }
 #pragma unroll
@@ -674,7 +683,7 @@
                 for (int j = 0; j < LB; ++j) v[j] = gran_val(gv[j]);
             } else {
 #pragma unroll
-                for (int j = 0; j < LB; ++j) v[j] = ld_wt(rows, roff[j]);
+                for (int j = 0; j < LB; ++j) v[j] = ld(rows, roff[j]);
             }
 #pragma unroll
             for (int j = 0; j < LB; ++j)
@@ -815,6 +824,91 @@
     return true;
 }
 
+template <int NT, class SM>
+__device__ __forceinline__ void deferred_merge(__amdgpu_buffer_rsrc_t rows, int n, const RowGeo& geo, double inv_lambda,
+                                               SM& sm, int* l_row, double* w_eps_out) {
+    constexpr int P = kDirectRows / 64;
+    constexpr int LB = 32;
+    static_assert(kGroup == 16, "a group is one DPP row of lanes");
+    static_assert(kDirectRows / kGroup <= 16, "the group rows merge in one round in either hand-off form");
+    const int tid = threadIdx.x, lane = tid & 63;
+    const int stride = geo.stride, ncol = geo.ncol;
+    double rho_l[P];
+#pragma unroll
+    for (int j = 0; j < P; ++j) {
+        const int r = lane + 64 * j;
+        const double x = ld_prev(rows, r < n ? n * stride + r : kOffRange);
+        rho_l[j] = r < n ? x : INFINITY;
+    }
+    if (n > kGroup && direct_merge<NT, 1, false, true>(rows, n, geo, inv_lambda, sm, nullptr, w_eps_out, 0u, nullptr,
+                                                       nullptr, rho_l))
+        return;
+    double rho_g[P], m = INFINITY;
+#pragma unroll
+    for (int j = 0; j < P; ++j) {
+        double v = rho_l[j];
+        v = min_raw_f64(v, dpp_f64<0xB1>(v));
+        v = min_raw_f64(v, dpp_f64<0x4E>(v));
+        v = min_raw_f64(v, dpp_f64<0x141>(v));
+        v = min_raw_f64(v, dpp_f64<0x140>(v));
+        rho_g[j] = v;
+        m = min_raw_f64(m, v);
+    }
+    const double rho = wave_min_f64(m);
+    if (tid < 64) {
+        int base = 0;
+#pragma unroll
+        for (int j = 0; j < P; ++j) {
+            const bool in = lane + 64 * j < n;
+            const double s1 = exp((rho_g[j] - rho_l[j]) * inv_lambda);
+            const double s2 = exp((rho - rho_g[j]) * inv_lambda);
+            const bool need = in && s1 >= kMergeFloor && s2 >= kMergeFloor;
+            const unsigned long long bal = __ballot(need);
+            if (need) {
+                const int pos = base + lanes_below(bal);
+                l_row[pos] = lane + 64 * j;
+                sm.rho[pos] = s1;
+                sm.part[pos] = s2;
+            }
+            base += __popcll(bal);
+        }
+        if (lane == 0) sm.nrel = base;
+    }
+    __syncthreads();
+    const int nn = sm.nrel;
+    double acc = 0.0, accg = 0.0;
+    for (int b0 = 0; b0 < nn; b0 += LB) {
+        double v[LB];
+#pragma unroll
+        for (int j = 0; j < LB; ++j) {
+            const int i = b0 + j;
+            v[j] = ld_prev(rows, (i < nn && tid < ncol) ? l_row[i] * stride + 1 + tid : kOffRange);
+        }
+#pragma unroll
+        for (int j = 0; j < LB; ++j) {
+            const int i = b0 + j;
+            if (i < nn) {
+                accg = fma(sm.rho[i], v[j], accg);
+                if (i + 1 == nn || (l_row[i + 1] / kGroup) != (l_row[i] / kGroup)) {
+                    acc = fma(sm.part[i], accg, acc);
+                    accg = 0.0;
+                }
+            }
+        }
+    }
+    if (tid == 0) {
+        sm.eta = acc;
+        sm.rho_fin = rho;
+    }
+    __syncthreads();
+    if (tid >= 1 && tid < ncol) {
+        const double w = acc / sm.eta;
+        sm.weps[tid - 1] = w;
+        if (w_eps_out) w_eps_out[tid - 1] = w;
+    }
+    __syncthreads();
+}
+
 __device__ __forceinline__ double median10(double* v) {
 #define CX(i, j) { const double lo = min_raw_f64(v[i], v[j]), hi = max_raw_f64(v[i], v[j]); v[i] = lo; v[j] = hi; }
     CX(4, 9) CX(3, 8) CX(2, 7) CX(1, 6) CX(0, 5) CX(1, 4) CX(6, 9) CX(0, 3) CX(5, 8) CX(0, 2)
diff --git a/mppi_robotarm_amd/csrc/mppi_rocm.hip b/mppi_robotarm_amd/csrc/mppi_rocm.hip
--- a/mppi_robotarm_amd/csrc/mppi_rocm.hip
+++ b/mppi_robotarm_amd/csrc/mppi_rocm.hip
@@ -225,6 +225,10 @@
 
 using Scratch = MergeScratch<2 * kMaxT>;
 
+constexpr int kPF = 4;
+
+constexpr unsigned kFlagPending = 1u << 31;
+
 __device__ __forceinline__ double nominal_src(const DevStep* st, int tid, int T) {
     const int t = tid >> 1, src = t + 1 < T ? t + 1 : T - 1;
     return tid < 2 * T ? st->u[src][tid & 1] : 0.0;
@@ -240,11 +244,14 @@
 
 __host__ __device__ __forceinline__ double clamp_u(double u, double lo, double hi) { return u < lo ? lo : (u > hi ? hi : u); }
 
-template <int NT, bool CLAMP>
+template <int NT, bool CLAMP, bool DEFER = false>
 __device__ void nominal_update_block(DevStep* nxt, const KConst& c, Scratch& sm, double u_src, double u_first,
-                                     float* upd, HostOut ho, const ClampK& cl, bool publish = true) {
+                                     float* upd, HostOut ho, const ClampK& cl, bool publish = true,
+                                     float4* s_ua = nullptr, bool store = true) {
     const int tid = threadIdx.x;
     const int T = c.T;
+    if constexpr (!DEFER) store = true;
+    if (!store) upd = nullptr;
     if (tid < ((2 * T + 63) & ~63)) {
         const int t = tid >> 1, d = tid & 1;
         const int src = t + 1 < T ? t + 1 : T - 1;
@@ -262,13 +269,19 @@
         if (tid < 2 * T) {
             if (upd && t + 1 < T) upd[2 * (t + 1) + d] = (float)un;
             if (ho.p) ho.p[4 + tid] = un;
-            nxt->u[t][d] = un;
+            if (store) nxt->u[t][d] = un;
             if (d == 0) {
                 const double u0 = un, u1 = other;
                 const double g0 = c.gamma * u0, g1 = c.gamma * u1;
                 const double a0 = g0 * c.sig_inv[0] + g1 * c.sig_inv[2];
                 const double a1 = g0 * c.sig_inv[1] + g1 * c.sig_inv[3];
-                nxt->ua[t] = make_float4((float)u0, (float)u1, (float)a0, (float)a1);
+                const float4 row = make_float4((float)u0, (float)u1, (float)a0, (float)a1);
+                if (store) nxt->ua[t] = row;
+                if constexpr (DEFER) {
+                    s_ua[t] = row;
+                    if (t == T - 1)
+                        for (int p = 0; p < kPF; ++p) s_ua[T + p] = row;
+                }
             }
         }
     }
@@ -280,10 +293,20 @@
     }
 }
 
-
-constexpr int kPF = 4;
-
-template <int LPS, int NT, bool POLL, bool CLAMP, bool OBST>
+template <int NT, bool CLAMP>
+__device__ __forceinline__ void deferred_finish(const KConst& c, const double* rows, const DevStep* st, DevStep* nxt,
+                                                double* w_eps_out, float* upd, const ClampK& cl, Scratch& sm,
+                                                int* l_row, float4* s_ua, bool store) {
+    const int tid = threadIdx.x;
+    const double u_cur = nominal_src(st, tid, c.T), u_first = nominal_first(st, tid);
+    const RowGeo geo(2 * c.T);
+    deferred_merge<NT>(rows_rsrc(rows, c.nblocks * (geo.stride + 1) * 8), c.nblocks, geo, c.inv_lambda, sm, l_row,
+                       store ? w_eps_out : nullptr);
+    nominal_update_block<NT, CLAMP, true>(nxt, c, sm, u_cur, u_first, upd, HostOut{nullptr, 0u}, cl, false, s_ua, store);
+}
+
+
+template <int LPS, int NT, bool POLL, bool CLAMP, bool OBST, bool DEFER = false>
 __global__ __launch_bounds__(NT) void rollout_kernel(
     const KConst c, const StepStatic ss, const DevStep* __restrict__ st, const float2* __restrict__ noise,
     double* __restrict__ S_out, double* __restrict__ slab, double* __restrict__ gslab,
@@ -292,6 +315,8 @@
     float* __restrict__ upd, const HostOut ho, unsigned long long* __restrict__ dbg, const ClampK cl,
     const ObstK ob) {
     static_assert(CLAMP || !OBST, "the OBST kernels are built with CLAMP only");
+    static_assert(!DEFER || !POLL, "the deferred form leaves plain rows");
+    static_assert(!DEFER || NT >= kDirectRows, "s_k holds the deferred merge's row list");
     __shared__ float4 s_win[kSlots];
     __shared__ float4 s_ua[kMaxT + kPF];
     __shared__ double s_redd[NT / 64];
@@ -318,8 +343,14 @@
 #pragma unroll
     for (int j = 0; j < kPF; ++j) ring[j] = np[(size_t)(j < T ? j : T - 1) * K];
     const unsigned tag_v = POLL ? __hip_atomic_load(epoch, __ATOMIC_RELAXED, __HIP_MEMORY_SCOPE_AGENT) + 1u : 0u;
-    const double u_cur = (flags & MPPI_FLAG_FUSED_UPDATE) ? nominal_src(st, tid, T) : 0.0;
-    const double u_first = (flags & MPPI_FLAG_FUSED_UPDATE) ? nominal_first(st, tid) : 0.0;
+    const double u_cur = (!DEFER && (flags & MPPI_FLAG_FUSED_UPDATE)) ? nominal_src(st, tid, T) : 0.0;
+    const double u_first = (!DEFER && (flags & MPPI_FLAG_FUSED_UPDATE)) ? nominal_first(st, tid) : 0.0;
+    bool pending = false;
+    if constexpr (DEFER) {
+        pending = (flags & kFlagPending) != 0;
+        if (pending) deferred_finish<NT, CLAMP>(c, gslab, st, nxt, w_eps_out, upd, cl, sm, s_k, s_ua, blockIdx.x == 0);
+        STAMP(10, NOW());
+    }
     const float4 wrow = ss.win[tid & (kSlots - 1)];
     Search<LPS> sr;
     sr.load(ss.key, ss.ctr, tid & (LPS - 1));
@@ -335,7 +366,8 @@
     }
     int hits = 0;
     bool hit_last = false;
-    for (int i = tid; i < T + kPF; i += NT) s_ua[i] = st->ua[i < T ? i : T - 1];
+    if (!pending)
+        for (int i = tid; i < T + kPF; i += NT) s_ua[i] = st->ua[i < T ? i : T - 1];
     if (tid < kSlots) s_win[tid] = wrow;
     __syncthreads();
     float4 uring[kPF];
@@ -447,7 +479,7 @@
     const int nrows = c.nblocks;
     const int ngroups = (nrows + kGroup - 1) / kGroup;
     constexpr int kValBytes = POLL ? 16 : 8;
-    const __amdgpu_buffer_rsrc_t slab_r = rows_rsrc(slab, nrows * stride * kValBytes);
+    const __amdgpu_buffer_rsrc_t slab_r = rows_rsrc(slab, nrows * (stride + (DEFER ? 1 : 0)) * kValBytes);
     const __amdgpu_buffer_rsrc_t gslab_r = rows_rsrc(gslab, ngroups * stride * kValBytes);
     const unsigned tag = __builtin_amdgcn_readfirstlane(tag_v);
     auto publish = [&](int idx, double v) {
@@ -456,6 +488,8 @@
     };
     const double rho_b = block_min_f64<NT>(owner ? S : INFINITY, sm);
     if (tid == 0) publish(blockIdx.x * stride, rho_b);
+    if constexpr (DEFER)
+        if (tid == 0) publish(nrows * stride + blockIdx.x, rho_b);
     const LaneWeight lw = block_weigh(owner, S, rho_b, c.inv_lambda, lane, wave, s_cnt, s_redd);
     __syncthreads();
     double eta_b;
@@ -505,6 +539,7 @@
     }
     STAMP(2, NOW());
     STAMP(5, (unsigned long long)nl);
+    if constexpr (DEFER) return;
     if (!handoff_merge<NT, 1, POLL>(slab_r, gslab_r, nrows, geo, c.inv_lambda, sm, counters, c.acquire != 0, &s_flag,
                                     partial_out, w_eps_out, tag, epoch, tmo, dbg, dbg))
         return;
@@ -534,6 +569,15 @@
     merge_rows_block<NT, 1, true, false>(r, 0, n, RowGeo(2 * c.T), c.inv_lambda, sm, nullptr, 0, nullptr, w_eps_out,
                                          0u, nullptr);
     if (flags & MPPI_FLAG_FUSED_UPDATE) nominal_update_block<NT, CLAMP>(nxt, c, sm, u_cur, u_first, upd, ho, cl);
+}
+
+template <int NT, bool CLAMP>
+__global__ __launch_bounds__(NT) void finalize_kernel(const KConst c, const double* rows, const DevStep* cur,
+                                                      DevStep* nxt, double* w_eps_out, float* upd, const ClampK cl) {
+    __shared__ Scratch sm;
+    __shared__ int s_row[kDirectRows];
+    __shared__ float4 s_ua[kMaxT + kPF];
+    deferred_finish<NT, CLAMP>(c, rows, cur, nxt, w_eps_out, upd, cl, sm, s_row, s_ua, true);
 }
 
 constexpr int kTrajTB = 8;
@@ -686,6 +730,9 @@
     StepStatic stat{};
     mppi_host::DevBuf<DevStep> d_step;
     int cur = 0;
+    mppi_host::DevBuf<double> d_drows;
+    int drow = 0;
+    bool pending = false;
     mppi_host::PinnedBuf<DevStep> h_step;
     mppi_host::Event staged;
     bool stage_pending = false;
@@ -734,6 +781,33 @@
     });
 }
 
+bool capturing(const mppi_ctx* c) {
+    if (!c->stream) return false;
+    hipStreamCaptureStatus cs = hipStreamCaptureStatusNone;
+    if (hipStreamIsCapturing(c->stream, &cs) != hipSuccess) {
+        (void)hipGetLastError();
+        return false;
+    }
+    return cs != hipStreamCaptureStatusNone;
+}
+
+int finalize_pending(mppi_ctx* c) {
+    if (!c->pending) return MPPI_OK;
+    if (capturing(c))
+        return fail(MPPI_E_ARG, "a deferred fused step is pending on a capturing stream: call mppi_sync before the capture");
+    const size_t slab = (size_t)c->nblocks * (3 + 2 * c->cfg.T);
+    const bool big = c->nt == 512, cl = c->ck.mode != 0;
+    auto* f = big ? (cl ? finalize_kernel<512, true> : finalize_kernel<512, false>)
+                  : (cl ? finalize_kernel<256, true> : finalize_kernel<256, false>);
+    hipLaunchKernelGGL(f, dim3(1), dim3(c->nt), 0, c->stream, c->kc, c->d_drows + c->drow * slab,
+                       c->d_step + c->cur, c->d_step + (c->cur ^ 1), c->d_weps, reinterpret_cast<float*>(c->d_upd.h),
+                       c->ck);
+    if (int rc = launch_check("finalize_kernel")) return rc;
+    c->pending = false;
+    c->cur ^= 1;
+    return MPPI_OK;
+}
+
 bool took_update(mppi_ctx* c, int rc, unsigned flags) {
     if (rc != MPPI_OK || !(flags & MPPI_FLAG_FUSED_UPDATE)) return false;
     c->cur ^= 1;
@@ -774,6 +848,8 @@
     if (int rc = c->hand.setup(c->nblocks, ncu, per_cu, 2 + 2 * c->cfg.T, 0)) return rc;
     c->kc.acquire = c->hand.acquire;
     if (int rc = c->d_step.alloc_zeroed(2)) return rc;
+    if (c->nblocks <= kDirectRows)
+        if (int rc = c->d_drows.alloc_zeroed(2 * (size_t)c->nblocks * (3 + 2 * c->cfg.T))) return rc;
     if (int rc = c->d_weps.alloc_zeroed(2 * kMaxT)) return rc;
     if (int rc = c->d_base.alloc(kMaxT)) return rc;
     if (int rc = c->d_upd.alloc(kMaxT)) return rc;
@@ -870,6 +946,7 @@
 
 void mppi_ctx_destroy(mppi_ctx* c) {
     if (!c) return;
+    (void)finalize_pending(c);
     if (c->stream) (void)hipStreamSynchronize(c->stream);
     (void)hipDeviceSynchronize();
     delete c;
@@ -877,6 +954,8 @@
 
 int mppi_set_stream(mppi_ctx* c, void* stream) {
     if (!c) return fail(MPPI_E_ARG, "null context");
+    if (c->stream != (hipStream_t)stream)
+        if (int rc = finalize_pending(c)) return rc;
     c->stream = (hipStream_t)stream;
     return MPPI_OK;
 }
@@ -900,6 +979,7 @@
     mppi_host::stage_window(window, W, h.win, h.key, &h.ctr);
     h.x0 = make_float4((float)x0[0], (float)x0[1], (float)x0[2], (float)x0[3]);
     if (!u) return MPPI_OK;
+    if (int rc = finalize_pending(c)) return rc;
     const int T = c->cfg.T;
     if (skip_same && c->nominal_published && !memcmp(u, c->h_dout + 4, 2 * (size_t)T * sizeof(double)))
         return MPPI_OK;
@@ -1014,9 +1094,32 @@
         if (partial_dev) return fail(MPPI_E_ARG, "MPPI_FLAG_EXCHANGE merges on device: no partial_out");
         partial_dev = c->ex.d_xrow;
     }
+    const float2* nz = reinterpret_cast<const float2*>(noise_dev);
+    if (flags == MPPI_FLAG_FUSED_UPDATE && !partial_dev && c->d_drows && !capturing(c)) {
+        const size_t slab = (size_t)c->nblocks * (3 + 2 * c->cfg.T);
+        double* prev = c->d_drows + c->drow * slab;
+        double* mine = c->d_drows + (c->drow ^ 1) * slab;
+        const unsigned fl = flags | (c->pending ? kFlagPending : 0u);
+        with_rollout(c, false, [&](auto lps, auto nt, auto p, auto cl, auto ob) {
+            hipLaunchKernelGGL((rollout_kernel<lps, nt, false, cl, ob, true>), dim3(c->nblocks), dim3(nt), 0, c->stream,
+                               c->kc, c->stat, c->d_step + c->cur, nz, S_dev, mine, prev, nullptr, nullptr, c->d_weps,
+                               c->d_step + (c->cur ^ 1), fl, c->ex.xd, nullptr, nullptr,
+                               reinterpret_cast<float*>(c->d_upd.h), HostOut{nullptr, 0u}, c->d_dbg, c->ck, c->ok);
+        });
+        const int rc = launch_check("rollout_kernel");
+        if (rc != MPPI_OK) return rc;
+        if (c->pending) c->cur ^= 1;
+        c->drow ^= 1;
+        c->pending = true;
+        c->upd_valid = true;
+        c->nominal_published = false;
+        c->x_flipped = false;
+        return rc;
+    }
+    if (int rc = finalize_pending(c)) return rc;
+    flags &= ~MPPI_FLAG_INLINE_MERGE;
     const DevStep* cur = c->d_step + c->cur;
     DevStep* nxt = c->d_step + (c->cur ^ 1);
-    const float2* nz = reinterpret_cast<const float2*>(noise_dev);
     with_rollout(c, c->hand.poll, [&](auto lps, auto nt, auto p, auto cl, auto ob) {
         hipLaunchKernelGGL((rollout_kernel<lps, nt, p, cl, ob>), dim3(c->nblocks), dim3(nt), 0, c->stream, c->kc, c->stat, cur,
                            nz, S_dev, c->hand.d_slab, c->hand.d_gslab, c->hand.d_counter, partial_dev, c->d_weps, nxt,
@@ -1044,6 +1147,7 @@
 
 int mppi_merge_partials(mppi_ctx* c, const double* partials_dev, int n, unsigned flags) {
     if (!c || !partials_dev || n < 1) return fail(MPPI_E_ARG, "bad argument");
+    if (int rc = finalize_pending(c)) return rc;
     if ((flags & MPPI_FLAG_FUSED_UPDATE) && c->cfg.T < 5)
         return fail(MPPI_E_ARG, "device median filter needs T >= 5 (use the host update)");
     if ((flags & MPPI_FLAG_HOST_OUT) && !(flags & MPPI_FLAG_FUSED_UPDATE))
@@ -1063,6 +1167,7 @@
 
 int mppi_get_weighted_noise(mppi_ctx* c, double* w_eps_host) {
     if (!c || !w_eps_host) return fail(MPPI_E_ARG, "null argument");
+    if (int rc = finalize_pending(c)) return rc;
     const size_t bytes = 2 * (size_t)c->cfg.T * sizeof(double);
     HIP_TRY(hipMemcpyAsync(c->h_buf, c->d_weps, bytes, hipMemcpyDeviceToHost, c->stream));
     HIP_TRY(hipStreamSynchronize(c->stream));
@@ -1072,6 +1177,7 @@
 
 int mppi_get_nominal(mppi_ctx* c, double* u_host) {
     if (!c || !u_host) return fail(MPPI_E_ARG, "null argument");
+    if (int rc = finalize_pending(c)) return rc;
     const size_t bytes = 2 * (size_t)c->cfg.T * sizeof(double);
     HIP_TRY(hipMemcpyAsync(c->h_buf, (const char*)(c->d_step + c->cur) + offsetof(DevStep, u), bytes,
                            hipMemcpyDeviceToHost, c->stream));
@@ -1082,6 +1188,7 @@
 
 int mppi_rollout_traj(mppi_ctx* c, const double* base_u, const float* noise_dev, int K, float* out_dev) {
     if (!c || !out_dev || K < 1 || K > c->cfg.K_local) return fail(MPPI_E_ARG, "bad argument");
+    if (int rc = finalize_pending(c)) return rc;
     const DevStep* cur = c->d_step + c->cur;
     const float2* base;
     int bstride = 1;
@@ -1102,6 +1209,7 @@
 
 int mppi_optimal_traj(mppi_ctx* c, float* out_dev) {
     if (!c || !out_dev) return fail(MPPI_E_ARG, "null argument");
+    if (int rc = finalize_pending(c)) return rc;
     if (!c->upd_valid) return fail(MPPI_E_ARG, "mppi_optimal_traj needs a preceding MPPI_FLAG_FUSED_UPDATE launch");
     launch_traj(c, 1, c->d_upd, 1, nullptr, 1, reinterpret_cast<float4*>(out_dev));
     return launch_check("traj_kernel");
@@ -1109,6 +1217,7 @@
 
 int mppi_get_step_outputs(mppi_ctx* c, double* u_host, const float* traj_dev, float* traj_host) {
     if (!c || !u_host || (traj_dev && !traj_host)) return fail(MPPI_E_ARG, "bad argument");
+    if (int rc = finalize_pending(c)) return rc;
     const int T = c->cfg.T;
     const size_t ub = 2 * (size_t)T * sizeof(double), tb = 4 * (size_t)T * sizeof(float);
     float* h_traj = reinterpret_cast<float*>(c->h_out + 2 * kMaxT);
@@ -1288,6 +1397,7 @@
 
 int mppi_debug_nearest(mppi_ctx* c, const float* noise_dev, int K, int* slot_dev, float* pos_dev) {
     if (!c || !noise_dev || !slot_dev || !pos_dev || K < 1 || K > c->cfg.K_local) return fail(MPPI_E_ARG, "bad argument");
+    if (int rc = finalize_pending(c)) return rc;
     hipLaunchKernelGGL(nearest_debug_kernel, dim3((K + kThreads - 1) / kThreads), dim3(kThreads), 0, c->stream, c->kc,
                        c->stat, c->d_step + c->cur, reinterpret_cast<const float2*>(noise_dev), K, slot_dev,
                        reinterpret_cast<float2*>(pos_dev), c->ck);
@@ -1317,6 +1427,7 @@
 
 int mppi_debug_obstacle_hits(mppi_ctx* c, const float* noise_dev, int K, unsigned* mask_dev, float* dir_dev) {
     if (!c || !noise_dev || !mask_dev || !dir_dev || K < 1 || K > c->cfg.K_local) return fail(MPPI_E_ARG, "bad argument");
+    if (int rc = finalize_pending(c)) return rc;
     hipLaunchKernelGGL(obstacle_debug_kernel, dim3((K + kThreads - 1) / kThreads), dim3(kThreads), 0, c->stream, c->kc,
                        c->stat, c->d_step + c->cur, reinterpret_cast<const float2*>(noise_dev), K, mask_dev,
                        reinterpret_cast<float4*>(dir_dev), c->ck, c->ok);
@@ -1331,8 +1442,15 @@
 
 int mppi_sync(mppi_ctx* c) {
     if (!c) return fail(MPPI_E_ARG, "null context");
+    if (int rc = finalize_pending(c)) return rc;
     HIP_TRY(hipStreamSynchronize(c->stream));
     return check_timeout(c);
+}
+
+int mppi_debug_pending(const mppi_ctx* c, int* pending) {
+    if (!c || !pending) return fail(MPPI_E_ARG, "null argument");
+    *pending = c->pending ? 1 : 0;
+    return MPPI_OK;
 }
 
 int mppi_ctx_handoff(const mppi_ctx* c, int* poll) {
diff --git a/mppi_robotarm_amd/engine.py b/mppi_robotarm_amd/engine.py
--- a/mppi_robotarm_amd/engine.py
+++ b/mppi_robotarm_amd/engine.py
@@ -80,9 +80,9 @@
             return
         s = torch.cuda.current_stream(self.device)
         if s.cuda_stream != self.stream.cuda_stream:
+            N.check(self._c_set_stream(self._ctx, C.c_void_p(s.cuda_stream)), self._prefix + "set_stream")
             s.wait_stream(self.stream)
             self.stream = s
-            N.check(self._c_set_stream(self._ctx, C.c_void_p(s.cuda_stream)), self._prefix + "set_stream")
 
     def new_noise(self) -> torch.Tensor:
         return torch.empty((self.T, self.K_local, self.dim_u), dtype=torch.float32, device=self.device)
@@ -153,7 +153,9 @@
 
     def rollout(self, noise: torch.Tensor, S_out: torch.Tensor | None = None,
                 partial_out: torch.Tensor | None = None, fused_update: bool = False, exchange: bool = False,
-                host_out: bool = False) -> None:
+                host_out: bool = False, merge: str = "auto") -> None:
+        if merge not in ("auto", "inline"):
+            raise ValueError('merge must be "auto" or "inline"')
         self._sync_stream()
         self._check_noise(noise)
         if S_out is not None:
@@ -165,7 +167,8 @@
                                 C.c_void_p(partial_out.data_ptr()) if partial_out is not None else None,
                                 (N.MPPI_FLAG_FUSED_UPDATE if fused_update else 0)
                                 | (N.MPPI_FLAG_EXCHANGE if exchange else 0)
-                                | (N.MPPI_FLAG_HOST_OUT if host_out else 0)),
+                                | (N.MPPI_FLAG_HOST_OUT if host_out else 0)
+                                | (N.MPPI_FLAG_INLINE_MERGE if merge == "inline" and self._prefix == "mppi_" else 0)),
                 self._prefix + "rollout")
 
     def merge(self, partials: torch.Tensor, n: int, fused_update: bool = False, flags: int = 0) -> None:
@@ -277,6 +280,11 @@
         N.check(self._lib.mppi_ctx_handoff(self._ctx, C.byref(poll)), "mppi_ctx_handoff")
         self.handoff = "poll" if poll.value else "counter"
         self.obstacles, self.obstacle_cost = np.zeros((0, 3)), 0.0
+
+    def pending(self) -> bool:
+        p = C.c_int()
+        N.check(self._lib.mppi_debug_pending(self._ctx, C.byref(p)), "mppi_debug_pending")
+        return bool(p.value)
 
     def merge(self, partials: torch.Tensor, n: int, fused_update: bool = False, host_out: bool = False) -> None:
         super().merge(partials, n, fused_update, N.MPPI_FLAG_HOST_OUT if host_out else 0)
```

New measurement: 168.9 billion, median of 6. 1.08x the previous value.
